# sijieaaa/AGPlace

Measured on AMD Instinct MI355X. Metric: aerial-ground pairs/sec (backbone+ODE+pool), higher is better.
Workload: dtype f16 (fp16 x fp16, fp32 accumulate); 1 GPU; nuScenes-AG 6-cam (C3/C4): MM.forward_q on [b,3,224,1344] + DBVanilla2D on [b,1,3,224,224], ResNet18 stem+layer1-3, euler h=0.1 x3 FCODE, GeM, stage-2 fusion; inference forward; the voxel branch's pooled outputs enter as fixed tensors (SURVEY.md 8d); global_batch=64, parallelism=dp1, bn=per-rank (eval: running statistics), paired_trunks=True, hipgraph=True, steps_in_flight=2, library_default_precision=4, headline_is_library_default=True, streams=2, query_sub_batches_on_streams=1, query_input=fp32 normalised panorama

## Files before the change

### agplace_amd/_lib.py

```python
import ctypes as C
import os

_HERE = os.path.dirname(os.path.abspath(__file__))
LIB_PATH = os.environ.get("AGP_HIP_LIB") or os.path.join(_HERE, "lib", "libagplace_hip.so")

AGP_OK = 0
PREC_BF16 = 1
PREC_F16W2 = 2
PREC_BF16X3 = 3
PREC_F16 = 4
FMT_BF16, FMT_F16 = 0, 1
ACT = {None: 0, "id": 0, "relu": 1, "tanh": 2, "sigmoid": 3}
ODE = {"euler": 0, "midpoint": 1, "rk4": 2}
ODE_ADAPTIVE = {"dopri5": 3}
ODE_STATUS = {0: "ok", 1: "odeint_max_steps attempted steps did not reach t = 1", 2: "step size underflow (t + dt == t)",
              3: "the error ratio is NaN"}
ODE_MAX_STEPS_LIMIT = 4096
E_UNSUPPORTED = 3
GP_FLOATS = 1 + 16384 + 1
_ERR = {1: "AGP_E_BADARG (unsupported shape / enum / null pointer)",
        2: "AGP_E_LAUNCH (HIP launch failed)",
        3: "AGP_E_UNSUPPORTED"}


class ConvDesc(C.Structure):
    _fields_ = [
        ("in_hi", C.c_void_p), ("in_lo", C.c_void_p),
        ("w_hi", C.c_void_p), ("w_lo", C.c_void_p),
        ("out_hi", C.c_void_p), ("out_lo", C.c_void_p),
        ("res_hi", C.c_void_p), ("res_lo", C.c_void_p),
        ("scale", C.c_void_p), ("shift", C.c_void_p),
        ("n", C.c_int32), ("hin", C.c_int32), ("win", C.c_int32), ("cin", C.c_int32),
        ("pin", C.c_int32), ("in_w_step", C.c_int32),
        ("hout", C.c_int32), ("wout", C.c_int32), ("cout", C.c_int32), ("pout", C.c_int32),
        ("kh", C.c_int32), ("kw", C.c_int32), ("stride", C.c_int32), ("pad", C.c_int32),
        ("relu", C.c_int32), ("prec", C.c_int32),
        ("w_q8", C.c_void_p), ("w_q8_exp", C.c_int32),
        ("stat_partial", C.c_void_p),
        ("pool_partial", C.c_void_p), ("pool_p", C.c_void_p), ("pool_eps", C.c_float), ("hi_only", C.c_int32),
        ("w_cm", C.c_void_p),
        ("bstat_z_hi", C.c_void_p), ("bstat_z_lo", C.c_void_p), ("bstat_y_hi", C.c_void_p),
        ("bstat_mean", C.c_void_p), ("bstat_rstd", C.c_void_p),
        ("w_cm_lo", C.c_void_p),
        ("in_h16", C.c_void_p), ("out_absmax", C.c_void_p),
        ("pool_stat", C.c_int32), ("reserved0", C.c_int32),
    ]


class BBlock64Desc(C.Structure):
    _fields_ = [("inp", C.c_void_p), ("out", C.c_void_p), ("w1", C.c_void_p), ("w2", C.c_void_p),
                ("scale1", C.c_void_p), ("shift1", C.c_void_p), ("scale2", C.c_void_p), ("shift2", C.c_void_p),
                ("pool_partial", C.c_void_p), ("n", C.c_int32), ("h", C.c_int32), ("w", C.c_int32), ("form", C.c_int32)]


class VecProgOp(C.Structure):
    _fields_ = [("op", C.c_int32), ("dst", C.c_int32), ("r", C.c_int32 * 6), ("k", C.c_int32), ("act", C.c_int32),
                ("aux", C.c_int32), ("n", C.c_int32), ("f0", C.c_float), ("pad", C.c_int32), ("p", C.c_void_p * 6)]


VP_LOAD, VP_STORE, VP_LINEAR, VP_FCODE, VP_L2NORM, VP_LAYERNORM, VP_WSUM = 1, 2, 3, 4, 5, 6, 7
VECPROG_MAXOPS, VECPROG_NREG = 36, 6

_P, _I, _L, _F = C.c_void_p, C.c_int, C.c_int64, C.c_float

SIGNATURES = {
    "agp_version": (C.c_char_p, []),
    "agp_arch": (C.c_char_p, []),
    "agp_range_flag_set": (_P, [_P]),
    "agp_range_flag_get": (_P, []),
    "agp_split_f32": (_I, [_P, _P, _P, _L, _I, _P]),
    "agp_split_conv_weight": (_I, [_P, _I, _I, _I, _I, _I, _P, _P, _P]),
    "agp_split_conv_weight_both": (_I, [_P, _I, _I, _I, _I, _P, _P, _P, _P, _I, _P]),
    "agp_pack_f32_to_nhwc": (_I, [_P, _L, _L, _L, _L, _I, _I, _I, _I, _I, _I, _P, _P, _P]),
    "agp_pack_f32_to_nhwc4_h16": (_I, [_P, _L, _L, _L, _L, _I, _I, _I, _I, _I, _P, _P, _P, _P]),
    "agp_pack_u8_cams_to_nhwc": (_I, [_P, _I, _I, _I, _I, C.POINTER(_F), C.POINTER(_F), _I, _P, _P, _P]),
    "agp_resize_ksize": (_I, [_I, _I]),
    "agp_resize_coeffs": (_I, [_I, _I, C.POINTER(C.c_int32), C.POINTER(C.c_int32)]),
    "agp_resized_size": (_I, [_I, _I, _I, C.POINTER(_I), C.POINTER(_I)]),
    "agp_resize_u8_cams": (_I, [_P, _I, _I, _I, _I, _I, _I, _P, _P, _P, _P, _P, _P]),
    "agp_resize_pack_u8_cams": (_I, [_P, _I, _I, _I, _I, _I, _I, _P, _P, _P, _P, C.POINTER(_F), C.POINTER(_F), _I, _P, _P, _P]),
    "agp_unpack_nhwc_to_f32": (_I, [_P, _P, _I, _I, _I, _I, _I, _P, _P]),
    "agp_map_zero_halo": (_I, [_P, _P, _I, _I, _I, _I, _I, _P]),
    "agp_map_absmax": (_I, [_P, _P, _I, _I, _I, _I, _I, _P, _P]),
    "agp_map_absmax_reset": (_I, [_P, _I, _P]),
    "agp_conv2d_fwd": (_I, [C.POINTER(ConvDesc), _P]),
    "agp_conv2d_fwd_grouped": (_I, [C.POINTER(ConvDesc), _I, _P]),
    "agp_bblock64_fwd_grouped": (_I, [C.POINTER(BBlock64Desc), _I, _P]),
    "agp_bblock64_pool_floats": (_L, [C.POINTER(BBlock64Desc)]),
    "agp_bblock64_pool_finish": (_I, [_P, _I, _I, _I, _P, _P]),
    "agp_conv_w_q8_prepare": (_I, [_P, _I, _I, _P, C.POINTER(C.c_int32), _P]),
    "agp_conv2d_tile_plan": (_I, [C.POINTER(ConvDesc), _I, C.POINTER(C.c_int32)]),
    "agp_conv2d_stat_tiles": (_I, [C.POINTER(ConvDesc)]),
    "agp_conv2d_pool_blocks": (_I, [C.POINTER(ConvDesc)]),
    "agp_pool_from_conv": (_I, [_P, _I, _I, _I, _I, _P, _P, _P, _P]),
    "agp_bn_stats_from_partial": (_I, [_P, _I, _I, _L, _F, _F, _P, _P, _P, _P, _P, _P, _P, _P, _P]),
    "agp_stem_pool_fwd": (_I, [C.POINTER(ConvDesc), _P]),
    "agp_stem_pool_raw_fwd": (_I, [C.POINTER(ConvDesc), _I, _L, _L, _L, _L, _I, C.POINTER(_F), C.POINTER(_F), _P]),
    "agp_maxpool3x3s2_fwd": (_I, [_P, _P, _I, _I, _I, _I, _I, _P, _P, _I, _I, _I, _P, _P]),
    "agp_bcast_add_fwd": (_I, [_P, _P, _P, _I, _I, _I, _I, _I, _P, _P, _I, _P]),
    "agp_pool_workspace_floats": (_L, [_I, _I, _I, _I]),
    "agp_pool_fwd": (_I, [_P, _P, _I, _I, _I, _I, _I, _P, _F, _P, _P, _P, _P]),
    "agp_pool_f32_fwd": (_I, [_P, _L, _L, _L, _L, _I, _I, _I, _I, _P, _F, _P, _P, _P, _P]),
    "agp_gem_f32_bwd": (_I, [_P, _L, _L, _L, _L, _I, _I, _I, _I, _P, _F, _P, _P, _P, _P, _P]),
    "agp_linear_fwd": (_I, [_P, _P, _P, _P, _P, _P, _I, _I, _I, _I, _P, _P]),
    "agp_fcode_fwd": (_I, [_P, _P, _P, _P, _P, _P, _I, _I, _I, C.POINTER(_F), _I, _P, _P, _P]),
    "agp_fcode_traj_floats": (_L, [_I, _I, _I]),
    "agp_fcode_bwd_workspace_bytes": (_L, [_I, _I, _I]),
    "agp_fcode_bwd": (_I, [_P, _P, _P, _P, _I, _I, _I, C.POINTER(_F), _I, _P, _P, _P, _P, _L, _P]),
    "agp_fcode_adaptive_ctrl_bytes": (_L, [_I]),
    "agp_fcode_adaptive_ring_floats": (_L, [_I, _I, _I]),
    "agp_fcode_adaptive_fwd": (_I, [_P, _P, _P, _P, _P, _P, _I, _I, _I, C.c_double, C.c_double, _I, _P, _P, _I, _P, _P]),
    "agp_fcode_adaptive_bwd_workspace_bytes": (_L, [_I, _I]),
    "agp_fcode_adaptive_bwd": (_I, [_P, _P, _P, _P, _P, _I, _I, _I, _I, _P, _P, _P, _P, _L, _P]),
    "agp_linear_bwd_workspace_bytes": (_L, [_I, _I, _I]),
    "agp_linear_bwd": (_I, [_P, _P, _P, _P, _P, _I, _I, _I, _I, _P, _P, _P, _P, _L, _P]),
    "agp_layernorm_bwd": (_I, [_P, _P, _P, _P, _I, _I, _F, _I, _P, _P, _P, _P, _P]),
    "agp_l2normalize_bwd": (_I, [_P, _P, _I, _I, _P, _P]),
    "agp_layernorm_fwd": (_I, [_P, _P, _P, _P, _I, _I, _F, _I, _P, _P]),
    "agp_l2normalize_fwd": (_I, [_P, _I, _I, _P, _P]),
    "agp_wsum_fwd": (_I, [_P] * 12 + [_L, _P, _P]),
    "agp_dot_f32": (_I, [_P, _P, _L, _P, _P]),
    "agp_vecprog_run": (_I, [C.POINTER(VecProgOp), _I, _I, _I, C.POINTER(_F), _I, _P]),
    "agp_vecprog_run2": (_I, [C.POINTER(VecProgOp), _I, _I, C.POINTER(VecProgOp), _I, _I, _I, C.POINTER(_F), _I, _P]),
    "agp_conv2d_wgrad_workspace_bytes": (_L, [C.POINTER(ConvDesc)]),
    "agp_conv2d_wgrad": (_I, [C.POINTER(ConvDesc), _P, _P, _L, _P]),
    "agp_conv2d_wgrad_param": (_I, [C.POINTER(ConvDesc), _P, _I, _P, _L, _P]),
    "agp_upsample2_zero": (_I, [_P, _P, _I, _I, _I, _I, _I, _P, _P, _I, _I, _I, _P]),
    "agp_train_reduce_workspace_floats": (_L, [_I, _I, _I, _I]),
    "agp_bn_stats": (_I, [_P, _P, _I, _I, _I, _I, _I, _F, _F] + [_P] * 10),
    "agp_map_affine": (_I, [_P, _P, _P, _P, _P, _P, _I, _I, _I, _I, _I, _I, _P, _P, _P, _P]),
    "agp_bn_bwd": (_I, [_P] * 9 + [_I] * 6 + [_P] * 9),
    "agp_bn_bwd_from_partial": (_I, [_P, _I] + [_P] * 9 + [_I] * 7 + [_P] * 8),
    "agp_bn_bwd_frozen": (_I, [_P] * 9 + [_I] * 6 + [_P] * 9),
    "agp_bn_sums": (_I, [_P, _P, _I, _I, _I, _I, _I, _P, _P, _P]),
    "agp_bn_sums_from_partial": (_I, [_P, _I, _I, _L, _P, _P]),
    "agp_bn_stats_from_sums": (_I, [_P, _I, _F, _F] + [_P] * 9),
    "agp_bn_bwd_sums": (_I, [_P] * 8 + [_I] * 6 + [_P] * 5),
    "agp_bn_bwd_apply": (_I, [_P] * 11 + [_I] * 6 + [_P] * 6),
    "agp_bn_frozen_coeffs": (_I, [_P, _P, _P, _P, _I, _F, _P, _P, _P, _P, _P]),
    "agp_map_chan_sum": (_I, [_P, _P, _I, _I, _I, _I, _I, _P, _P, _P]),
    "agp_map_add": (_I, [_P] * 6 + [_I] * 5 + [_P, _P, _P]),
    "agp_maxpool3x3s2_bwd": (_I, [_P, _P, _P] + [_I] * 8 + [_P, _P, _P]),
    "agp_maxpool_bn_bwd": (_I, [_P, _P, _P, _I, _I, _I] + [_P] * 12 + [_I] * 7 + [_P] * 7),
    "agp_affine_maxpool3x3s2_fwd": (_I, [_P, _P, _P, _P] + [_I] * 5 + [_P, _P] + [_I] * 3 + [_P, _P, _P]),
    "agp_pool_bwd": (_I, [_P, _P, _P, _P, _P, _P, _F, _P, _P, _I, _I, _I, _I, _I, _P, _P, _P, _P]),
    "agp_netvlad_fwd": (_I, [_P, _P, _P, _I, _I, _I, _I, _I, _P, _P]),
    "agp_netvlad_bwd": (_I, [_P, _P, _P, _P, _I, _I, _I, _I, _I, _P, _P, _P, _P, _P]),
    "agp_netvlad_workspace_bytes": (_L, [_I, _I, _I, _I]),
    "agp_netvlad_fwd_mfma": (_I, [_P, _P, _P, _I, _I, _I, _I, _I, _P, _P, _L, _P]),
    "agp_sparse_conv_fwd": (_I, [_P, _P, _L, _P, _L, _I, _I, _I, _P, _P, _P, _P, _P, _P, _I, _P, _P, _I, _P, _P, _P, _P]),
    "agp_sparse_tile_taps": (_I, [_P, _L, _I, _L, _P, _P, _P, _L, _P]),
    "agp_sparse_zplane_perm": (_I, [_P, _P, _I, _L, _P, _P]),
    "agp_sparse_kernel_map": (_I, [_P, _L, _P, _L, _P, _I, _P, _P, _P]),
    "agp_sparse_kernel_map_grid": (_I, [_P, _L, _P, _L, _I, _I, _I, _P, _P, _P, _P, _P]),
    "agp_sparse_conv_cin1_fwd": (_I, [_P, _L, _P, _L, _I, _P, _I, _P, _P, _I, _P, _P, _P, _P]),
    "agp_sparse_conv0_fwd": (_I, [_P, _L, _P, _P, _I, _I, _P, _I, _P, _P, _I, _P, _P, _P, _I, _P]),
    "agp_sparse_coords_workspace_bytes": (_L, [_L, _I, _I]),
    "agp_sparse_build": (_I, [_P, _I, _L, _P, _I, _I, _P, _P, _P, _P, _P, _P, _L, _P]),
    "agp_sparse_coarsen": (_I, [_P, _P, _L, _I, _I, _P, _P, _P, _P, _L, _P]),
    "agp_sparse_points_workspace_bytes": (_L, [_L, _I]),
    "agp_sparse_build_points": (_I, [_P, _P, _L, _I, _F, _P, _I, _P, _P, _P, _P, _P, _P, _L, _P]),
    "agp_seg_pool_fwd": (_I, [_P, _P, _P, _I, _I, _P, _F, _P, _P, _P]),
    "agp_eca_scale_fwd": (_I, [_P, _I, _I, _P, _I, _P, _P]),
    "agp_seg_affine_fwd": (_I, [_P, _P, _P, _P, _P, _P, _P, _L, _I, _I, _P, _P, _P, _P]),
    "agp_sparse_conv_wgrad_workspace_bytes": (_L, [_L, _I, _I, _I]),
    "agp_sparse_conv_wgrad": (_I, [_P, _P, _L, _P, _L, _I, _I, _I, _P, _P, _P, _P, _L, _P]),
    "agp_sparse_conv_cin1_wgrad": (_I, [_P, _L, _P, _L, _I, _P, _P, _I, _P, _P, _I, _P]),
    "agp_seg_dot_fwd": (_I, [_P, _P, _P, _P, _P, _I, _I, _P, _P]),
    "agp_eca_scale_bwd": (_I, [_P, _P, _P, _P, _I, _I, _P, _I, _P, _P, _P]),
    "agp_seg_pool_bwd": (_I, [_P, _P, _P, _P, _P, _P, _P, _P, _F, _P, _P, _L, _I, _P, _P, _P, _P]),
    "agp_triplet_loss_workspace_floats": (_L, [_I]),
    "agp_triplet_loss": (_I, [_P, _I, _I, _P, _I, _F, _P, _P, _P, _P]),
    "agp_sare_loss": (_I, [_P, _I, _I, _P, _I, _I, _P, _P, _P, _P]),
    "agp_pairdist_loss_workspace_floats": (_L, [_I, _I]),
    "agp_pairdist_loss": (_I, [_P, _P, _I, _I, _I, _P, _P, _F, _F, _I, _P, _P, _P, _P, _P, _P]),
    "agp_mine_best_positive": (_I, [_P, _L, _P, _L, _I, _P, _P, _P, _P, _P]),
    "agp_knn_pad_rows": (_L, [_L]),
    "agp_knn_prepare_db": (_I, [_P, _L, _I, _I, _P, _P, _P, _P]),
    "agp_knn_workspace_bytes": (_L, [_L, _L, _I, _I]),
    "agp_knn_search": (_I, [_P, _L, _P, _P, _P, _P, _L, _I, _I, _I, _P, _P, _P, _L, _P]),
    "agp_knn_coarse_pass": (_I, [_P, _L, _P, _P, _P, _L, _I, _I, _P, _L, _P]),
}

_lib = None


def load():
    global _lib
    if _lib is not None:
        return _lib
    if not os.path.exists(LIB_PATH):
        raise RuntimeError(
            f"agplace_amd: HIP extension not built: {LIB_PATH} is missing. Run "
            "`python -c 'import __graft_entry__ as g; g.build()'` (or `make -C agplace_amd/csrc`). "
            "There is no CPU fallback.")
    import torch
    lib = C.CDLL(LIB_PATH)
    for name, (res, args) in SIGNATURES.items():
        fn = getattr(lib, name)
        fn.restype = res
        fn.argtypes = args
    _lib = lib
    return lib


def check(rc, what):
    if rc != AGP_OK:
        raise RuntimeError(f"{what} failed: {_ERR.get(rc, rc)}")


def ptr(t):
    return None if t is None else t.data_ptr()


def stream():
    import torch
    return torch.cuda.current_stream().cuda_stream
```

### agplace_amd/csrc/igemm.hip

```cpp

#ifndef AGP_SCHED
#define AGP_SCHED 0
#endif

#include "igemm_params.hpp"

namespace agp_igemm {


template <int BK> struct Swz;
template <> struct Swz<32> { __device__ static __forceinline__ int f(int row) { return (row >> 2) & 3; } };
template <> struct Swz<64> { __device__ static __forceinline__ int f(int row) { return (row >> 1) & 7; } };

template <int WM, int WN, int BK, int NPREC, int NST>
constexpr int igemm_lds_bytes() {
    constexpr int stage = (WM * 64 * PrecT<NPREC>::XPL + WN * 64 * PrecT<NPREC>::WPL) * BK * 2;
    constexpr int epi = WM * WN * 32 * EPI_ROWB + (NPREC == 3 ? WM * WN * 64 * 2 * 4 : 0);
    return (NST * stage > epi) ? NST * stage : epi;
}

#if defined(__HIP_DEVICE_COMPILE__)
template <int WM, int WN, int BK, int NPREC, int EPI, int NST, bool RG = false>
__device__ __forceinline__ void igemm_body(const IgemmParams& p, const int bid, uint32_t* rflag = nullptr) {
    constexpr int BM = WM * 64, BN = WN * 64, NW = WM * WN;
// ... 379 lines not shown
    }
    for (int i = n; i < 5; ++i) g.start[i] = grid;
    if (plan) {
        *plan = TilePlan{AGP_CONV_KERNEL_GENERIC, WM * 64, WN * 64, mt, one_nt ? ps[0].NT : 0, mt, 0, grid};
        return AGP_OK;
    }
    static std::atomic<uint64_t> attr_done{0};
    if (!agp_lds_attr((const void*)igemm_group_kernel<WM, WN, BK, NPREC, EPI_CONV, NST, RG>, lds, attr_done)) return AGP_E_LAUNCH;
    g.rflag = RG ? agp_range_flag_get() : nullptr;
    AGP_LAUNCH((igemm_group_kernel<WM, WN, BK, NPREC, EPI_CONV, NST, RG>), dim3(grid), dim3(WM * WN * 64), lds, s, g);
    AGP_CHECK_LAUNCH();
    return AGP_OK;
}

int launch_group_f16(IgemmParams* ps, int n, hipStream_t s, TilePlan* plan = nullptr) {
#if defined(AGP_TUNING)
    const int var = AGP_TUNE("GROUP_VARIANT", 0);
    if (var == 1) return launch_group_f16_cfg<64, 2>(ps, n, s, plan);
    if (var == 2) return launch_group_f16_cfg<32, 2>(ps, n, s, plan);
#endif
    return agp_rg_dispatch(agp_range_flag_get(), [&](auto rg) { return launch_group_f16_cfg<32, 3, decltype(rg)::value>(ps, n, s, plan); });
}

template <int WM, int WN, int BK, int NPREC, int EPI, int NST, bool RG = false>
int launch_cfg_rg(IgemmParams& p, uint32_t* rflag, hipStream_t s, TilePlan* plan = nullptr) {
    constexpr int lds = igemm_lds_bytes<WM, WN, BK, NPREC, NST>();
    static_assert(lds <= 160 * 1024, "LDS budget");
    constexpr int BM = WM * 64, BN = WN * 64;
    p.MT = (p.M + BM - 1) / BM;
    p.NT = (p.N + BN - 1) / BN;
    p.mt_chunk = (p.MT + 7) / 8;
    const int grid = p.mt_chunk * 8 * p.NT;
    if (plan) {
        *plan = TilePlan{AGP_CONV_KERNEL_GENERIC, BM, BN, p.MT, p.NT, p.MT, 0, grid};
        return AGP_OK;
    }
    static std::atomic<uint64_t> attr_done{0};
    if (!agp_lds_attr((const void*)igemm_kernel<WM, WN, BK, NPREC, EPI, NST, RG>, lds, attr_done)) return AGP_E_LAUNCH;
    const int splits = 1;
    AGP_LAUNCH((igemm_kernel<WM, WN, BK, NPREC, EPI, NST, RG>), dim3(grid, splits), dim3(WM * WN * 64), lds, s, p, rflag);
    AGP_CHECK_LAUNCH();
    return AGP_OK;
}
template <int WM, int WN, int BK, int NPREC, int EPI, int NST>
int launch_cfg(IgemmParams& p, hipStream_t s, TilePlan* plan = nullptr) {
    if constexpr (EPI == EPI_CONV && PrecT<NPREC>::F16) {
        uint32_t* const rflag = agp_range_flag_get();
        return agp_rg_dispatch(rflag, [&](auto rg) { return launch_cfg_rg<WM, WN, BK, NPREC, EPI, NST, decltype(rg)::value>(p, rflag, s, plan); });
    }
    return launch_cfg_rg<WM, WN, BK, NPREC, EPI, NST>(p, nullptr, s, plan);
}

inline int igemm_variant() { return AGP_TUNE("IGEMM_VARIANT", 0); }

template <int EPI>
int launch_igemm(IgemmParams& p, int prec, hipStream_t s, TilePlan* plan = nullptr) {
    const bool wide = (p.N % 128 == 0) || (EPI == EPI_GMIN);
    const int var = igemm_variant();
    p.dbg = AGP_TUNE("IGEMM_DBG", 0);
    if (EPI == EPI_GMIN && var == 0) {
        if (prec == AGP_PREC_BF16X3) return launch_cfg<4, 2, 32, 3, EPI, 2>(p, s, plan);
        if (prec == AGP_PREC_BF16)
            return p.CK % 64 == 0 ? launch_cfg<4, 2, 64, 1, EPI, 2>(p, s, plan) : launch_cfg<4, 2, 32, 1, EPI, 2>(p, s, plan);
        if (prec == AGP_PREC_F16)
            return p.CK % 64 == 0 ? launch_cfg<4, 2, 64, 4, EPI, 2>(p, s, plan) : launch_cfg<4, 2, 32, 4, EPI, 2>(p, s, plan);
        return AGP_E_BADARG;
    }
    if (prec == AGP_PREC_BF16X3) {
#if defined(AGP_TUNING)
        if (var == 1) return wide ? launch_cfg<2, 2, 32, 3, EPI, 3>(p, s, plan) : launch_cfg<4, 1, 32, 3, EPI, 3>(p, s, plan);
        if (var == 2) return wide ? launch_cfg<4, 2, 32, 3, EPI, 2>(p, s, plan) : launch_cfg<4, 1, 32, 3, EPI, 2>(p, s, plan);
        if (var == 3) return wide ? launch_cfg<4, 2, 32, 3, EPI, 3>(p, s, plan) : launch_cfg<4, 1, 32, 3, EPI, 3>(p, s, plan);
        if (var == 4) return wide ? launch_cfg<2, 2, 32, 3, EPI, 4>(p, s, plan) : launch_cfg<4, 1, 32, 3, EPI, 4>(p, s, plan);
#endif
        return wide ? launch_cfg<2, 2, 32, 3, EPI, 2>(p, s, plan) : launch_cfg<4, 1, 32, 3, EPI, 2>(p, s, plan);
    } else if (prec == AGP_PREC_BF16) {
        if (p.CK % 64 == 0) {
#if defined(AGP_TUNING)
            if (var == 1) return wide ? launch_cfg<2, 2, 64, 1, EPI, 3>(p, s, plan) : launch_cfg<4, 1, 64, 1, EPI, 3>(p, s, plan);
#endif
            return wide ? launch_cfg<2, 2, 64, 1, EPI, 2>(p, s, plan) : launch_cfg<4, 1, 64, 1, EPI, 2>(p, s, plan);
        }
        return wide ? launch_cfg<2, 2, 32, 1, EPI, 2>(p, s, plan) : launch_cfg<4, 1, 32, 1, EPI, 2>(p, s, plan);
    }
    if constexpr (EPI == EPI_CONV) {
        if (prec == AGP_PREC_F16W2)
            return wide ? launch_cfg<2, 2, 32, 2, EPI, 2>(p, s, plan) : launch_cfg<4, 1, 32, 2, EPI, 2>(p, s, plan);
        if (prec == AGP_PREC_F16) {
#if defined(AGP_TUNING)
            if (var == 5) {
                if (p.CK % 64 == 0) return wide ? launch_cfg<2, 2, 64, 4, EPI, 2>(p, s, plan) : launch_cfg<4, 1, 64, 4, EPI, 2>(p, s, plan);
                return wide ? launch_cfg<2, 2, 32, 4, EPI, 2>(p, s, plan) : launch_cfg<4, 1, 32, 4, EPI, 2>(p, s, plan);
            }
#endif
            if (p.tap_stride && var == 0) {
                if (!wide) return launch_cfg<4, 1, 32, 4, EPI, 2>(p, s, plan);
                if ((int64_t)((p.M + 255) / 256) * (p.N / 128) >= 512) return launch_cfg<4, 2, 32, 4, EPI, 3>(p, s, plan);
            }
            return wide ? launch_cfg<2, 2, 32, 4, EPI, 3>(p, s, plan) : launch_cfg<4, 1, 32, 4, EPI, 3>(p, s, plan);
        }
    }
    return AGP_E_BADARG;
}

}
using namespace agp_igemm;

int agp_internal_conv_d16(agp_igemm::IgemmParams& p, int prec, hipStream_t s, agp_igemm::TilePlan* plan);
int agp_internal_conv_d16_pool(agp_igemm::IgemmParams& p, int prec, hipStream_t s);
int agp_internal_stem_raw(agp_igemm::IgemmParams& p, int kind, const void* x, long long sn, long long sc, long long sh, long long sw,
                          int h, int w, int ncam, const float* mean3, const float* std3, hipStream_t s);
int agp_internal_conv_kxr(agp_igemm::IgemmParams& p, const agp_conv_desc* d, hipStream_t s, agp_igemm::TilePlan* plan);

extern "C" int agp_conv2d_stat_tiles(const agp_conv_desc* d) {
    if (!d || d->prec != AGP_PREC_BF16X3) return 0;
    const int force = AGP_TUNE("CONV_KERNEL", 0);
    if (d->in_w_step != d->cin && !force && d->cout % 64 == 0)
        return (int)(((int64_t)d->n * d->hout * d->wout + 255) / 256);
    if (d->in_w_step == d->cin && !force && !AGP_TUNE("IGEMM_VARIANT", 0) && d->cin % 32 == 0 && d->cout % 64 == 0 &&
        !(d->kh == 3 && d->kw == 3 && d->stride == 1 && d->pad == 1)) {
        const int bm = (d->cout % 128 == 0) ? 128 : 256;
        return (int)(((int64_t)d->n * d->hout * d->wout + bm - 1) / bm);
    }
    const bool kxr_ok = d->kh == 3 && d->kw == 3 && d->stride == 1 && d->pad == 1 && d->pin == 1 &&
                        d->pout == 1 && d->in_w_step == d->cin && d->hout == d->hin && d->wout == d->win &&
                        (int64_t)d->n * (d->hin + 2) * (d->win + 2) * d->cin * 2 < (1ll << 31);
    if (!kxr_ok || d->cin % 32 || d->cout % 64 || (force && force != 3)) return 0;
    const int64_t m = (int64_t)d->n * d->hin * (d->win + 2);
    const int bm = (d->cout % 128 == 0 && !d->hi_only) ? 128 : 256;
    return (int)((m + bm - 1) / bm);
}

static bool conv_kxr_ok(const agp_conv_desc* d);
bool agp_internal_use_kxr2(const agp_conv_desc* d);

extern "C" int agp_conv2d_pool_blocks(const agp_conv_desc* d) {
    if (!d || d->prec != AGP_PREC_F16 || d->in_lo || d->out_lo || d->cin % 32 || d->cout % 64 || d->n <= 0) return 0;
    if (!conv_kxr_ok(d) || !agp_internal_use_kxr2(d) || AGP_TUNE("CONV_KERNEL", 0) || AGP_TUNE("NO_CONV_POOL", 0)) return 0;
    const int64_t rp = ((int64_t)d->hin * (d->win + 2) + 63) / 64 * 64;
    if ((int64_t)d->n * rp >= (1ll << 31)) return 0;
    return (int)(((int64_t)d->n * rp + 511) / 512 * 8);
}

static bool conv_kxr_ok(const agp_conv_desc* d) {
    return d->kh == 3 && d->kw == 3 && d->stride == 1 && d->pad == 1 && d->pin == 1 &&
           d->pout == 1 && d->in_w_step == d->cin && d->hout == d->hin && d->wout == d->win &&
           (int64_t)d->n * (d->hin + 2) * (d->win + 2) * d->cin * 2 < (1ll << 31);
}

static int conv_fill_params(const agp_conv_desc* d, IgemmParams& p);
void agp_internal_conv_kxr_geometry(agp_igemm::IgemmParams& p, const agp_conv_desc* d);
bool agp_internal_use_kxr2(const agp_conv_desc* d);
int agp_internal_conv_kxr2(agp_igemm::IgemmParams* ps, int n, hipStream_t s, agp_igemm::TilePlan* plan);
int agp_internal_conv_s2(agp_igemm::IgemmParams* ps, const agp_conv_desc* descs, int n, hipStream_t s, agp_igemm::TilePlan* plan);

static int conv2d_fwd_one(const agp_conv_desc* d, void* stream, TilePlan* plan);

static int conv2d_fwd_group(const agp_conv_desc* descs, int n, void* stream, TilePlan* plan) {
    if (!descs || n <= 0) return AGP_E_BADARG;
    bool group = n >= 2 && n <= 4;
    for (int i = 0; i < n && group; ++i) {
        const agp_conv_desc* d = descs + i;
        group = d->in_hi && d->w_hi && d->out_hi && !d->in_lo && !d->out_lo && !d->res_lo && d->n > 0 &&
                d->cin % 32 == 0 && d->cout % 64 == 0 && conv_kxr_ok(d) && agp_internal_use_kxr2(d) &&
                d->cin == descs[0].cin && d->cout == descs[0].cout && !AGP_TUNE("CONV_KERNEL", 0);
    }
    if (!group && !AGP_TUNE("CONV_KERNEL", 0) && !AGP_TUNE("NO_S2", 0)) {
        const int h = n / 2;
        bool s2 = (n == 2 || n == 4);
        for (int i = 0; i < h && s2; ++i) {
            const agp_conv_desc* c = descs + i;
            const agp_conv_desc* d = descs + h + i;
            s2 = c->prec == AGP_PREC_F16 && d->prec == AGP_PREC_F16 && c->in_hi && c->w_hi && c->out_hi && d->w_hi && d->out_hi &&
                 !c->in_lo && !c->out_lo && !d->in_lo && !d->out_lo && !c->res_hi && !d->res_hi && !c->stat_partial && !d->stat_partial &&
                 !c->pool_partial && !d->pool_partial &&
                 c->kh == 3 && c->kw == 3 && c->stride == 2 && c->pad == 1 && c->pin == 1 && c->pout == 1 && c->in_w_step == c->cin &&
                 d->kh == 1 && d->kw == 1 && d->stride == 2 && d->pad == 0 && d->pin == 1 && d->pout == 1 && d->in_w_step == d->cin &&
                 d->in_hi == c->in_hi && d->n == c->n && d->hin == c->hin && d->win == c->win && d->cin == c->cin &&
                 d->cout == c->cout && d->hout == c->hout && d->wout == c->wout && !d->relu &&
                 c->hout == (c->hin - 1) / 2 + 1 && c->wout == (c->win - 1) / 2 + 1 &&
                 c->cin % 32 == 0 && c->cout % 64 == 0 && c->n > 0 && c->cin == descs[0].cin && c->cout == descs[0].cout &&
                 (int64_t)c->n * (c->hin + 2) * (c->win + 2) * c->cin * 2 < (1ll << 31) &&
                 (int64_t)c->n * (c->hout + 2) * (c->wout + 2) * c->cout * 2 < (1ll << 31);
        }
        if (s2) {
            IgemmParams ps[2];
            for (int i = 0; i < h; ++i) {
                ps[i] = IgemmParams{};
                const int rc = conv_fill_params(descs + i, ps[i]);
                if (rc != AGP_OK) return rc;
                const agp_conv_desc* d = descs + h + i;
                ps[i].w2_hi = d->w_hi; ps[i].w2_cm = d->w_cm; ps[i].scale2 = d->scale; ps[i].shift2 = d->shift; ps[i].o2_hi = d->out_hi;
            }
            return agp_internal_conv_s2(ps, descs, h, (hipStream_t)stream, plan);
        }
    }
    if (!group) {
        bool g2 = n >= 2 && n <= 4 && !AGP_TUNE("CONV_KERNEL", 0) && !AGP_TUNE("NO_IGEMM_GROUP", 0);
        for (int i = 0; i < n && g2; ++i) {
            const agp_conv_desc* d = descs + i;
            g2 = d->in_hi && d->w_hi && d->out_hi && !d->in_lo && !d->out_lo && !d->res_lo && d->n > 0 &&
                 d->prec == AGP_PREC_F16 && !d->stat_partial && d->cin % 64 == 0 && d->cout % 128 == 0 &&
                 !conv_kxr_ok(d) && d->in_w_step == d->cin && !(d->pin < d->pad);
        }
        if (g2) {
            IgemmParams ps[4];
            for (int i = 0; i < n; ++i) {
                ps[i] = IgemmParams{};
                const int rc = conv_fill_params(descs + i, ps[i]);
                if (rc != AGP_OK) return rc;
            }
            return launch_group_f16(ps, n, (hipStream_t)stream, plan);
        }
        if (plan && n > 1) return AGP_E_UNSUPPORTED;
        for (int i = 0; i < n; ++i) {
            const int rc = conv2d_fwd_one(descs + i, stream, plan);
            if (rc != AGP_OK) return rc;
        }
        return AGP_OK;
    }
    IgemmParams ps[4];
    for (int i = 0; i < n; ++i) {
        ps[i] = IgemmParams{};
        const int rc = conv_fill_params(descs + i, ps[i]);
        if (rc != AGP_OK) return rc;
        agp_internal_conv_kxr_geometry(ps[i], descs + i);
    }
    return agp_internal_conv_kxr2(ps, n, (hipStream_t)stream, plan);
}

extern "C" int agp_conv2d_fwd_grouped(const agp_conv_desc* descs, int n, void* stream) {
    return conv2d_fwd_group(descs, n, stream, nullptr);
}

extern "C" int agp_conv2d_fwd(const agp_conv_desc* d, void* stream) { return conv2d_fwd_one(d, stream, nullptr); }

extern "C" int agp_conv2d_tile_plan(const agp_conv_desc* descs, int n, int32_t plan[8]) {
    if (!descs || !plan || n <= 0) return AGP_E_BADARG;
    TilePlan tp = {};
    const int rc = n == 1 ? conv2d_fwd_one(descs, nullptr, &tp) : conv2d_fwd_group(descs, n, nullptr, &tp);
    if (rc != AGP_OK) return rc;
    const int32_t v[8] = {tp.kernel, tp.BM, tp.BN, tp.MT, tp.NT, tp.MT_full, tp.half_tiles, tp.grid};
    for (int i = 0; i < 8; ++i) plan[i] = v[i];
    return AGP_OK;
}

static int conv2d_fwd_one(const agp_conv_desc* d, void* stream, TilePlan* plan) {
    if (!d || !d->in_hi || !d->w_hi || !d->out_hi) return AGP_E_BADARG;
    if (d->prec == AGP_PREC_BF16X3) {
        if ((!d->hi_only && (!d->in_lo || !d->w_lo)) || !d->out_lo || (d->res_hi && !d->res_lo)) return AGP_E_BADARG;
    } else if (d->prec == AGP_PREC_F16W2 || d->prec == AGP_PREC_F16) {
        if (d->in_lo || d->out_lo || d->res_lo) return AGP_E_BADARG;
        if (d->prec == AGP_PREC_F16W2 && !d->w_lo) return AGP_E_BADARG;
    } else {
        return AGP_E_BADARG;
    }
    if (d->cin % 32 || d->cout % 64 || d->n <= 0) return AGP_E_BADARG;
    if (d->pin < d->pad && d->in_w_step == d->cin) return AGP_E_BADARG;
    IgemmParams p = {};
    {
        const int rc = conv_fill_params(d, p);
        if (rc != AGP_OK) return rc;
    }
    const int force = AGP_TUNE("CONV_KERNEL", 0);
    const bool kxr_ok = conv_kxr_ok(d);
    const bool stem = d->in_w_step != d->cin;
#if defined(AGP_TUNING)
    if (p.dbg & 0x1000000) {
        const uint64_t a = ((uint64_t)(uint32_t)AGP_TUNE("CENSUS_BUF_HI", 0) << 32) | (uint32_t)AGP_TUNE("CENSUS_BUF_LO", 0);
        p.gmin = (float*)(uintptr_t)a;
        if (!p.gmin) p.dbg &= ~0x1000000;
    }
#endif
    int which = force ? force : (kxr_ok ? 3 : (stem ? 2 : 1));
    if (which == 3 && !kxr_ok) which = stem ? 2 : 1;
    if (d->hi_only && (d->prec != AGP_PREC_BF16X3 || which != 3)) return AGP_E_BADARG;
    if (d->w_cm && d->w_cm == d->w_hi && (which != 3 || !p.w_cm)) return AGP_E_BADARG;
    if (which == 3) return agp_internal_conv_kxr(p, d, (hipStream_t)stream, plan);
    if (which == 2) return agp_internal_conv_d16(p, d->prec, (hipStream_t)stream, plan);
    return launch_igemm<EPI_CONV>(p, d->prec, (hipStream_t)stream, plan);
}

static int conv_fill_params(const agp_conv_desc* d, IgemmParams& p) {
    const int hp = d->hin + 2 * d->pin, wp = d->win + 2 * d->pin;
    const int wstep = d->in_w_step;
    const int64_t x_elems = (int64_t)d->n * hp * wp * wstep;
    const int64_t w_elems = (int64_t)d->cout * d->kh * d->kw * d->cin;
    if (x_elems * 2 >= (1ll << 32) || w_elems * 2 >= (1ll << 31)) return AGP_E_BADARG;
    p.x_hi = d->in_hi; p.x_lo = d->in_lo; p.x_bytes = (uint32_t)(x_elems * 2);
    p.w_hi = d->w_hi; p.w_lo = d->w_lo; p.w_bytes = (uint32_t)(w_elems * 2);
    if (d->prec == AGP_PREC_F16W2 && d->w_q8) { p.w_q8 = d->w_q8; p.w_q8_exp = d->w_q8_exp; }
    if (d->prec == AGP_PREC_F16 && d->w_cm) p.w_cm = d->w_cm;
    if ((d->prec == AGP_PREC_F16W2 || d->prec == AGP_PREC_BF16X3) && d->w_cm && d->kh == 3 && d->kw == 3 &&
        d->stride == 1 && d->pad == 1 && d->in_w_step == d->cin && (d->w_cm_lo || (d->hi_only && d->prec == AGP_PREC_BF16X3))) {
        p.w_cm = d->w_cm; p.w_cm_lo = d->w_cm_lo;
    }
    if (d->stat_partial) {
        if (agp_conv2d_stat_tiles(d) <= 0) return AGP_E_BADARG;
        p.stat_partial = d->stat_partial;
        if (d->bstat_z_hi) {
            if (!d->bstat_mean || !d->bstat_rstd || d->in_w_step != d->cin ||
                !(d->kh == 3 && d->kw == 3 && d->stride == 1 && d->pad == 1))
                return AGP_E_BADARG;
            p.bs_z_hi = d->bstat_z_hi; p.bs_z_lo = d->bstat_z_lo; p.bs_y_hi = d->bstat_y_hi;
            p.bs_mean = d->bstat_mean; p.bs_rstd = d->bstat_rstd;
        }
    } else if (d->bstat_z_hi) {
        return AGP_E_BADARG;
    }
    if (d->pool_partial) {
        if (agp_conv2d_pool_blocks(d) <= 0) return AGP_E_BADARG;
        if (d->pool_stat != 0 && d->pool_stat != 1) return AGP_E_BADARG;
        p.pool_partial = d->pool_partial; p.pool_p = d->pool_stat ? nullptr : d->pool_p; p.pool_eps = d->pool_eps; p.pool_sq = d->pool_stat;
    }
    p.M = d->n * d->hout * d->wout;
    p.N = d->cout;
    p.KW = d->kw; p.CK = d->cin; p.ntaps = d->kh * d->kw;
    p.Ktot = d->kh * d->kw * d->cin;
    p.d_howo = make_fastdiv((uint32_t)(d->hout * d->wout));
    p.d_wo = make_fastdiv((uint32_t)d->wout);
    p.x_sw = wstep; p.x_sh = wp * wstep; p.x_sn = hp * wp * wstep;
    p.x_base = ((d->pin - d->pad) * wp + (d->pin - d->pad)) * wstep;
    p.sy = d->stride; p.sx = d->stride;
    const int hop = d->hout + 2 * d->pout, wop = d->wout + 2 * d->pout;
    p.o_hi = d->out_hi; p.o_lo = d->out_lo;
    p.o_sw = d->cout; p.o_sh = wop * d->cout; p.o_sn = hop * wop * d->cout;
    p.o_base = (d->pout * wop + d->pout) * d->cout;
    p.r_hi = d->res_hi; p.r_lo = d->res_lo;
    p.scale = d->scale; p.shift = d->shift; p.relu = d->relu;
    p.dbg = AGP_TUNE("IGEMM_DBG", 0);
    return AGP_OK;
}

int agp_internal_gmin(const void* q_hi, const void* q_lo, int64_t nq, const void* db_hi,
                      const void* db_lo, const float* db_norm, int64_t nb, int64_t nb_pad, int d,
                      int prec, float* gmin, int gq_stride, hipStream_t s) {
    IgemmParams p = {};
    if (nq * d * 2 >= (1ll << 32) || nb_pad * d * 2 >= (1ll << 31)) return AGP_E_BADARG;
    p.x_hi = q_hi; p.x_lo = q_lo; p.x_bytes = (uint32_t)(nq * d * 2);
    p.w_hi = db_hi; p.w_lo = db_lo; p.w_bytes = (uint32_t)(nb_pad * d * 2);
    p.M = (int)nq; p.N = (int)nb; p.Ktot = d; p.KW = 1; p.CK = d; p.ntaps = 1;
    p.d_howo = make_fastdiv(1); p.d_wo = make_fastdiv(1);
    p.x_sn = d; p.x_sh = 0; p.x_sw = 0; p.x_base = 0; p.sy = 1; p.sx = 1;
    p.gmin = gmin; p.wnorm = db_norm; p.gq_stride = gq_stride;
    return launch_igemm<EPI_GMIN>(p, prec, s);
}


extern "C" int agp_sparse_conv_fwd(const void* f_hi, const void* f_lo, int64_t n_in_rows, const int32_t* nbr, int64_t n_out,
                                   int cin, int cout, int ntaps, const void* w_hi, const void* w_lo, const float* scale,
                                   const float* shift, const void* res_hi, const void* res_lo, int relu, void* out_hi,
                                   void* out_lo, int prec, const int64_t* n_dev, const int32_t* row_perm, const uint32_t* tile_taps, void* stream) {
    if (!f_hi || !nbr || !w_hi || !out_hi || n_out <= 0 || n_in_rows <= 0 || ntaps <= 0) return AGP_E_BADARG;
    if (cin % 32 || cout % 64) return AGP_E_BADARG;
    if (prec == AGP_PREC_BF16X3) { if (!f_lo || !w_lo || !out_lo || (res_hi && !res_lo)) return AGP_E_BADARG; }
    else if (prec == AGP_PREC_F16W2 || prec == AGP_PREC_F16) { if (f_lo || out_lo || res_lo || (prec == AGP_PREC_F16W2 && !w_lo)) return AGP_E_BADARG; }
    else return AGP_E_BADARG;
    const int64_t x_elems = n_in_rows * cin, w_elems = (int64_t)cout * ntaps * cin;
    if (x_elems * 2 >= (1ll << 31) || w_elems * 2 >= (1ll << 31) || n_out * (int64_t)cout * 2 >= (1ll << 31)) return AGP_E_BADARG;
    IgemmParams p = {};
    p.x_hi = f_hi; p.x_lo = f_lo; p.x_bytes = (uint32_t)(x_elems * 2);
    p.w_hi = w_hi; p.w_lo = w_lo; p.w_bytes = (uint32_t)(w_elems * 2);
    p.M = (int)n_out; p.N = cout; p.Ktot = ntaps * cin;
    p.KW = ntaps; p.CK = cin; p.ntaps = ntaps;
    p.d_howo = make_fastdiv((uint32_t)n_out); p.d_wo = make_fastdiv((uint32_t)n_out);
    p.x_sn = 0; p.x_sh = 0; p.x_sw = 0; p.x_base = 0; p.sy = 1; p.sx = 1;
    p.xrow_tab = nbr; p.tap_stride = (int)n_out; p.tab_mul = cin; p.m_dev = n_dev; p.row_perm = row_perm; p.tile_taps = tile_taps;
    p.o_hi = out_hi; p.o_lo = out_lo; p.o_sn = 0; p.o_sh = 0; p.o_sw = cout; p.o_base = 0;
    p.r_hi = res_hi; p.r_lo = res_lo; p.scale = scale; p.shift = shift; p.relu = relu;
    return launch_igemm<EPI_CONV>(p, prec, (hipStream_t)stream);
}

static int stem_pool_impl(const agp_conv_desc* d, int kind, int64_t sn, int64_t sc, int64_t sh, int64_t sw, int ncam,
                          const float* mean3, const float* std3, void* stream) {
    if (!d || !d->in_hi || !d->w_hi || !d->out_hi || d->in_lo || d->out_lo || d->res_hi) return AGP_E_BADARG;
    if (d->prec != AGP_PREC_F16W2 && d->prec != AGP_PREC_F16) return AGP_E_BADARG;
    if (d->prec == AGP_PREC_F16W2 && !d->w_lo) return AGP_E_BADARG;
    if (d->cin != 32 || d->in_w_step != 4 || d->kw != 1 || d->kh != 7 || d->stride != 2 || d->pad != 3 || d->pin != 3 ||
        d->cout != 64 || !d->relu || d->n <= 0)
        return AGP_E_BADARG;
    const int h1 = (d->hin + 2 * 3 - 7) / 2 + 1, w1 = (d->win + 2 * 3 - 7) / 2 + 1;
    const int h2 = (h1 + 2 - 3) / 2 + 1, w2 = (w1 + 2 - 3) / 2 + 1;
    if (d->hout != h2 || d->wout != w2) return AGP_E_BADARG;
    IgemmParams p = {};
    const int hp = d->hin + 6, wp = d->win + 6;
    const int64_t x_elems = (int64_t)d->n * hp * wp * 4;
    const int64_t w_elems = (int64_t)64 * 7 * 32;
    if (kind == 0 && x_elems * 2 >= (1ll << 32)) return AGP_E_BADARG;
// ... 27 lines not shown
```

### agplace_amd/csrc/igemm_kxr2.hip

```cpp

#include <type_traits>

#include "igemm_params.hpp"

#ifndef AGP_CENSUS
#define AGP_CENSUS 0
#endif
#if AGP_CENSUS
#define KXR2_STAMP(i) do { if (census && tid == 0) rec[4 + (i)] = __builtin_amdgcn_s_memrealtime(); } while (0)
#else
#define KXR2_STAMP(i) do { } while (0)
#endif

namespace agp_igemm {

constexpr int KXR2_MAXP = 4;
struct Kxr2Group {
    IgemmParams p[KXR2_MAXP];
    int mt_end[KXR2_MAXP];
    int nprob, MT, NT, mt_chunk;
};

constexpr int KXR2_BM = 256, KXR2_MINB = 3;
constexpr int kxr2_lds_bytes() { return 2 * (KXR2_BM + 16) * 64 + 3 * 64 * 64 + 2 * 64 * 4; }
// ... 249 lines not shown
    }

    KXR2_STAMP(2);
    if (p.dbg & 128) {
        float t = 0.f;
#pragma unroll
        for (int a = 0; a < TN; ++a)
#pragma unroll
            for (int b = 0; b < TM; ++b)
#pragma unroll
                for (int r = 0; r < 16; ++r) t += acc[a][b][r];
        if (t == 1.2345e30f) ((float*)p.o_hi)[0] = t;
        return;
    }
    asm volatile("s_waitcnt lgkmcnt(0)" ::: "memory");
    __builtin_amdgcn_s_barrier();
    constexpr int ERS = 144;
    char* const strip = smem + wave * (32 * ERS);
    const int a_off = l31 * ERS + lh * 16;
    const int l_off = (lane >> 3) * ERS + (lane & 7) * 16;
    const float* tb = tab + 8 * lh;
    bf16_t* const ohi = (bf16_t*)p.o_hi;
    const float relu_lo = p.relu ? 0.f : -65504.f;
    RangeTrack<RG> rg;
    u32x4 rres[TM][TN * 2];
    if (rhi) {
#pragma unroll
        for (int tm = 0; tm < TM; ++tm) {
#pragma unroll
            for (int i = 0; i < 4; ++i) *(u32x4*)(strip + l_off + i * (8 * ERS)) = rpf[tm * 4 + i];
            __builtin_amdgcn_fence(__ATOMIC_RELEASE, "wavefront");
#pragma unroll
            for (int jj = 0; jj < TN * 2; ++jj) rres[tm][jj] = *(const u32x4*)(strip + a_off + jj * 32);
            __builtin_amdgcn_fence(__ATOMIC_RELEASE, "wavefront");
        }
    }
    float psum[2] = {0.f, 0.f};
    const float* const ppp = POOL ? p.pool_p : nullptr;
    const float pool_pw = ppp ? ppp[0] : 1.f, pool_eps = POOL ? p.pool_eps : 0.f;
    const bool pool_cube = pool_pw == 3.f;
    const bool pool_sq = POOL && p.pool_sq;
#pragma unroll
    for (int tm = 0; tm < TM; ++tm) {
        u32x4 outv[TN * 2];
#pragma unroll
        for (int jp = 0; jp < TN; ++jp) {
            f32x4 sc4[2][2], sh4[2][2];
#pragma unroll
            for (int u = 0; u < 2; ++u) {
                const int jj = 2 * jp + u;
                sc4[u][0] = *(const f32x4*)(tb + 16 * jj);
                sc4[u][1] = *(const f32x4*)(tb + 16 * jj + 4);
                sh4[u][0] = *(const f32x4*)(tb + BN + 16 * jj);
                sh4[u][1] = *(const f32x4*)(tb + BN + 16 * jj + 4);
            }
#pragma unroll
            for (int u = 0; u < 2; ++u) {
                const int jj = 2 * jp + u;
                float v[8];
#pragma unroll
                for (int e = 0; e < 8; ++e) v[e] = acc[jj >> 1][tm][8 * (jj & 1) + e] * sc4[u][e >> 2][e & 3] + sh4[u][e >> 2][e & 3];
                if (rhi) {
                    float r[8];
                    unpack8_h(rres[tm][jj], r);
#pragma unroll
                    for (int e = 0; e < 8; ++e) v[e] += r[e];
                }
                rg.any8(v);
                outv[jj] = pack8_h_lo(v, relu_lo);
            }
        }
#pragma unroll
        for (int jj = 0; jj < TN * 2; ++jj) *(u32x4*)(strip + a_off + jj * 32) = outv[jj];
        __builtin_amdgcn_fence(__ATOMIC_RELEASE, "wavefront");
        u32x4 lines[4];
#pragma unroll
        for (int i = 0; i < 4; ++i) lines[i] = *(const u32x4*)(strip + l_off + i * (8 * ERS));
#pragma unroll
        for (int i = 0; i < 4; ++i) {
            const int off = eoff[tm * 4 + i];
            if (off >= 0) *(u32x4*)(ohi + off) = lines[i];
        }
        if constexpr (POOL) {
            if (ppart) {
                const bf16_t* const col = (const bf16_t*)strip + lane;
                const uint32_t mk = pmask[tm];
#pragma unroll
                for (int p8 = 0; p8 < 32; p8 += 8) {
                    float v[8];
#pragma unroll
                    for (int u = 0; u < 8; ++u) v[u] = h2f(col[(p8 + u) * (ERS / 2)]);
#pragma unroll
                    for (int u = 0; u < 8; ++u) {
                        const bool a = (mk >> (p8 + u)) & 1u;
                        psum[0] += a ? v[u] : 0.f;
                        if (pool_sq) {
                            psum[1] += a ? v[u] * v[u] : 0.f;
                        } else if (ppp) {
                            const float c = fmaxf(v[u], pool_eps);
                            const float gq = pool_cube ? c * c * c : __builtin_exp2f(pool_pw * __builtin_log2f(c));
                            psum[1] += a ? gq : 0.f;
                        }
                    }
                }
            }
        }
        __builtin_amdgcn_fence(__ATOMIC_RELEASE, "wavefront");
    }
    if constexpr (POOL) {
        if (ppart && n0 + lane < pN) {
            float* o = ppart + ((size_t)(mt * NW + wave) * 2) * pN + n0 + lane;
            o[0] = psum[0];
            if (ppp || pool_sq) o[pN] = psum[1];
        }
    }
    rg.flush(rg_word(rf...), relu_lo);
#if AGP_CENSUS
    if (census && tid == 0) {
        rec[4 + 3] = __builtin_amdgcn_s_memrealtime();
        asm volatile("s_waitcnt vmcnt(0)" ::: "memory");
        rec[3] = __builtin_amdgcn_s_memrealtime();
    }
#endif
#endif
}

template <bool POOL, bool RG>
int launch_kxr2(Kxr2Group& g, hipStream_t s, TilePlan* plan) {
    constexpr int BM = KXR2_BM, lds = kxr2_lds_bytes();
    static_assert(lds * KXR2_MINB <= 160 * 1024, "LDS budget of the intended workgroups per CU");
    static std::atomic<uint64_t> attr_done{0};
    int mt = 0;
    for (int i = 0; i < g.nprob; ++i) {
        mt += (g.p[i].M + BM - 1) / BM;
        g.mt_end[i] = mt;
    }
    const XcdGrid xg = xcd_grid(mt, (g.p[0].N + 63) / 64);
    if (plan) return plan_xcd(plan, AGP_CONV_KERNEL_KXR2, BM, 64, xg);
    g.MT = xg.MT;
    g.NT = xg.NT;
    g.mt_chunk = xg.mt_chunk;
    if (!agp_lds_attr(RG ? (const void*)igemm_kxr2_kernel<POOL, uint32_t*> : (const void*)igemm_kxr2_kernel<POOL>, lds, attr_done)) return AGP_E_LAUNCH;
    if constexpr (RG) {
        AGP_LAUNCH((igemm_kxr2_kernel<POOL, uint32_t*>), dim3(xg.blocks), dim3(256), lds, s, g, agp_range_flag_get());
    } else {
        AGP_LAUNCH((igemm_kxr2_kernel<POOL>), dim3(xg.blocks), dim3(256), lds, s, g);
    }
    AGP_CHECK_LAUNCH();
    return AGP_OK;
}

}

int agp_internal_conv_kxrw(agp_igemm::IgemmParams* ps, int n, hipStream_t s, agp_igemm::TilePlan* plan);

int agp_internal_conv_kxr2(agp_igemm::IgemmParams* ps, int n, hipStream_t s, agp_igemm::TilePlan* plan) {
    using namespace agp_igemm;
    if (n < 1 || n > KXR2_MAXP) return AGP_E_BADARG;
    if (AGP_TUNE("KXR_WIDE", 1) && ps[0].N % 128 == 0) return agp_internal_conv_kxrw(ps, n, s, plan);
    Kxr2Group g = {};
    g.nprob = n;
    for (int i = 0; i < n; ++i) {
        if (ps[i].N != ps[0].N || ps[i].CK != ps[0].CK) return AGP_E_BADARG;
        g.p[i] = ps[i];
    }
    bool pool = false;
    for (int i = 0; i < n; ++i) pool = pool || ps[i].pool_partial != nullptr;
    return agp_rg_dispatch(agp_range_flag_get(), [&](auto rg) {
        constexpr bool RG = decltype(rg)::value;
        if (pool) return launch_kxr2<true, RG>(g, s, plan);
        return launch_kxr2<false, RG>(g, s, plan);
    });
}
```

### agplace_amd/csrc/igemm_kxrw.hip

```cpp

#include <type_traits>

#include "igemm_params.hpp"

namespace agp_igemm {

constexpr int KXRW_MAXP = 4;
struct KxrwGroup {
    IgemmParams p[KXRW_MAXP];
    int mt_end[KXRW_MAXP];
    int nprob, MT, NT, mt_chunk;
    int MT_full, half_bid0;
    uint32_t* rflag;
    uint32_t r_bytes[KXRW_MAXP];
};
constexpr uint32_t KXRW_ROOB = 0xffffff00u;

constexpr int KW_ROWB = 64;
template <int TM_, int TN_> struct KwShape {
    static constexpr int BM = 128 * TM_, BN = 32 * TN_, BMX = BM + 16;
    static constexpr int XBUF = BMX * KW_ROWB, WTAP = BN * KW_ROWB;
    static constexpr int LDS = 2 * XBUF + 3 * WTAP + 2 * BN * 4;
    static constexpr int STRIP = 32 * 2 * BN, XWAVES = XBUF / STRIP, SPARE = LDS + (TM_ == 1 ? 2048 : 0);
    static constexpr int EPI_LDS = SPARE + (4 - XWAVES) * STRIP;
};

template <bool POOL, int TM_, int TN_, bool RG, bool RES>
__device__ __forceinline__ void kxrw_tile(const KxrwGroup& g, const int pid, const int m0, const int n0) {
#if defined(__HIP_DEVICE_COMPILE__)
    using SH = KwShape<TM_, TN_>;
    constexpr int BN = SH::BN, NW = 4, TM = TM_, TN = TN_, ROWB = KW_ROWB;
    constexpr int X_BUF = SH::XBUF, W_TAP = SH::WTAP;
    constexpr int XINS = SH::BMX / 16;
    constexpr int NX = (XINS + NW - 1) / NW;
    constexpr int NWP = BN / (NW * 16);
    static_assert(TN == 4 && (TM == 2 || TM == 1), "the full tile (256 x 128) and its half tile (128 x 128)");
    static_assert(NWP == 2 && (NX == 5 || NX == 3), "the vmcnt counts exist for these");
    extern __shared__ __attribute__((aligned(16))) char smem[];
    char* const ws = smem + 2 * X_BUF;
    float* const tab = (float*)(ws + 3 * W_TAP);

    const int tid = threadIdx.x;
    const int lane = tid & 63;
    const int wave = __builtin_amdgcn_readfirstlane(tid >> 6);

    const IgemmParams& p = g.p[pid];

    const FastDiv d_howo = p.d_howo, d_wo = p.d_wo;
    const int pM = p.M, pN = p.N, pKtot = p.Ktot;
    const uint32_t pR = (uint32_t)p.img_rows;
    const int x_sn = p.x_sn, x_sh_ = p.x_sh, x_sw = p.x_sw, x_base = p.x_base;
    const int o_sn = p.o_sn, o_sw = p.o_sw, o_base = p.o_base;
    const float* const pscale = p.scale;
    const float* const pshift = p.shift;

    const int lrow = lane >> 2, lpos = lane & 3;
    int xoff[NX], woff[NWP];
#pragma unroll
    for (int q = 0; q < NX; ++q) {
        int ins = wave + NW * q;
        ins = ins < XINS ? ins : XINS - 1;
        const int row = ins * 16 + lrow;
        const int m = m0 + row;
        const uint32_t img = fdiv((uint32_t)m, d_howo);
        const uint32_t rem = (uint32_t)m - img * d_howo.d;
        const uint32_t y = fdiv(rem, d_wo);
        const uint32_t xq = rem - y * d_wo.d;
        const int el = (int)img * x_sn + (int)y * x_sh_ + (int)xq * x_sw + x_base;
        xoff[q] = el * 2 + ((lpos ^ swz32(row)) << 4);
    }
#pragma unroll
    for (int i = 0; i < NWP; ++i) {
        const int row = (wave + NW * i) * 16 + lrow;
        int n = n0 + row;
        n = n < pN ? n : pN - 1;
        woff[i] = (p.w_cm ? n * 64 : n * pKtot * 2) + ((lpos ^ swz32(row)) << 4);
    }
    const __amdgpu_buffer_rsrc_t rx = __builtin_amdgcn_make_buffer_rsrc((void*)p.x_hi, 0, p.x_bytes, 0x00020000);
    const __amdgpu_buffer_rsrc_t rw = __builtin_amdgcn_make_buffer_rsrc((void*)(p.w_cm ? p.w_cm : p.w_hi), 0, p.w_bytes, 0x00020000);

    const int CK = __builtin_amdgcn_readfirstlane(p.CK), x_sh = __builtin_amdgcn_readfirstlane(x_sh_);
    const int cchunks = CK / 32;
    const int nsteps = 3 * cchunks;
    const int tapb = CK * 2;
    float tab_s = 1.f, tab_t = 0.f;
    if (tid < BN) {
        const int n = n0 + tid < pN ? n0 + tid : pN - 1;
        if (pscale) tab_s = pscale[n];
        if (pshift) tab_t = pshift[n];
    }
    float pool_pw_v = 1.f;
    if (POOL && p.pool_p) pool_pw_v = p.pool_p[0];
    auto load_x = [&](int buf, int ky_, int cc_) {
        const int xs = __builtin_amdgcn_readfirstlane((ky_ * x_sh + cc_ * 32) * 2);
        char* base_ = smem + buf * X_BUF;
#pragma unroll
        for (int q = 0; q < NX; ++q) {
            int ins = wave + NW * q;
            ins = ins < XINS ? ins : XINS - 1;
            __builtin_amdgcn_raw_ptr_buffer_load_lds(rx, LDS_PTR(base_ + ins * 1024), 16, xoff[q], xs, 0, 0);
        }
    };
    const int wmul = __builtin_amdgcn_readfirstlane(p.w_cm ? pN : 1);
    auto load_w = [&](int slot, int wbytes) {
        const int so = __builtin_amdgcn_readfirstlane(wbytes * wmul);
#pragma unroll
        for (int i = 0; i < NWP; ++i)
            __builtin_amdgcn_raw_ptr_buffer_load_lds(rw, LDS_PTR(ws + slot * W_TAP + (wave + NW * i) * 1024), 16, woff[i], so, 0, 0);
    };
    load_x(0, 0, 0);
    load_w(0, 0);
    load_w(1, tapb);

    const int l31 = lane & 31, lh = lane >> 5;
    int xrd[3][2], wrd[2];
#pragma unroll
    for (int kx = 0; kx < 3; ++kx)
#pragma unroll
        for (int ks = 0; ks < 2; ++ks) {
            const int r = wave * (TM * 32) + l31 + kx;
            xrd[kx][ks] = r * ROWB + (((2 * ks + lh) ^ swz32(r)) << 4);
        }
    {
        const int wrow = (l31 & 0x13) | ((l31 & 4) << 1) | ((l31 & 8) >> 1);
#pragma unroll
        for (int ks = 0; ks < 2; ++ks) wrd[ks] = wrow * ROWB + (((2 * ks + lh) ^ swz32(wrow)) << 4);
    }

    f32x16 acc[TN][TM];
#pragma unroll
    for (int a = 0; a < TN; ++a)
#pragma unroll
        for (int b = 0; b < TM; ++b)
#pragma unroll
            for (int r = 0; r < 16; ++r) acc[a][b][r] = 0.f;

    constexpr int LPP = BN / 8, PPI = 64 / LPP, NEI = 32 / PPI;
    int eoff[TM * NEI];
    {
        const uint32_t wlast = d_wo.d - 1;
        const int img_extra = o_sn - (int)d_howo.d * o_sw;
#pragma unroll
        for (int q = 0; q < TM * NEI; ++q) {
            const int m = m0 + wave * (TM * 32) + (q / NEI) * 32 + (q % NEI) * PPI + lane / LPP;
            const uint32_t mm = (uint32_t)(m < pM ? m : pM - 1);
            const uint32_t img = fdiv(mm, d_howo);
            const uint32_t rem = mm - img * d_howo.d;
            const uint32_t y = fdiv(rem, d_wo);
            const uint32_t xq = rem - y * d_wo.d;
            const bool ok = (m < pM) && rem < pR && xq != 0 && xq != wlast;
            const int chunk = (lane % LPP) ^ (((q % NEI) * PPI + lane / LPP) & 15);
            eoff[q] = ok ? (int)mm * o_sw + (int)img * img_extra + o_base + n0 + 8 * chunk : -1;
        }
    }
    float* const ppart = POOL ? p.pool_partial : nullptr;
    static_assert(LPP == 16 && PPI == 4 && NEI == 8 && SH::STRIP == NEI * 1024, "a tile row = 8 pieces of 4 pixel lines of 256 bytes");
    const int xidle = nsteps & 1;
    char* const strip0 = wave < SH::XWAVES ? smem + xidle * X_BUF + wave * SH::STRIP : smem + SH::SPARE + (wave - SH::XWAVES) * SH::STRIP;
    char* const strip1 = wave < 2 ? smem + (xidle ^ 1) * X_BUF + wave * SH::STRIP : ws + (wave - 2) * SH::STRIP;
    static_assert(TM == 1 || (SH::XWAVES == 2 && 2 * SH::STRIP <= 3 * W_TAP), "tile row 1: two waves per X buffer, two in the W ring");
    const __amdgpu_buffer_rsrc_t rr = __builtin_amdgcn_make_buffer_rsrc((void*)p.r_hi, 0, g.r_bytes[pid], 0x00020000);
    auto load_residual = [&](char* strip, int tm, int i) {
        const int off = eoff[tm * NEI + i];
        __builtin_amdgcn_raw_ptr_buffer_load_lds(rr, LDS_PTR(strip + i * 1024), 16, off >= 0 ? off * 2 : (int)KXRW_ROOB, 0, 0, 0);
    };

    int ky = 0, cc = 0;
    wait_vm_lgkm<NWP>();
    __builtin_amdgcn_s_barrier();
    if (tid < BN) { tab[tid] = tab_s; tab[BN + tid] = tab_t; }
    const float pool_pw = __builtin_bit_cast(float, __builtin_amdgcn_readfirstlane(__builtin_bit_cast(int, pool_pw_v)));
    auto phase = [&](auto KX, auto LAST, const char* xb, int st_, int nky_, int ncc_, int wcur_, int wnext_) {
        constexpr int kx = decltype(KX)::value;
        constexpr bool last = decltype(LAST)::value;
        constexpr int nres = last && RES && kx < 2 ? NEI / 2 : 0;
        const char* wb = ws + kx * W_TAP;
        bf16x8 xf[2][TM], wf[2][TN];
#pragma unroll
        for (int t = 0; t < TM; ++t) xf[0][t] = *(const bf16x8*)(xb + xrd[kx][0] + t * (32 * ROWB));
#pragma unroll
        for (int t = 0; t < TN; ++t) wf[0][t] = *(const bf16x8*)(wb + wrd[0] + t * (32 * ROWB));
        constexpr int ndma = (kx == 0 ? (last ? NWP : NWP + NX) : (last ? 0 : NWP)) + nres;
        static_assert(ndma <= 8, "one piece per MFMA pair");
#pragma unroll
        for (int t = 0; t < TM; ++t) xf[1][t] = *(const bf16x8*)(xb + xrd[kx][1] + t * (32 * ROWB));
#pragma unroll
        for (int t = 0; t < TN; ++t) wf[1][t] = *(const bf16x8*)(wb + wrd[1] + t * (32 * ROWB));
        auto piece = [&](int i) {
            if (nres && i >= ndma - nres) {
                load_residual(strip0, 0, kx * (NEI / 2) + i - (ndma - nres));
            } else if (kx == 0) {
                if (i < NWP) {
                    const int so = __builtin_amdgcn_readfirstlane((wcur_ + 2 * tapb) * wmul);
                    __builtin_amdgcn_raw_ptr_buffer_load_lds(rw, LDS_PTR(ws + 2 * W_TAP + (wave + NW * i) * 1024), 16, woff[i], so, 0, 0);
                } else {
                    const int q = i - NWP;
                    const int xs = __builtin_amdgcn_readfirstlane((nky_ * x_sh + ncc_ * 32) * 2);
                    int ins = wave + NW * q;
                    ins = ins < XINS ? ins : XINS - 1;
                    __builtin_amdgcn_raw_ptr_buffer_load_lds(rx, LDS_PTR(smem + ((st_ + 1) & 1) * X_BUF + ins * 1024), 16, xoff[q], xs, 0, 0);
                }
            } else {
                const int so = __builtin_amdgcn_readfirstlane((wnext_ + (kx - 1) * tapb) * wmul);
                __builtin_amdgcn_raw_ptr_buffer_load_lds(rw, LDS_PTR(ws + (kx - 1) * W_TAP + (wave + NW * i) * 1024), 16, woff[i], so, 0, 0);
            }
        };
        int ip = 0;
#pragma unroll
        for (int ks = 0; ks < 2; ++ks)
#pragma unroll
            for (int tn = 0; tn < TN; ++tn)
#pragma unroll
                for (int tm = 0; tm < TM; ++tm) {
                    acc[tn][tm] = __builtin_amdgcn_mfma_f32_32x32x16_f16(__builtin_bit_cast(f16x8, wf[ks][tn]),
                                                                         __builtin_bit_cast(f16x8, xf[ks][tm]), acc[tn][tm], 0, 0, 0);
                    if ((TM == 1 || (tm & 1)) && ip < ndma) { piece(ip); ++ip; }
                }
        __builtin_amdgcn_sched_group_barrier(0x100, 2 * (TM + TN), 0);
#pragma unroll
        for (int i = 0; i < 8; ++i) {
            __builtin_amdgcn_sched_group_barrier(0x008, TM == 1 ? 1 : 2, 0);
            if (i < ndma) __builtin_amdgcn_sched_group_barrier(0x010, 1, 0);
        }
        __builtin_amdgcn_sched_barrier(0);
    };
    using I0 = std::integral_constant<int, 0>; using I1 = std::integral_constant<int, 1>; using I2 = std::integral_constant<int, 2>;
    using BF = std::false_type; using BT = std::true_type;
    for (int st = 0; st < nsteps - 1; ++st) {
        int nky = ky, ncc = cc + 1;
        if (ncc == cchunks) { ncc = 0; ++nky; }
        const int wcur = (ky * 3 * CK + cc * 32) * 2, wnext = (nky * 3 * CK + ncc * 32) * 2;
        const char* xb = smem + (st & 1) * X_BUF;
        phase(I0{}, BF{}, xb, st, nky, ncc, wcur, wnext);
        wait_vm_lgkm<NX + NWP>();
        __builtin_amdgcn_s_barrier();
        phase(I1{}, BF{}, xb, st, nky, ncc, wcur, wnext);
        wait_vm_lgkm<NX + NWP>();
        __builtin_amdgcn_s_barrier();
        phase(I2{}, BF{}, xb, st, nky, ncc, wcur, wnext);
        wait_vm_lgkm<NWP>();
        __builtin_amdgcn_s_barrier();
        ky = nky; cc = ncc;
    }
    {
        const int st = nsteps - 1;
        const int wcur = (ky * 3 * CK + cc * 32) * 2;
        const char* xb = smem + (st & 1) * X_BUF;
        phase(I0{}, BT{}, xb, st, 0, 0, wcur, 0);
        wait_vm_lgkm<NWP + (RES ? NEI / 2 : 0)>();
        __builtin_amdgcn_s_barrier();
        phase(I1{}, BT{}, xb, st, 0, 0, wcur, 0);
        wait_vm_lgkm<(RES ? NEI : 0)>();
        __builtin_amdgcn_s_barrier();
        phase(I2{}, BT{}, xb, st, 0, 0, wcur, 0);
    }

    asm volatile("s_waitcnt lgkmcnt(0)" ::: "memory");
    __builtin_amdgcn_s_barrier();
    if constexpr (RES) {
        if constexpr (TM == 2) {
#pragma unroll
            for (int i = 0; i < NEI; ++i) load_residual(strip1, 1, i);
            wait_vm_lgkm<NEI>();
        } else {
            wait_vm_lgkm<0>();
        }
    }
    const int a_off = l31 * (2 * BN) + ((lh ^ (l31 & 1)) << 4), a_swz = (l31 >> 1) & 7;
    const int l_off = lane * 16;
    const float* tb = tab + 8 * lh;
    bf16_t* const ohi = (bf16_t*)p.o_hi;
    const float relu_lo = p.relu ? 0.f : -65504.f;
    RangeTrack<RG> rg;
    float psum[2][2] = {{0.f, 0.f}, {0.f, 0.f}};
    float psum0[2][2] = {{0.f, 0.f}, {0.f, 0.f}};
    const float* const ppp = POOL ? p.pool_p : nullptr;
    const float pool_eps = POOL ? p.pool_eps : 0.f;
    const bool pool_cube = pool_pw == 3.f;
    const bool pool_sq = POOL && p.pool_sq;
#pragma unroll
    for (int tm = 0; tm < TM; ++tm) {
        char* const strip = tm == 0 ? strip0 : strip1;
        if constexpr (POOL && TM == 2) {
            if (tm == 1) {
#pragma unroll
                for (int a = 0; a < 2; ++a)
#pragma unroll
                    for (int b = 0; b < 2; ++b) { psum0[a][b] = psum[a][b]; psum[a][b] = 0.f; }
            }
        }
        u32x4 rres[TN * 2];
        if constexpr (RES) {
#pragma unroll
            for (int jj = 0; jj < TN * 2; ++jj) rres[jj] = *(const u32x4*)(strip + a_off + ((jj ^ a_swz) << 5));
        }
        u32x4 outv[TN * 2];
#pragma unroll
        for (int jj = 0; jj < TN * 2; ++jj) {
            const f32x4 s0 = *(const f32x4*)(tb + 16 * jj), s1 = *(const f32x4*)(tb + 16 * jj + 4);
            const f32x4 h0 = *(const f32x4*)(tb + BN + 16 * jj), h1 = *(const f32x4*)(tb + BN + 16 * jj + 4);
            float v[8];
#pragma unroll
            for (int e = 0; e < 8; ++e)
                v[e] = acc[jj >> 1][tm][8 * (jj & 1) + e] * (e < 4 ? s0[e & 3] : s1[e & 3]) + (e < 4 ? h0[e & 3] : h1[e & 3]);
            if constexpr (RES) {
                float r[8];
                unpack8_h(rres[jj], r);
#pragma unroll
                for (int e = 0; e < 8; ++e) v[e] += r[e];
            }
            rg.any8(v);
            outv[jj] = pack8_h_lo(v, relu_lo);
        }
#pragma unroll
        for (int jj = 0; jj < TN * 2; ++jj) *(u32x4*)(strip + a_off + ((jj ^ a_swz) << 5)) = outv[jj];
        __builtin_amdgcn_fence(__ATOMIC_RELEASE, "wavefront");
        u32x4 lines[NEI];
#pragma unroll
        for (int i = 0; i < NEI; ++i) lines[i] = *(const u32x4*)(strip + l_off + i * 1024);
        if constexpr (TM == 2) {
            if (tm == 0 && RES) wait_vm_lgkm<0>();
        }
#pragma unroll
        for (int i = 0; i < NEI; ++i) {
            const int off = eoff[tm * NEI + i];
            if (off >= 0) *(u32x4*)(ohi + off) = lines[i];
        }
        if constexpr (POOL) {
            if (ppart) {
#pragma unroll
                for (int i = 0; i < NEI; ++i)
                    if (eoff[tm * NEI + i] < 0) *(u32x4*)(strip + l_off + i * 1024) = u32x4{0u, 0u, 0u, 0u};
                __builtin_amdgcn_fence(__ATOMIC_RELEASE, "wavefront");
                auto sweep = [&](auto STAT) {
#pragma clang fp contract(off)
                    constexpr int stat = decltype(STAT)::value;
#pragma unroll
                    for (int p8 = 0; p8 < 32; p8 += 8) {
                        uint32_t w[8];
#pragma unroll
                        for (int u = 0; u < 8; ++u) w[u] = *(const uint32_t*)(strip + (p8 + u) * (2 * BN) + ((lane * 4) ^ (((p8 + u) & 15) << 4)));
#pragma unroll
                        for (int u = 0; u < 8; ++u) {
                            const float v0 = h2f((bf16_t)(w[u] & 0xffffu)), v1 = h2f((bf16_t)(w[u] >> 16));
                            psum[0][0] += v0;
                            psum[1][0] += v1;
                            if constexpr (stat == 1) {
                                psum[0][1] += v0 * v0;
                                psum[1][1] += v1 * v1;
                            } else if constexpr (stat >= 2) {
                                const float c0 = fmaxf(v0, pool_eps), c1 = fmaxf(v1, pool_eps);
                                psum[0][1] += stat == 2 ? c0 * c0 * c0 : __builtin_exp2f(pool_pw * __builtin_log2f(c0));
                                psum[1][1] += stat == 2 ? c1 * c1 * c1 : __builtin_exp2f(pool_pw * __builtin_log2f(c1));
                            }
                        }
                    }
                };
                using I3 = std::integral_constant<int, 3>;
                if (pool_sq) sweep(I1{});
                else if (!ppp) sweep(I0{});
                else if (pool_cube) sweep(I2{});
                else sweep(I3{});
            }
        }
        __builtin_amdgcn_fence(__ATOMIC_RELEASE, "wavefront");
    }
    if constexpr (POOL) {
        if (ppart) {
            if constexpr (TM == 2) {
#pragma unroll
                for (int a = 0; a < 2; ++a)
#pragma unroll
                    for (int b = 0; b < 2; ++b) psum[a][b] = psum0[a][b] + psum[a][b];
            }
            if constexpr (TM == 1) {
                float* const scr = (float*)(ws + 3 * W_TAP) + 2 * BN;
                if (wave & 1) *(f32x4*)(scr + ((wave >> 1) * 64 + lane) * 4) = f32x4{psum[0][0], psum[0][1], psum[1][0], psum[1][1]};
                __syncthreads();
                if (!(wave & 1)) {
                    const f32x4 o = *(const f32x4*)(scr + ((wave >> 1) * 64 + lane) * 4);
                    psum[0][0] += o[0]; psum[0][1] += o[1]; psum[1][0] += o[2]; psum[1][1] += o[3];
                }
            }
            if (TM == 2 || !(wave & 1)) {
                const int block = m0 / 64 + (TM == 2 ? wave : (wave >> 1));
#pragma unroll
                for (int h = 0; h < 2; ++h) {
                    const int n = n0 + 2 * lane + h;
                    if (n < pN) {
                        float* o = ppart + ((size_t)block * 2) * pN + n;
                        o[0] = psum[h][0];
                        if (ppp || pool_sq) o[pN] = psum[h][1];
                    }
                }
            }
        }
    }
    rg.flush(g.rflag, relu_lo);
#endif
}

template <bool POOL, bool MIX, bool RG>
__global__ void __launch_bounds__(256, 2) igemm_kxrw_kernel(KxrwGroup g) {
#if defined(__HIP_DEVICE_COMPILE__)
    constexpr int TM_ = 2, TN_ = 4;
    constexpr int BM = KwShape<TM_, TN_>::BM, BN = KwShape<TM_, TN_>::BN;
    const int bid = blockIdx.x;
    const int gNT = g.NT, gnprob = g.nprob;
    const int e0 = g.mt_end[0], e1 = g.mt_end[1], e2 = g.mt_end[2];
    int mt, nt, sub = 0;
    bool half = false;
    if (MIX && bid >= g.half_bid0) {
        const int h = bid - g.half_bid0;
        nt = h % gNT;
        const int hm = h / gNT;
        mt = g.MT_full + (hm >> 1);
        sub = hm & 1;
        half = true;
        if (mt >= g.MT) return;
    } else {
        const int xcd = bid & 7, j = bid >> 3;
        nt = j % gNT;
        mt = xcd * g.mt_chunk + j / gNT;
        if (mt >= g.MT_full) return;
    }
    const int pid = group_problem(mt, gnprob, e0, e1, e2);
    const int n0 = nt * BN;
    if constexpr (MIX) {
        if (half) {
            const int m0 = mt * BM + sub * (BM / 2);
            if (m0 >= g.p[pid].M) return;
            if (g.p[pid].r_hi) kxrw_tile<POOL, 1, TN_, RG, true>(g, pid, m0, n0);
            else kxrw_tile<POOL, 1, TN_, RG, false>(g, pid, m0, n0);
            return;
        }
    }
    if (g.p[pid].r_hi) kxrw_tile<POOL, TM_, TN_, RG, true>(g, pid, mt * BM, n0);
    else kxrw_tile<POOL, TM_, TN_, RG, false>(g, pid, mt * BM, n0);
#endif
}

struct KxrwPlan {
    int MT_full, mt_chunk, half_bid0, half_tiles, blocks;
    bool mix;
};
inline KxrwPlan kxrw_plan(int MT, int NT) {
    KxrwPlan k = {};
    k.MT_full = MT;
    const int slots = 512, T = MT * NT;
    const int tail = T - (T - 1) / slots * slots;
    if (tail <= slots / 4 && tail % NT == 0) {
        k.MT_full = MT - tail / NT;
        k.mix = true;
    }
    const XcdGrid xg = xcd_grid(k.MT_full, NT);
    k.mt_chunk = xg.mt_chunk;
    k.half_bid0 = xg.blocks;
    k.half_tiles = k.mix ? 2 * (MT - k.MT_full) * NT : 0;
    k.blocks = k.half_bid0 + k.half_tiles;
    return k;
}

template <bool POOL, bool MIX, bool RG>
int launch_kxrw(KxrwGroup& g, const KxrwPlan& k, hipStream_t s) {
    constexpr int lds = KwShape<2, 4>::EPI_LDS;
    static_assert(2 * lds <= 160 * 1024, "two workgroups per CU");
    static_assert(KwShape<1, 4>::EPI_LDS <= lds, "half tiles: their stage, the pooling scratch and their strips fit the full tile's LDS");
    static std::atomic<uint64_t> attr_done{0};
    if (!agp_lds_attr((const void*)igemm_kxrw_kernel<POOL, MIX, RG>, lds, attr_done)) return AGP_E_LAUNCH;
    AGP_LAUNCH((igemm_kxrw_kernel<POOL, MIX, RG>), dim3(MIX ? k.blocks : k.half_bid0), dim3(256), lds, s, g);
    AGP_CHECK_LAUNCH();
    return AGP_OK;
}

}

int agp_internal_conv_kxrw(agp_igemm::IgemmParams* ps, int n, hipStream_t s, agp_igemm::TilePlan* plan) {
    using namespace agp_igemm;
    if (n < 1 || n > KXRW_MAXP || ps[0].N % 128) return AGP_E_BADARG;
    constexpr int bm = KwShape<2, 4>::BM, bn = KwShape<2, 4>::BN;
    KxrwGroup g = {};
    g.nprob = n;
    int mt = 0;
    bool pool = false;
    for (int i = 0; i < n; ++i) {
        if (ps[i].N != ps[0].N || ps[i].CK != ps[0].CK) return AGP_E_BADARG;
        g.p[i] = ps[i];
        mt += (ps[i].M + bm - 1) / bm;
        g.mt_end[i] = mt;
        pool = pool || ps[i].pool_partial != nullptr;
        const int64_t rb = (int64_t)(ps[i].M / (int)ps[i].d_howo.d) * ps[i].o_sn * 2;
        if (ps[i].r_hi && (rb <= 0 || rb > (int64_t)KXRW_ROOB)) return AGP_E_BADARG;
        g.r_bytes[i] = (uint32_t)rb;
    }
    g.MT = mt;
    g.NT = ps[0].N / bn;
    const KxrwPlan k = kxrw_plan(g.MT, g.NT);
    if (plan) {
        *plan = TilePlan{AGP_CONV_KERNEL_KXRW, bm, bn, g.MT, g.NT, k.MT_full, k.half_tiles, k.blocks};
        return AGP_OK;
    }
    const bool mix = k.mix;
    g.MT_full = k.MT_full;
    g.mt_chunk = k.mt_chunk;
    g.half_bid0 = k.half_bid0;
    g.rflag = agp_range_flag_get();
    return agp_rg_dispatch(g.rflag, [&](auto rg) {
        constexpr bool RG = decltype(rg)::value;
        if (mix) return pool ? launch_kxrw<true, true, RG>(g, k, s) : launch_kxrw<false, true, RG>(g, k, s);
        return pool ? launch_kxrw<true, false, RG>(g, k, s) : launch_kxrw<false, false, RG>(g, k, s);
    });
}
```

### agplace_amd/csrc/igemm_params.hpp

```cpp
#pragma once
#include "common.hpp"

namespace agp_igemm {

enum { EPI_CONV = 0, EPI_GMIN = 1 };

struct IgemmParams {
    const void* x_hi; const void* x_lo; uint32_t x_bytes;
    const void* w_hi; const void* w_lo; uint32_t w_bytes;
    int M, N, Ktot;
    int KW, CK, ntaps;
    FastDiv d_howo, d_wo;
    int x_sn, x_sh, x_sw, x_base, sy, sx;
    void* o_hi; void* o_lo;
    int o_sn, o_sh, o_sw, o_base;
    const void* r_hi; const void* r_lo;
    const float* scale; const float* shift;
    int relu;
    float* gmin; const float* wnorm; int gq_stride;
    const int* xrow_tab;
    int tap_stride, tab_mul;
    const void* w2_hi; const float* scale2; const float* shift2; void* o2_hi;
    const int64_t* m_dev;
    const int* row_perm;
    const uint32_t* tile_taps;
    int pool_h1, pool_w1, pool_h2, pool_w2, pool_ty, pool_tx;
    float* stat_partial;
    const void* bs_z_hi; const void* bs_z_lo; const void* bs_y_hi; const float* bs_mean; const float* bs_rstd;
    float* pool_partial; const float* pool_p; float pool_eps;
    int pool_sq;
    int img_rows;
    const void* w_cm;
    const void* w2_cm;
    const void* w_cm_lo;
    const void* w_q8; int w_q8_exp;
    int dbg;
    int MT, NT, mt_chunk;
};

struct StemRaw {
    const void* x;
    long long sn, sc, sh, sw;
    int h, w, ncam, wcam;
    float m[3], s[3];
    uint32_t bytes;
};

template <int NPREC> struct PrecT {
    static constexpr int XPL = (NPREC == 3) ? 2 : 1;
    static constexpr int WPL = (NPREC == 3 || NPREC == 2) ? 2 : 1;
    static constexpr int NPROD = (NPREC == 3) ? 3 : (NPREC == 2 ? 2 : 1);
    static constexpr bool F16 = (NPREC == 2 || NPREC == 4);
};

template <int NPREC>
__device__ __forceinline__ void mfma32(f32x16& acc, const bf16x8& wh, const bf16x8& wl, const bf16x8& xh,
                                       const bf16x8& xl) {
    if (NPREC == 3) {
        acc = __builtin_amdgcn_mfma_f32_32x32x16_bf16(wl, xh, acc, 0, 0, 0);
        acc = __builtin_amdgcn_mfma_f32_32x32x16_bf16(wh, xl, acc, 0, 0, 0);
        acc = __builtin_amdgcn_mfma_f32_32x32x16_bf16(wh, xh, acc, 0, 0, 0);
    } else if (NPREC == 1) {
        acc = __builtin_amdgcn_mfma_f32_32x32x16_bf16(wh, xh, acc, 0, 0, 0);
    } else {
        const f16x8 x = __builtin_bit_cast(f16x8, xh);
        if (NPREC == 2)
            acc = __builtin_amdgcn_mfma_f32_32x32x16_f16(__builtin_bit_cast(f16x8, wl), x, acc, 0, 0, 0);
        acc = __builtin_amdgcn_mfma_f32_32x32x16_f16(__builtin_bit_cast(f16x8, wh), x, acc, 0, 0, 0);
    }
}
template <int NPREC>
__device__ __forceinline__ void mfma16(f32x4& acc, const bf16x8& wh, const bf16x8& wl, const bf16x8& xh,
                                       const bf16x8& xl) {
    if (NPREC == 3) {
        acc = __builtin_amdgcn_mfma_f32_16x16x32_bf16(wl, xh, acc, 0, 0, 0);
        acc = __builtin_amdgcn_mfma_f32_16x16x32_bf16(wh, xl, acc, 0, 0, 0);
        acc = __builtin_amdgcn_mfma_f32_16x16x32_bf16(wh, xh, acc, 0, 0, 0);
    } else if (NPREC == 1) {
        acc = __builtin_amdgcn_mfma_f32_16x16x32_bf16(wh, xh, acc, 0, 0, 0);
    } else {
        const f16x8 x = __builtin_bit_cast(f16x8, xh);
        if (NPREC == 2)
            acc = __builtin_amdgcn_mfma_f32_16x16x32_f16(__builtin_bit_cast(f16x8, wl), x, acc, 0, 0, 0);
        acc = __builtin_amdgcn_mfma_f32_16x16x32_f16(__builtin_bit_cast(f16x8, wh), x, acc, 0, 0, 0);
    }
}

__device__ __forceinline__ int swz32(int row) { return (row >> 2) & 3; }

template <int N> __device__ __forceinline__ void wait_vm_lgkm() {
    if constexpr (N == 0) asm volatile("s_waitcnt vmcnt(0) lgkmcnt(0)" ::: "memory");
    else if constexpr (N == 1) asm volatile("s_waitcnt vmcnt(1) lgkmcnt(0)" ::: "memory");
    else if constexpr (N == 2) asm volatile("s_waitcnt vmcnt(2) lgkmcnt(0)" ::: "memory");
    else if constexpr (N == 4) asm volatile("s_waitcnt vmcnt(4) lgkmcnt(0)" ::: "memory");
    else if constexpr (N == 5) asm volatile("s_waitcnt vmcnt(5) lgkmcnt(0)" ::: "memory");
    else if constexpr (N == 6) asm volatile("s_waitcnt vmcnt(6) lgkmcnt(0)" ::: "memory");
    else if constexpr (N == 7) asm volatile("s_waitcnt vmcnt(7) lgkmcnt(0)" ::: "memory");
    else if constexpr (N == 8) asm volatile("s_waitcnt vmcnt(8) lgkmcnt(0)" ::: "memory");
    else static_assert(N < 0, "add the count");
}

__device__ __forceinline__ int group_problem(int& mt, int nprob, int e0, int e1, int e2) {
    int pid = 0, base = 0;
    if (nprob > 1 && mt >= e0) { pid = 1; base = e0; }
    if (nprob > 2 && mt >= e1) { pid = 2; base = e1; }
    if (nprob > 3 && mt >= e2) { pid = 3; base = e2; }
    mt -= base;
    return pid;
}

constexpr int EPI_ROWB = 64 * 4 + 16;

struct TilePlan {
    int32_t kernel, BM, BN, MT, NT, MT_full, half_tiles, grid;
};

struct XcdGrid {
    int MT, NT, mt_chunk, blocks;
};
inline XcdGrid xcd_grid(int MT, int NT) {
    const int mt_chunk = (MT + 7) / 8;
    return XcdGrid{MT, NT, mt_chunk, mt_chunk * 8 * NT};
}
inline int plan_xcd(TilePlan* plan, int kernel, int BM, int BN, const XcdGrid& x) {
    *plan = TilePlan{kernel, BM, BN, x.MT, x.NT, x.MT, 0, x.blocks};
    return AGP_OK;
}

}
```

### agplace_amd/csrc/igemm_s2.hip

```cpp

#include <type_traits>

#include "igemm_params.hpp"

namespace agp_igemm {

constexpr int S2_MAXP = 2;
struct S2Group {
    IgemmParams p[S2_MAXP];
    int mt_end[S2_MAXP];
    int nprob, MT, NT, mt_chunk;
};

constexpr int S2_BM = 128, S2_ROWB = 64;
constexpr int S2_BMX = S2_BM + 16;
constexpr int S2_XBLK = S2_BMX * S2_ROWB;
constexpr int S2_XBUF = 2 * S2_XBLK;
template <int TN> constexpr int s2_lds() {
    return 2 * S2_XBUF + 4 * (32 * TN * S2_ROWB) + 4 * (32 * TN) * 4;
}

template <int TN, class... RF>
__global__ void __launch_bounds__(256, TN == 2 ? 3 : 2) igemm_s2_kernel(S2Group g, RF... rf) {
#if defined(__HIP_DEVICE_COMPILE__)
    constexpr bool RG = sizeof...(RF) != 0;
    constexpr int BM = S2_BM, BN = 32 * TN, NW = 4, ROWB = S2_ROWB;
    constexpr int S2_WTAP = BN * S2_ROWB;
    constexpr int NWP = TN / 2;
    constexpr int XINS = 2 * (S2_BMX / 16);
    constexpr int NX = (XINS + NW - 1) / NW;
    static_assert(NX == 5, "the vmcnt counts below are written for NX = 5");
    extern __shared__ __attribute__((aligned(16))) char smem[];
    char* const ws = smem + 2 * S2_XBUF;
    float* const tab = (float*)(ws + 4 * S2_WTAP);

    const int tid = threadIdx.x;
    const int lane = tid & 63;
    const int wave = __builtin_amdgcn_readfirstlane(tid >> 6);

    const int bid = blockIdx.x;
    const int xcd = bid & 7, j = bid >> 3;
    const int gNT = g.NT, gchunk = g.mt_chunk, gMT = g.MT, gnprob = g.nprob;
    const int e0 = g.mt_end[0];
    const int nt = j % gNT;
    int mt = xcd * gchunk + j / gNT;
    if (mt >= gMT) return;
    int pid = 0;
    if (gnprob > 1 && mt >= e0) { pid = 1; mt -= e0; }
    const IgemmParams& p = g.p[pid];
    const int m0 = mt * BM, n0 = nt * BN;

    const FastDiv d_howo = p.d_howo, d_wo = p.d_wo;
    const int pM = p.M, pN = p.N, pKtot = p.Ktot;
    const int x_sn = p.x_sn, x_sh_ = p.x_sh, x_sw = p.x_sw, x_base = p.x_base;
    const int o_sn = p.o_sn, o_sw = p.o_sw, o_base = p.o_base;
    const bool has_ds = p.w2_hi != nullptr;

    const int lrow = lane >> 2, lpos = lane & 3;
    const int cpix = p.CK * 2;
    int xoff[NX];
#pragma unroll
    for (int q = 0; q < NX; ++q) {
        int ins = wave + NW * q;
        ins = ins < XINS ? ins : XINS - 1;
        const int blk = ins >= XINS / 2 ? 1 : 0;
        const int row = (ins - blk * (XINS / 2)) * 16 + lrow;
        const int m = m0 + row;
        const uint32_t img = fdiv((uint32_t)m, d_howo);
        const uint32_t rem = (uint32_t)m - img * d_howo.d;
        const uint32_t y = fdiv(rem, d_wo);
        const uint32_t xq = rem - y * d_wo.d;
        const int el = (int)img * x_sn + (int)y * x_sh_ + (int)xq * x_sw + x_base;
        xoff[q] = el * 2 + blk * cpix + ((lpos ^ swz32(row)) << 4);
    }
    int woff_c[NWP], woff_d[NWP];
#pragma unroll
    for (int i = 0; i < NWP; ++i) {
        const int row = (wave + NW * i) * 16 + lrow;
        const int n = (n0 + row) < pN ? (n0 + row) : pN - 1;
        const int wsw = (lpos ^ swz32(row)) << 4;
        woff_c[i] = (p.w_cm ? n * 64 : n * pKtot * 2) + wsw;
        woff_d[i] = (p.w2_cm ? n * 64 : n * p.CK * 2) + wsw;
    }
    const __amdgpu_buffer_rsrc_t rx = __builtin_amdgcn_make_buffer_rsrc((void*)p.x_hi, 0, p.x_bytes, 0x00020000);
    const __amdgpu_buffer_rsrc_t rw = __builtin_amdgcn_make_buffer_rsrc((void*)(p.w_cm ? p.w_cm : p.w_hi), 0, p.w_bytes, 0x00020000);
    const __amdgpu_buffer_rsrc_t rd = __builtin_amdgcn_make_buffer_rsrc((void*)(has_ds ? (p.w2_cm ? p.w2_cm : p.w2_hi) : (p.w_cm ? p.w_cm : p.w_hi)), 0,
                                                                        has_ds ? (uint32_t)(pN * p.CK * 2) : p.w_bytes, 0x00020000);

    const int CK = __builtin_amdgcn_readfirstlane(p.CK);
    const int in_row = __builtin_amdgcn_readfirstlane(p.sy);
    const int cchunks = CK / 32;
    const int nsteps = 3 * cchunks;
    const int tapb = CK * 2;
    float tab_v[4] = {1.f, 0.f, 1.f, 0.f};
    if (tid < BN) {
        const int n = n0 + tid < pN ? n0 + tid : pN - 1;
        if (p.scale) tab_v[0] = p.scale[n];
        if (p.shift) tab_v[1] = p.shift[n];
        if (has_ds && p.scale2) tab_v[2] = p.scale2[n];
        if (has_ds && p.shift2) tab_v[3] = p.shift2[n];
    }
    auto load_x = [&](int buf, int ky_, int cc_) {
        const int xs = __builtin_amdgcn_readfirstlane((ky_ * in_row + cc_ * 32) * 2);
        char* base = smem + buf * S2_XBUF;
#pragma unroll
        for (int q = 0; q < NX; ++q) {
            int ins = wave + NW * q;
            ins = ins < XINS ? ins : XINS - 1;
            __builtin_amdgcn_raw_ptr_buffer_load_lds(rx, LDS_PTR(base + ins * 1024), 16, xoff[q], xs, 0, 0);
        }
    };
    const int wmul = __builtin_amdgcn_readfirstlane(p.w_cm ? pN : 1), dmul = __builtin_amdgcn_readfirstlane(p.w2_cm ? pN : 1);
    auto load_w = [&](int slot, int wbytes) {
        const int so = __builtin_amdgcn_readfirstlane(wbytes * wmul);
#pragma unroll
        for (int i = 0; i < NWP; ++i)
            __builtin_amdgcn_raw_ptr_buffer_load_lds(rw, LDS_PTR(ws + slot * S2_WTAP + (wave + NW * i) * 1024), 16, woff_c[i], so, 0, 0);
    };
    load_x(0, 0, 0);
    load_w(0, 0);
    load_w(1, tapb);

    const int l31 = lane & 31, lh = lane >> 5;
    int xrd[3][2];
#pragma unroll
    for (int kx = 0; kx < 3; ++kx)
#pragma unroll
        for (int ks = 0; ks < 2; ++ks) {
            const int r = wave * 32 + l31 + (kx == 2 ? 1 : 0);
            xrd[kx][ks] = (kx == 1 ? S2_XBLK : 0) + r * ROWB + (((2 * ks + lh) ^ swz32(r)) << 4);
        }
    int wrd[2];
    {
        const int wrow = (l31 & 0x13) | ((l31 & 4) << 1) | ((l31 & 8) >> 1);
#pragma unroll
        for (int ks = 0; ks < 2; ++ks) wrd[ks] = wrow * ROWB + (((2 * ks + lh) ^ swz32(wrow)) << 4);
    }

    f32x16 acc[TN], acc2[TN];
#pragma unroll
    for (int a = 0; a < TN; ++a)
#pragma unroll
        for (int r = 0; r < 16; ++r) { acc[a][r] = 0.f; acc2[a][r] = 0.f; }

    constexpr int LPP = BN / 8, PPI = 64 / LPP, NEI = 32 / PPI;
    int eoff[NEI];
    {
        const uint32_t wlast = d_wo.d - 1;
        const int img_extra = o_sn - (int)d_howo.d * o_sw;
#pragma unroll
        for (int q = 0; q < NEI; ++q) {
            const int m = m0 + wave * 32 + q * PPI + lane / LPP;
            const uint32_t mm = (uint32_t)(m < pM ? m : pM - 1);
            const uint32_t img = fdiv(mm, d_howo);
            const uint32_t rem = mm - img * d_howo.d;
            const uint32_t y = fdiv(rem, d_wo);
            const uint32_t xq = rem - y * d_wo.d;
            const bool ok = (m < pM) && xq != 0 && xq != wlast;
            eoff[q] = ok ? (int)mm * o_sw + (int)img * img_extra + o_base + n0 + 8 * (lane % LPP) : -1;
        }
    }

    int ky = 0, cc = 0;
    wait_vm_lgkm<NWP>();
    __builtin_amdgcn_s_barrier();
    if (tid < BN) { tab[tid] = tab_v[0]; tab[BN + tid] = tab_v[1]; tab[2 * BN + tid] = tab_v[2]; tab[3 * BN + tid] = tab_v[3]; }
    auto phase = [&](auto KX, auto LAST, const char* xb, int st_, int ky_, int nky_, int ncc_, int wcur_, int wnext_) {
        constexpr int kx = decltype(KX)::value;
        constexpr bool last = decltype(LAST)::value;
        const char* wb = ws + kx * S2_WTAP;
        bf16x8 xf[2], wf[2][TN];
#pragma unroll
        for (int ks = 0; ks < 2; ++ks) {
            xf[ks] = *(const bf16x8*)(xb + xrd[kx][ks]);
#pragma unroll
            for (int t = 0; t < TN; ++t) wf[ks][t] = *(const bf16x8*)(wb + wrd[ks] + t * (32 * ROWB));
        }
        constexpr int ndma = kx == 0 ? (last ? NWP : NWP + NX) : (last ? 0 : (kx == 2 ? 2 * NWP : NWP));
        auto piece = [&](int i) {
            if (kx == 0) {
                if (i < NWP) {
                    const int so = __builtin_amdgcn_readfirstlane((wcur_ + 2 * tapb) * wmul);
                    __builtin_amdgcn_raw_ptr_buffer_load_lds(rw, LDS_PTR(ws + 2 * S2_WTAP + (wave + NW * i) * 1024), 16, woff_c[i], so, 0, 0);
                } else {
                    const int q = i - NWP;
                    const int xs = __builtin_amdgcn_readfirstlane((nky_ * in_row + ncc_ * 32) * 2);
                    int ins = wave + NW * q;
                    ins = ins < XINS ? ins : XINS - 1;
                    __builtin_amdgcn_raw_ptr_buffer_load_lds(rx, LDS_PTR(smem + ((st_ + 1) & 1) * S2_XBUF + ins * 1024), 16, xoff[q], xs, 0, 0);
                }
            } else if (i < NWP) {
                const int so = __builtin_amdgcn_readfirstlane((wnext_ + (kx - 1) * tapb) * wmul);
                __builtin_amdgcn_raw_ptr_buffer_load_lds(rw, LDS_PTR(ws + (kx - 1) * S2_WTAP + (wave + NW * i) * 1024), 16, woff_c[i], so, 0, 0);
            } else {
                const int so = __builtin_amdgcn_readfirstlane((nky_ == 1 ? ncc_ : 0) * 64 * dmul);
                const int k = i - NWP;
                __builtin_amdgcn_raw_ptr_buffer_load_lds(rd, LDS_PTR(ws + 3 * S2_WTAP + (wave + NW * k) * 1024), 16,
                                                         has_ds ? woff_d[k] : woff_c[k], has_ds ? so : 0, 0, 0);
            }
        };
        int ip = 0;
#pragma unroll
        for (int ks = 0; ks < 2; ++ks)
#pragma unroll
            for (int tn = 0; tn < TN; ++tn) {
                acc[tn] = __builtin_amdgcn_mfma_f32_32x32x16_f16(__builtin_bit_cast(f16x8, wf[ks][tn]), __builtin_bit_cast(f16x8, xf[ks]),
                                                                 acc[tn], 0, 0, 0);
                if (ip < ndma) { piece(ip); ++ip; }
            }
#pragma unroll
        for (int i = 2 * TN; i < ndma; ++i) piece(i);
        __builtin_amdgcn_sched_group_barrier(0x100, 2 * (1 + TN), 0);
#pragma unroll
        for (int i = 0; i < 2 * TN; ++i) {
            __builtin_amdgcn_sched_group_barrier(0x008, 1, 0);
            if (i < ndma) __builtin_amdgcn_sched_group_barrier(0x010, 1, 0);
        }
        __builtin_amdgcn_sched_barrier(0);
        if (kx == 1 && ky_ == 1 && has_ds) {
            const char* db = ws + 3 * S2_WTAP;
            bf16x8 df[2][TN];
#pragma unroll
            for (int ks = 0; ks < 2; ++ks)
#pragma unroll
                for (int t = 0; t < TN; ++t) df[ks][t] = *(const bf16x8*)(db + wrd[ks] + t * (32 * ROWB));
#pragma unroll
            for (int ks = 0; ks < 2; ++ks)
#pragma unroll
                for (int tn = 0; tn < TN; ++tn)
                    acc2[tn] = __builtin_amdgcn_mfma_f32_32x32x16_f16(__builtin_bit_cast(f16x8, df[ks][tn]),
                                                                      __builtin_bit_cast(f16x8, xf[ks]), acc2[tn], 0, 0, 0);
        }
    };
    using I0 = std::integral_constant<int, 0>; using I1 = std::integral_constant<int, 1>; using I2 = std::integral_constant<int, 2>;
    for (int st = 0; st < nsteps - 1; ++st) {
        int nky = ky, ncc = cc + 1;
        if (ncc == cchunks) { ncc = 0; ++nky; }
        const int wcur = (ky * 3 * CK + cc * 32) * 2, wnext = (nky * 3 * CK + ncc * 32) * 2;
        const char* xb = smem + (st & 1) * S2_XBUF;
        phase(I0{}, std::false_type{}, xb, st, ky, nky, ncc, wcur, wnext);
        wait_vm_lgkm<NX + NWP>();
        __builtin_amdgcn_s_barrier();
        phase(I1{}, std::false_type{}, xb, st, ky, nky, ncc, wcur, wnext);
        wait_vm_lgkm<NX + NWP>();
        __builtin_amdgcn_s_barrier();
        phase(I2{}, std::false_type{}, xb, st, ky, nky, ncc, wcur, wnext);
        wait_vm_lgkm<2 * NWP>();
        __builtin_amdgcn_s_barrier();
        ky = nky; cc = ncc;
    }
    {
        const int st = nsteps - 1;
        const int wcur = (ky * 3 * CK + cc * 32) * 2;
        const char* xb = smem + (st & 1) * S2_XBUF;
        phase(I0{}, std::true_type{}, xb, st, ky, 0, 0, wcur, 0);
        wait_vm_lgkm<NWP>();
        __builtin_amdgcn_s_barrier();
        phase(I1{}, std::true_type{}, xb, st, ky, 0, 0, wcur, 0);
        wait_vm_lgkm<0>();
        __builtin_amdgcn_s_barrier();
        phase(I2{}, std::true_type{}, xb, st, ky, 0, 0, wcur, 0);
    }

    asm volatile("s_waitcnt lgkmcnt(0)" ::: "memory");
    __builtin_amdgcn_s_barrier();
    constexpr int ERS = 2 * BN + 16;
    char* const strip = smem + wave * (32 * ERS);
    const int a_off = l31 * ERS + lh * 16;
    const int l_off = (lane / LPP) * ERS + (lane % LPP) * 16;
    RangeTrack<RG> rg;
    auto epilogue = [&](const f32x16* a, const float* tb0, bf16_t* out, float relu_lo, bool sym) {
        const float* tb = tb0 + 8 * lh;
        u32x4 outv[TN * 2];
#pragma unroll
        for (int jj = 0; jj < TN * 2; ++jj) {
            const f32x4 s0 = *(const f32x4*)(tb + 16 * jj), s1 = *(const f32x4*)(tb + 16 * jj + 4);
            const f32x4 h0 = *(const f32x4*)(tb + BN + 16 * jj), h1 = *(const f32x4*)(tb + BN + 16 * jj + 4);
            float v[8];
#pragma unroll
            for (int e = 0; e < 8; ++e) v[e] = a[jj >> 1][8 * (jj & 1) + e] * (e < 4 ? s0[e & 3] : s1[e & 3]) + (e < 4 ? h0[e & 3] : h1[e & 3]);
            if (sym) rg.sym8(v);
            else rg.any8(v);
            outv[jj] = pack8_h_lo(v, relu_lo);
        }
#pragma unroll
        for (int jj = 0; jj < TN * 2; ++jj) *(u32x4*)(strip + a_off + jj * 32) = outv[jj];
        __builtin_amdgcn_fence(__ATOMIC_RELEASE, "wavefront");
        u32x4 lines[NEI];
#pragma unroll
        for (int i = 0; i < NEI; ++i) lines[i] = *(const u32x4*)(strip + l_off + i * (PPI * ERS));
#pragma unroll
        for (int i = 0; i < NEI; ++i)
            if (eoff[i] >= 0) *(u32x4*)(out + eoff[i]) = lines[i];
        __builtin_amdgcn_fence(__ATOMIC_RELEASE, "wavefront");
    };
    epilogue(acc, tab, (bf16_t*)p.o_hi, p.relu ? 0.f : -65504.f, false);
    if (has_ds) epilogue(acc2, tab + 2 * BN, (bf16_t*)p.o2_hi, -65504.f, true);
    rg.flush(rg_word(rf...), p.relu ? 0.f : -65504.f);
#endif
}

}

int agp_internal_conv_s2(agp_igemm::IgemmParams* ps, const agp_conv_desc* descs, int n, hipStream_t s, agp_igemm::TilePlan* plan) {
    using namespace agp_igemm;
    if (n < 1 || n > S2_MAXP) return AGP_E_BADARG;
    S2Group g = {};
    g.nprob = n;
    int mt = 0;
    for (int i = 0; i < n; ++i) {
        const agp_conv_desc* d = descs + i;
        IgemmParams& p = ps[i];
        if (p.N != ps[0].N || p.CK != ps[0].CK) return AGP_E_BADARG;
        const int wpo = d->wout + 2, wpi = d->win + 2, hpi = d->hin + 2;
        p.M = d->n * d->hout * wpo;
        p.d_howo = make_fastdiv((uint32_t)(d->hout * wpo));
        p.d_wo = make_fastdiv((uint32_t)wpo);
        p.x_sw = 2 * d->cin; p.x_sh = 2 * wpi * d->cin; p.x_sn = hpi * wpi * d->cin;
        p.sy = wpi * d->cin;
        p.x_base = -2 * d->cin;
        p.o_sw = d->cout; p.o_sh = wpo * d->cout; p.o_sn = (d->hout + 2) * wpo * d->cout;
        p.o_base = wpo * d->cout;
        mt += (p.M + S2_BM - 1) / S2_BM;
        g.mt_end[i] = mt;
        g.p[i] = p;
    }
    g.MT = mt;
    g.mt_chunk = (g.MT + 7) / 8;
    const int wide = AGP_TUNE("S2_WIDE", 1);
    auto launch = [&](auto kern, int lds, std::atomic<uint64_t>& attr, auto... rf) -> int {
        if (!agp_lds_attr((const void*)kern, lds, attr)) return AGP_E_LAUNCH;
        AGP_LAUNCH(kern, dim3(g.mt_chunk * 8 * g.NT), dim3(256), lds, s, g, rf...);
        return AGP_OK;
    };
    static std::atomic<uint64_t> a4s{0}, a2s{0}, a4g{0}, a2g{0};
    uint32_t* const rflag = agp_range_flag_get();
    const bool w4 = wide && ps[0].N % 128 == 0;
    g.NT = w4 ? ps[0].N / 128 : (ps[0].N + 63) / 64;
    if (plan) {
        *plan = TilePlan{AGP_CONV_KERNEL_S2, S2_BM, w4 ? 128 : 64, g.MT, g.NT, g.MT, 0, g.mt_chunk * 8 * g.NT};
        return AGP_OK;
    }
    int rc;
    if (rflag) rc = w4 ? launch(igemm_s2_kernel<4, uint32_t*>, s2_lds<4>(), a4g, rflag)
                       : launch(igemm_s2_kernel<2, uint32_t*>, s2_lds<2>(), a2g, rflag);
    else rc = w4 ? launch(igemm_s2_kernel<4>, s2_lds<4>(), a4s) : launch(igemm_s2_kernel<2>, s2_lds<2>(), a2s);
    if (rc != AGP_OK) return rc;
    AGP_CHECK_LAUNCH();
    return AGP_OK;
}
```

### agplace_amd/ops.py

```python
import ctypes as C
import math
import os

import torch

from . import _lib
from ._lib import ptr, check

GEM_EPS = 1e-6
CONV_PROFILE = None
LO_FP8 = True
CHUNK_MAJOR_TRAIN = True
USE_W_CM = True


def _L():
    return _lib.load()


def _need_cuda(t, what):
    if not t.is_cuda:
        raise RuntimeError(f"{what}: tensor must live on the GPU (agplace_amd has no CPU path)")


# ... 461 lines not shown
        if pool is not None and x.lo is None and out.lo is None and int(_L().agp_conv2d_pool_blocks(C.byref(d))) > 0:
            d.pool_partial = 1
    if len(jobs) == 1:
        if stat_partial:
            arr[0].stat_partial = 1
        if hi_only:
            arr[0].hi_only = 1
        return tile_plan(arr[0])
    return tile_plan(arr)


class PoolReq:
    __slots__ = ("p", "eps", "want_mean", "want_gem", "mean", "gem", "fused", "_partial", "gem_out", "exp")

    def __init__(self, p=None, eps=GEM_EPS, want_mean=True, want_gem=False, gem_out=None):
        if want_gem and p is None:
            raise ValueError("PoolReq: GeM needs its exponent tensor p")
        self.p = None if p is None else p.detach()
        self.eps, self.want_mean, self.want_gem = eps, want_mean, want_gem
        self.mean = self.gem = self._partial = None
        self.gem_out = gem_out
        self.fused = False
        self.exp = 0

    @property
    def scale(self):
        t = self.mean if self.mean is not None else self.gem
        return pow2_scalar(t.device, self.exp)

    def true_mean(self):
        return scale_pow2(self.mean, self.exp)

    def true_gem(self):
        return scale_pow2(self.gem, self.exp)

    def attach(self, d, x, cw, out, prec):
        self.fused = False
        self.exp = out.exp
        if x.lo is None and out.lo is None:
            blocks = int(_L().agp_conv2d_pool_blocks(C.byref(d)))
            if blocks > 0:
                self._partial = torch.empty(blocks * 2 * cw.cout, dtype=torch.float32, device=out.hi.device)
                d.pool_partial = ptr(self._partial)
                d.pool_p = ptr(self.p) if self.want_gem else None
                d.pool_eps = math.ldexp(self.eps, -self.exp)
                self.fused = True

    def finish(self, out):
        go = self.gem_out
        if go is not None and (tuple(go.shape) != (out.n, out.c) or go.dtype != torch.float32 or not go.is_contiguous()):
            go = None
        self.exp = out.exp
        if not self.fused:
            self.mean, self.gem = pool_map(out, self.p, want_mean=self.want_mean, want_gem=self.want_gem, eps=self.eps, gem_out=go,
                                           raw=True)
            return
        dev = out.hi.device
        self.mean = torch.empty((out.n, out.c), dtype=torch.float32, device=dev) if self.want_mean else None
        self.gem = (go if go is not None else torch.empty((out.n, out.c), dtype=torch.float32, device=dev)) if self.want_gem else None
        check(_L().agp_pool_from_conv(ptr(self._partial), out.n, out.h, out.w, out.c, ptr(self.p) if self.want_gem else None,
                                      ptr(self.mean), ptr(self.gem), _lib.stream()), "agp_pool_from_conv")


class SqStatReq:
    __slots__ = ("fused", "partial", "blocks")

    def __init__(self):
        self.fused, self.partial, self.blocks = False, None, 0

    def attach(self, d, x, cw, out, prec):
        self.fused = False
        if x.lo is None and out.lo is None:
            blocks = int(_L().agp_conv2d_pool_blocks(C.byref(d)))
            if blocks > 0:
                self.partial = torch.empty(blocks * 2 * cw.cout, dtype=torch.float32, device=out.hi.device)
                d.pool_partial = ptr(self.partial)
                d.pool_stat = 1
                self.blocks = out.n * ((out.h * (out.w + 2) + 63) // 64)
                assert self.blocks <= blocks
                self.fused = True

    def finish(self, out):
        pass


def _fill_conv_desc(d, x, cw, out, residual, relu, prec, stat_partial=None, bstat=None):
    d.in_hi, d.in_lo = ptr(x.hi), ptr(x.lo)
    w_hi, w_lo = cw.planes(prec)
    d.w_hi, d.w_lo = ptr(w_hi), ptr(w_lo)
    d.out_hi, d.out_lo = ptr(out.hi), ptr(out.lo)
    d.res_hi = ptr(residual.hi) if residual is not None else None
    d.res_lo = ptr(residual.lo) if residual is not None else None
    d.scale, d.shift = ptr(cw.scale), ptr(cw.shift)
    d.n, d.hin, d.win, d.pin = x.n, x.h, x.w, x.pad
    d.cin = cw.cin
    d.in_w_step = cw.in_w_step_stem or cw.cin
    d.hout, d.wout, d.cout, d.pout = out.h, out.w, cw.cout, out.pad
    d.kh, d.kw, d.stride, d.pad = cw.kh, cw.kw, cw.stride, cw.pad
    d.relu = 1 if relu else 0
    d.prec = prec
    if stat_partial is not None:
        d.stat_partial = ptr(stat_partial)
        if bstat is not None:
            bz, by, bmean, brstd = bstat
            d.bstat_z_hi, d.bstat_z_lo = ptr(bz.hi), ptr(bz.lo)
            d.bstat_y_hi = ptr(by.hi) if by is not None else None
            d.bstat_mean, d.bstat_rstd = ptr(bmean), ptr(brstd)
    if not USE_W_CM and not getattr(cw, "_train_cm", False):
        pass
    elif prec == _lib.PREC_F16:
        d.w_cm = ptr(cw.cm())
    elif prec in (_lib.PREC_F16W2, _lib.PREC_BF16X3):
        if getattr(cw, "_train_cm", False):
            d.w_cm, d.w_cm_lo = d.w_hi, d.w_lo
        else:
            c2 = cw.cm2(prec)
            if c2 is not None:
                d.w_cm, d.w_cm_lo = ptr(c2[0]), ptr(c2[1])
    if LO_FP8 and prec == _lib.PREC_F16W2:
        q = cw.q8()
        if q is not None:
            d.w_q8, d.w_q8_exp = ptr(q[0]), q[1]
    return d


def conv2d_grouped(jobs, prec):
    jobs = [tuple(j) + (None,) * (6 - len(j)) for j in jobs]
    if len(jobs) == 1:
        x, cw, out, residual, relu, pool = jobs[0]
        return [conv2d(x, cw, out, residual=residual, relu=relu, prec=prec, pool=pool)]
    arr = (_lib.ConvDesc * len(jobs))()
    keep = []
    for d, (x, cw, out, residual, relu, pool) in zip(arr, jobs):
        keep.append(cw.planes(prec))
        _fill_conv_desc(d, x, cw, out, residual, relu, prec)
        if pool is not None:
            pool.attach(d, x, cw, out, prec)
    e0 = e1 = None
    if CONV_PROFILE is not None:
        e0, e1 = torch.cuda.Event(enable_timing=True), torch.cuda.Event(enable_timing=True)
        e0.record()
    check(_L().agp_conv2d_fwd_grouped(arr, len(jobs), _lib.stream()), "agp_conv2d_fwd_grouped")
    if CONV_PROFILE is not None:
        e1.record()
        x, cw, out = jobs[0][:3]
        macs = sum(j[0].n * j[2].h * j[2].w * j[1].cout * j[1].alg_k for j in jobs)
        CONV_PROFILE.append((e0, e1, macs, (sum(j[0].n for j in jobs), out.h, out.w, cw.cin, cw.cout, cw.kh, cw.kw, cw.stride)))
    for j in jobs:
        if j[5] is not None:
            j[5].finish(j[2])
    return [j[2] for j in jobs]


def conv2d(x: SplitMap, cw: ConvWeights, out: SplitMap, residual: SplitMap = None, relu=False, prec=3, stat_partial=None, pool=None,
           bstat=None, hi_only=False):
    d = _fill_conv_desc(_lib.ConvDesc(), x, cw, out, residual, relu, prec, stat_partial, bstat)
    if hi_only:
        d.hi_only = 1
    if pool is not None:
        pool.attach(d, x, cw, out, prec)
    if CONV_PROFILE is not None:
        e0, e1 = torch.cuda.Event(enable_timing=True), torch.cuda.Event(enable_timing=True)
        e0.record()
        check(_L().agp_conv2d_fwd(C.byref(d), _lib.stream()), "agp_conv2d_fwd")
        e1.record()
        CONV_PROFILE.append((e0, e1, x.n * out.h * out.w * cw.cout * cw.alg_k,
                             (x.n, out.h, out.w, cw.cin, cw.cout, cw.kh, cw.kw, cw.stride)))
    else:
        check(_L().agp_conv2d_fwd(C.byref(d), _lib.stream()), "agp_conv2d_fwd")
    if pool is not None:
        pool.finish(out)
    return out


FUSED_BLOCK64 = True


def bblock64_ok(x: SplitMap, cw1: ConvWeights, cw2: ConvWeights, prec):
    if not FUSED_BLOCK64 or prec != _lib.PREC_F16 or x.lo is not None or x.pad != 1 or x.c != 64 or x.h % 2:
        return False
    for cw in (cw1, cw2):
        if (cw.cin, cw.cout, cw.kh, cw.kw, cw.stride, cw.pad) != (64, 64, 3, 3, 1, 1) or cw.in_w_step_stem or cw.w is None:
            return False
    return x.n * (x.h + 2) * (x.w + 2) * 128 < (1 << 31)


def bblock64_grouped(jobs, exact=False):
    jobs = [tuple(j) + (None,) * (5 - len(j)) for j in jobs]
    arr = (_lib.BBlock64Desc * len(jobs))()
    keep = []
    for d, (x, cw1, cw2, out, pool) in zip(arr, jobs):
        if (out.n, out.h, out.w, out.c, out.pad) != (x.n, x.h, x.w, 64, 1) or out.lo is not None:
            raise ValueError("bblock64: the output map must have the input's geometry (fp16, halo 1, 64 channels)")
        w1, w2 = cw1.planes(_lib.PREC_F16)[0], cw2.planes(_lib.PREC_F16)[0]
        keep.append((w1, w2))
        d.inp, d.out, d.w1, d.w2 = ptr(x.hi), ptr(out.hi), ptr(w1), ptr(w2)
        d.scale1, d.shift1, d.scale2, d.shift2 = ptr(cw1.scale), ptr(cw1.shift), ptr(cw2.scale), ptr(cw2.shift)
        d.n, d.h, d.w, d.form = x.n, x.h, x.w, 1 if exact else 0
        if pool is not None:
            if pool.want_gem:
                raise ValueError("bblock64: the fused block pools the mean only")
            nfl = int(_L().agp_bblock64_pool_floats(C.byref(d)))
            pool._partial = torch.empty(nfl, dtype=torch.float32, device=out.hi.device)
            d.pool_partial = ptr(pool._partial)
    e0 = e1 = None
    if CONV_PROFILE is not None:
        e0, e1 = torch.cuda.Event(enable_timing=True), torch.cuda.Event(enable_timing=True)
        e0.record()
    check(_L().agp_bblock64_fwd_grouped(arr, len(jobs), _lib.stream()), "agp_bblock64_fwd_grouped")
    if CONV_PROFILE is not None:
        e1.record()
        macs = sum(2 * j[0].n * j[0].h * j[0].w * 64 * 576 for j in jobs)
        x = jobs[0][0]
        CONV_PROFILE.append((e0, e1, macs, (sum(j[0].n for j in jobs), x.h, x.w, 64, 64, 3, 3, 1, "bblock64")))
    for x, cw1, cw2, out, pool in jobs:
        if pool is not None:
            pool.fused = True
            pool.mean = torch.empty((out.n, 64), dtype=torch.float32, device=out.hi.device)
            pool.gem = None
            pool.exp = out.exp
            check(_L().agp_bblock64_pool_finish(ptr(pool._partial), out.n, out.h, out.w, ptr(pool.mean), _lib.stream()),
                  "agp_bblock64_pool_finish")
    return [j[3] for j in jobs]


def stem_pool(x: SplitMap, cw: ConvWeights, out: SplitMap, prec=2):
    d = _lib.ConvDesc()
    d.in_hi, d.in_lo = ptr(x.hi), ptr(x.lo)
    w_hi, w_lo = cw.planes(prec)
    d.w_hi, d.w_lo = ptr(w_hi), ptr(w_lo)
    d.out_hi, d.out_lo = ptr(out.hi), ptr(out.lo)
    d.res_hi = d.res_lo = None
    d.scale, d.shift = ptr(cw.scale), ptr(cw.shift)
    d.n, d.hin, d.win, d.pin = x.n, x.h, x.w, x.pad
    d.cin, d.in_w_step = cw.cin, cw.in_w_step_stem
    d.hout, d.wout, d.cout, d.pout = out.h, out.w, cw.cout, out.pad
    d.kh, d.kw, d.stride, d.pad = cw.kh, cw.kw, cw.stride, cw.pad
    d.relu, d.prec = 1, prec
    check(_L().agp_stem_pool_fwd(C.byref(d), _lib.stream()), "agp_stem_pool_fwd")
    return out


def stem_walk_reads(x):
    if torch.is_tensor(x) and x.dtype == torch.uint8 and x.dim() == 5 and x.shape[-1] == 3:
        n, ncam, h, wcam, _ = x.shape
        return x.is_contiguous() and wcam % 32 == 0 and x.data_ptr() % 16 == 0 and n * ncam * h * wcam * 3 < (1 << 31)
    if not torch.is_tensor(x) or x.dtype != torch.float32 or x.dim() != 4 or x.shape[1] != 3:
        return False
    sn, sc, sh, sw = x.stride()
    n, _, h, w = x.shape
    if sw != 1 or sn % 4 or sc % 4 or sh % 4 or w % 4 or x.data_ptr() % 16 or min(sn, sc, sh) < 0:
        return False
    return ((n - 1) * sn + 2 * sc + (h - 1) * sh + w) * 4 < (1 << 31)


def stem_pool_raw(x, cw: ConvWeights, out: SplitMap, mean=IMAGENET_MEAN, std=IMAGENET_STD):
    _need_cuda(x, "stem_pool_raw")
    d = _lib.ConvDesc()
    w_hi, _ = cw.planes(4)
    d.w_hi, d.w_lo = ptr(w_hi), None
    d.out_hi, d.out_lo = ptr(out.hi), None
    d.res_hi = d.res_lo = None
    d.in_lo = None
    d.scale, d.shift = ptr(cw.scale), ptr(cw.shift)
    m = (C.c_float * 3)(*mean)
    sd = (C.c_float * 3)(*std)
    if x.dtype == torch.uint8:
        if x.dim() != 5 or x.shape[-1] != 3:
            raise ValueError("stem_pool_raw expects uint8 [n, ncam, h, wcam, 3]")
        x = x.contiguous()
        n, ncam, h, wcam, _ = x.shape
        kind, w, st = 2, ncam * wcam, (0, 0, 0, 0)
    else:
        if x.dtype != torch.float32 or x.dim() != 4 or x.shape[1] != 3:
            raise ValueError("stem_pool_raw expects fp32 [n, 3, h, w]")
        n, _, h, w = x.shape
        kind, ncam, st = 1, 1, tuple(x.stride())
    d.in_hi = ptr(x)
    d.n, d.hin, d.win, d.pin = n, h, w, 3
    d.cin, d.in_w_step = cw.cin, cw.in_w_step_stem
    d.hout, d.wout, d.cout, d.pout = out.h, out.w, cw.cout, out.pad
    d.kh, d.kw, d.stride, d.pad = cw.kh, cw.kw, cw.stride, cw.pad
    d.relu, d.prec = 1, 4
    check(_L().agp_stem_pool_raw_fwd(C.byref(d), kind, st[0], st[1], st[2], st[3], ncam, m, sd, _lib.stream()),
          "agp_stem_pool_raw_fwd")
    return out


def conv_out_size(h, k, stride, pad):
    return (h + 2 * pad - k) // stride + 1


def maxpool3x3s2(x: SplitMap, out: SplitMap, argmax=None):
    check(_L().agp_maxpool3x3s2_fwd(ptr(x.hi), ptr(x.lo), x.n, x.h, x.w, x.c, x.pad, ptr(out.hi),
                                    ptr(out.lo), out.h, out.w, out.pad, ptr(argmax), _lib.stream()),
          "agp_maxpool3x3s2_fwd")
    return out


def bcast_add(x: SplitMap, vec, out: SplitMap):
    if tuple(vec.shape) != (x.n, x.c) or vec.device != x.hi.device:
        raise RuntimeError(f"bcast_add: vector of shape {tuple(vec.shape)} on {vec.device} for a map [{x.n}, {x.c}, ...] on {x.hi.device}")
    vec = vec.contiguous().float()
    check(_L().agp_bcast_add_fwd(ptr(x.hi), ptr(x.lo), ptr(vec), x.n, x.h, x.w, x.c, x.pad,
                                 ptr(out.hi), ptr(out.lo), out.pad, _lib.stream()), "agp_bcast_add_fwd")
    out.exp = x.exp
# ... 344 lines not shown
```

### agplace_amd/resnet.py

```python
import math

import os

import torch
import torch.nn as nn

from . import ops, train_graph

ARCH = {
    "resnet18": ("basic", [2, 2, 2, 2]),
    "resnet34": ("basic", [3, 4, 6, 3]),
    "resnet50": ("bottleneck", [3, 4, 6, 3]),
}
PLANES = [64, 128, 256, 512]


def _conv(cin, cout, k, stride, pad):
    m = nn.Conv2d(cin, cout, k, stride, pad, bias=False)
    nn.init.kaiming_normal_(m.weight, mode="fan_out", nonlinearity="relu")
    return m


class _Block(nn.Module):
    def __init__(self, kind, inplanes, planes, stride):
        super().__init__()
        self.kind, self.stride = kind, stride
        exp = 1 if kind == "basic" else 4
        if kind == "basic":
            self.conv1 = _conv(inplanes, planes, 3, stride, 1)
            self.bn1 = nn.BatchNorm2d(planes)
            self.conv2 = _conv(planes, planes, 3, 1, 1)
            self.bn2 = nn.BatchNorm2d(planes)
        else:
            self.conv1 = _conv(inplanes, planes, 1, 1, 0)
            self.bn1 = nn.BatchNorm2d(planes)
            self.conv2 = _conv(planes, planes, 3, stride, 1)
            self.bn2 = nn.BatchNorm2d(planes)
            self.conv3 = _conv(planes, planes * exp, 1, 1, 0)
            self.bn3 = nn.BatchNorm2d(planes * exp)
        self.relu = nn.ReLU(inplace=True)
        self.downsample = None
        if stride != 1 or inplanes != planes * exp:
            self.downsample = nn.Sequential(_conv(inplanes, planes * exp, 1, stride, 0),
                                            nn.BatchNorm2d(planes * exp))
        self.out_planes = planes * exp

    def convs(self):
        seq = [(self.conv1, self.bn1), (self.conv2, self.bn2)]
        if self.kind == "bottleneck":
            seq.append((self.conv3, self.bn3))
        ds = (self.downsample[0], self.downsample[1]) if self.downsample is not None else None
        return seq, ds


FUSE_STEM_POOL = True


class ResNet(nn.Module):

    def __init__(self, fe_type, nstages=4):
        super().__init__()
        kind, layers = ARCH[fe_type]
        self.fe_type, self.kind, self.nstages = fe_type, kind, nstages
        self.conv1 = _conv(3, 64, 7, 2, 3)
        self.bn1 = nn.BatchNorm2d(64)
        self.relu = nn.ReLU(inplace=True)
        self.maxpool = nn.MaxPool2d(3, 2, 1)
        inplanes = 64
        exp = 1 if kind == "basic" else 4
        for li in range(4):
            if li < nstages:
                blocks = []
                for bi in range(layers[li]):
                    stride = 2 if (li > 0 and bi == 0) else 1
                    blk = _Block(kind, inplanes, PLANES[li], stride)
                    inplanes = blk.out_planes
                    blocks.append(blk)
                setattr(self, f"layer{li + 1}", nn.Sequential(*blocks))
            else:
                setattr(self, f"layer{li + 1}", nn.Identity())
        self.avgpool = nn.AdaptiveAvgPool2d((1, 1))
        self.fc = nn.Linear(512 * exp, 1000)
        self.fc.requires_grad_(False)
        self._prep = {}
        self._prep_key = None
        self._ws = ops.Workspace()
        self._map_exp = {}

    def _version_key(self):
        return tuple((p.data_ptr(), p._version) for p in self.parameters()) + \
            tuple((b.data_ptr(), b._version) for b in self.buffers()) + tuple(sorted(self._map_exp.items()))

    def map_exponent_names(self):
        groups, internal = {}, []
        for li in range(self.nstages):
            mem = ["stem"] if li == 0 else []
            for bi, blk in enumerate(getattr(self, f"layer{li + 1}")):
                seq, ds = blk.convs()
                if ds:
                    mem.append(f"layer{li + 1}.{bi}.downsample")
                internal += [f"layer{li + 1}.{bi}.conv{ci + 1}" for ci in range(len(seq) - 1)]
                mem.append(f"layer{li + 1}.{bi}.out")
            groups[f"layer{li + 1}"] = mem
        return groups, internal

    def _prepared(self, scaled=False):
        key = self._version_key()
        if key != self._prep_key:
            self._prep, self._prep_key = {}, key
        scaled = bool(scaled) and any(self._map_exp.values())
        if scaled in self._prep:
            return self._prep[scaled]
        prep = {}
        mexp = prep["exp"] = {}

        def E(name):
            return int(self._map_exp.get(name, 0)) if scaled else 0

        def fold(conv, bn, e_in, e_out, stem=False):
            s, t = ops.fold_exp(*ops.fold_bn(bn.weight, bn.bias, bn.running_mean, bn.running_var, bn.eps), e_in, e_out)
            return ops.ConvWeights(conv.weight, s, t, conv.stride[0], conv.padding[0], stem=stem)

        mexp["stem"] = E("layer1")
        prep["stem"] = fold(self.conv1, self.bn1, 0, mexp["stem"], stem=True)
        for li in range(self.nstages):
            g_out = E(f"layer{li + 1}")
            for bi, blk in enumerate(getattr(self, f"layer{li + 1}")):
                seq, ds = blk.convs()
                g_in = E(f"layer{li}") if (bi == 0 and li > 0) else g_out
                cws, e_prev = [], g_in
                for ci, (c, b) in enumerate(seq):
                    e_o = g_out if ci == len(seq) - 1 else E(f"layer{li + 1}.{bi}.conv{ci + 1}")
                    cws.append(fold(c, b, e_prev, e_o))
                    mexp[(li, bi, ci)] = e_prev = e_o
                mexp[("ds", li, bi)] = g_out
                prep[(li, bi)] = (cws, fold(*ds, g_in, g_out) if ds else None)
        self._prep[scaled] = prep
        return prep

    @staticmethod
    def _input_geometry(x):
        if isinstance(x, ops.SplitMap):
            return x.n, x.h, x.w, x.hi.device
        if isinstance(x, ops.RawFrames):
            return x.shape[0], x.h, x.shape[1] * x.w, x.device
        if x.dtype == torch.uint8:
            n, ncam, h, w, _ = x.shape
            return n, h, ncam * w, x.device
        n, _, h, w = x.shape
        return n, h, w, x.device

    def _stem_input(self, x, tag, prec, lo=0, hi=None, h16=False):
        n, h, w, dev = self._input_geometry(x)
        hi = n if hi is None else hi
        if isinstance(x, ops.SplitMap):
            if x.c != 4 or x.pad != 3 or x.prec != (3 if prec == 3 else 2):
                raise ValueError("stem input map must be NHWC4 with halo 3 in the conv's storage format")
            return ops.slice_map(x, lo, hi)
        raw = isinstance(x, ops.RawFrames)
        want16 = h16 and prec == 3 and not raw and x.dtype != torch.uint8
        xin = ops.slice_map(self._ws.map(tag, n, h, w, 4, 3, prec, dev, h16=want16), lo, hi)
        if not want16 and xin.h16 is not None:
            xin = ops.SplitMap(xin.hi, xin.lo, xin.n, xin.h, xin.w, xin.c, xin.pad)
        if raw:
            ops.pack_cameras_resized_u8(x.frames[lo:hi], (x.h, x.w), prec, out=xin)
        elif x.dtype == torch.uint8:
            ops.pack_cameras_u8(x[lo:hi], prec, out=xin)
        else:
            xin = ops.pack_f32(x[lo:hi], 4, 3, prec, out=xin)
        return xin

    def forward_maps(self, x, prec=3, level_means=None, final_pool=None):
        return forward_maps_multi([self], [x], prec=prec, level_means=[level_means], final_pools=[final_pool])[0]

    def _unit(self, name, conv, bn, stem=False, pre="t."):
        u = self._units.get(pre + name)
        if u is None:
            u = train_graph.ConvBNUnit(conv, bn, pre + name, self._ws, stem=stem)
            self._units[pre + name] = u
        return u

    def forward_maps_train(self, x, prec=3, slot=0):
        if not hasattr(self, "_units"):
            self._units, self._tapes, self._tape_gens = {}, {}, {}
        self._tape_gens[slot] = self._tape_gens.get(slot, 0) + 1
        pre = "t." if slot == 0 else f"t{slot}."
        n, h, w, dev = self._input_geometry(x)
        ws = self._ws
        stem = self._unit("stem", self.conv1, self.bn1, stem=True, pre=pre)
        xin = self._stem_input(x, pre + "in", prec, h16=stem.wgrad_f16_ok(prec))
        c1 = self.conv1
        hs = ops.conv_out_size(xin.h, c1.kernel_size[0], c1.stride[0], c1.padding[0])
        wss = ops.conv_out_size(xin.w, c1.kernel_size[0], c1.stride[0], c1.padding[0])
        h2, w2 = ops.conv_out_size(hs, 3, 2, 1), ops.conv_out_size(wss, 3, 2, 1)
        pooled = ws.map(pre + "pool", n, h2, w2, 64, 1, prec, dev)
        argmax = ws.tensor(pre + "pool.argmax", (n, h2, w2, 64), torch.uint8, dev)
        blocks = []
        for li in range(self.nstages):
            for bi, blk in enumerate(getattr(self, f"layer{li + 1}")):
                seq, ds = blk.convs()
                units = [self._unit(f"l{li}.{bi}.c{ci}", c, b, pre=pre) for ci, (c, b) in enumerate(seq)]
                ud = self._unit(f"l{li}.{bi}.ds", ds[0], ds[1], pre=pre) if ds else None
                blocks.append((li, units, ud))
        stem.forward(xin, relu=True, prec=prec, pool=(pooled, argmax), out_h16=blocks[0][1][0].wgrad_f16_ok(prec))
        s = pooled
        cur, outs, tape = pooled, [], []
        for k, (li, units, ud) in enumerate(blocks):
            idt = ud.forward(cur, relu=False, prec=prec) if ud else cur
            t = cur
            for ci, u in enumerate(units):
                last = ci == len(units) - 1
                if not last:
                    want = units[ci + 1].wgrad_f16_ok(prec)
                elif k + 1 < len(blocks):
                    want = blocks[k + 1][1][0].wgrad_f16_ok(prec)
                else:
                    want = bool(getattr(self, "last_out_h16", False))
                only16 = (not last) and units[ci + 1].reads_f16_plane_only(prec)
                t = u.forward(t, residual=idt if last else None, relu=True, prec=prec, out_h16=want, out_f16_only=only16)
            tape.append((units, ud))
            cur = t
            if k + 1 == len(blocks) or blocks[k + 1][0] != li:
                outs.append(cur)
                tape.append(("stage_end", li))
        self._tapes[slot] = (tape, s, argmax, stem, prec, pre)
        return outs

    def tape_generation(self, slot=0):
        return getattr(self, "_tape_gens", {}).get(slot, 0)

    def backward_maps(self, stage_grads, slot=0):
        tape, s, argmax, stem, prec, pre = self._tapes[slot]
        ws, dev = self._ws, s.hi.device
        g, part = None, None
        rev = list(reversed(tape))
        for pos, item in enumerate(rev):
            if item[0] == "stage_end":
                sg = stage_grads[item[1]]
                if sg is not None:
                    if g is None:
                        g = sg
                    else:
                        acc = ws.map(f"{pre}gstage{item[1]}", g.n, g.h, g.w, g.c, 1, prec, dev)
                        g = train_graph.map_add(g, sg, acc)
                continue
            units, ud = item
            if g is None:
                continue
            prev_last = None
            if pos + 1 < len(rev):
                nxt = rev[pos + 1]
                if nxt[0] == "stage_end":
                    if stage_grads[nxt[1]] is None and pos + 2 < len(rev) and rev[pos + 2][0] != "stage_end":
                        prev_last = rev[pos + 2][0][-1]
                else:
                    prev_last = nxt[0][-1]
            gh, gres, (_, pnext) = units[-1].backward(g, partial=part, stats_for=units[-2] if len(units) > 1 else None)
            gx2 = None
            added = False
            for ci in range(len(units) - 2, -1, -1):
                if ci == 0:
                    gx2 = ud.backward(gres)[0] if ud is not None else gres
                    gh, _, (added, pnext) = units[0].backward(gh, partial=pnext, add=gx2, stats_for=prev_last)
                else:
                    gh, _, (_, pnext) = units[ci].backward(gh, partial=pnext, stats_for=units[ci - 1])
            if len(units) == 1:
                gx2 = ud.backward(gres)[0] if ud is not None else gres
                pnext = None
            if added:
                g, part = gh, pnext
            else:
                acc = ws.map(units[0].tag + ".gsum", gh.n, gh.h, gh.w, gh.c, 1, prec, dev)
                g, part = train_graph.map_add(gh, gx2, acc), None
        if g is not None:
            stem.backward(g, need_gx=False, pool_argmax=argmax, pooled=s)


STEM_READS_INPUT = "auto"
SATURATION_CHECK = True
STAGE1_CHUNK = 1 << 30


def forward_maps_multi(nets, xs, prec=3, level_means=None, final_pools=None):
    R = len(nets)
    level_means = level_means or [None] * R
    final_pools = final_pools or [None] * R
    stage_pool = [{} for _ in range(R)]
    a = nets[0]
    for b in nets[1:]:
        if (b.fe_type, b.nstages) != (a.fe_type, a.nstages):
            raise ValueError("forward_maps_multi: the trunks must share one architecture")
    preps = [net._prepared(scaled=prec != 3) for net in nets]
    geo = [net._input_geometry(x) for net, x in zip(nets, xs)]
    devs = [g[3] for g in geo]
    nchunks = max(1, -(-geo[0][0] // STAGE1_CHUNK))
    for r in range(R):
        for li in range(a.nstages):
            last_stage = li == a.nstages - 1
            if last_stage and final_pools[r] is not None:
                stage_pool[r][li] = final_pools[r]
            elif not last_stage and level_means[r] is not None:
                stage_pool[r][li] = ops.PoolReq(want_mean=True, want_gem=False)

    def run_stage(li, cur, lo, hi):
        act = [r for r in range(R) if hi[r] > lo[r]]
        nblocks = len(getattr(a, f"layer{li + 1}"))
        for bi in range(nblocks):
            blks = {r: getattr(nets[r], f"layer{li + 1}")[bi] for r in act}
            cws = {r: preps[r][(li, bi)] for r in act}
            idt = dict(cur)

            def view(r, tag, h_, w_, c_, e_):
                v = ops.slice_map(nets[r]._ws.map(tag, geo[r][0], h_, w_, c_, 1, prec, devs[r]), lo[r], hi[r])
                v.exp = e_
                return v
            mexp = {r: preps[r]["exp"] for r in act}
            lname = f"layer{li + 1}.{bi}"
            ds_jobs = []
            if cws[act[0]][1] is not None:
                for r in act:
                    dsw = cws[r][1]
                    ho = ops.conv_out_size(cur[r].h, 3, blks[r].stride, 1)
                    wo = ops.conv_out_size(cur[r].w, 3, blks[r].stride, 1)
                    idt[r] = view(r, f"ds{li}.{bi}", ho, wo, dsw.cout, mexp[r][("ds", li, bi)])
                    ds_jobs.append((cur[r], dsw, idt[r], None, False))
            t = dict(cur)
            nconv = len(cws[act[0]][0])
            if a.kind == "basic" and cws[act[0]][1] is None and len(act) <= 4 and \
                    all(ops.bblock64_ok(cur[r], cws[r][0][0], cws[r][0][1], prec) for r in act):
                jobs, pools = [], {}
                for r in act:
                    pool = stage_pool[r].get(li) if (bi == nblocks - 1 and (li > 0 or nchunks == 1)) else None
                    pools[r] = pool
                    out_ = view(r, f"c{li}.{bi}.1", cur[r].h, cur[r].w, 64, mexp[r][(li, bi, 1)])
                    jobs.append((cur[r], cws[r][0][0], cws[r][0][1], out_, pool if (pool is not None and not pool.want_gem) else None))
                outs_ = ops.bblock64_grouped(jobs)
                for r, o in zip(act, outs_):
                    if pools[r] is not None and pools[r].want_gem:
                        pools[r].fused = False
                        pools[r].finish(o)
                cur = {r: o for r, o in zip(act, outs_)}
                if ops.MAP_PROBE is not None:
                    for r in act:
                        ops.probe_map(nets[r], f"{lname}.out", cur[r])
                continue
            for ci in range(nconv):
                last = ci == nconv - 1
                jobs = []
                for r in act:
                    cw = cws[r][0][ci]
                    oh = ops.conv_out_size(t[r].h, cw.kh, cw.stride, cw.pad)
                    ow = ops.conv_out_size(t[r].w, cw.kw, cw.stride, cw.pad)
                    pool = stage_pool[r].get(li) if (last and bi == nblocks - 1 and (li > 0 or nchunks == 1)) else None
                    jobs.append((t[r], cw, view(r, f"c{li}.{bi}.{ci}", oh, ow, cw.cout, mexp[r][(li, bi, ci)]), idt[r] if last else None,
                                 True, pool))
                if ci == 0 and ds_jobs:
                    if len(jobs) + len(ds_jobs) <= 4 and not (cws[act[0]][0][0].kh == 3 and cws[act[0]][0][0].stride == 1):
                        outs_ = ops.conv2d_grouped(jobs + ds_jobs, prec)[:len(jobs)]
                    else:
                        ops.conv2d_grouped(ds_jobs, prec)
                        outs_ = ops.conv2d_grouped(jobs, prec)
                else:
                    outs_ = ops.conv2d_grouped(jobs, prec)
                t = {r: o for r, o in zip(act, outs_)}
                if ops.MAP_PROBE is not None:
                    for r in act:
                        ops.probe_map(nets[r], f"{lname}.out" if last else f"{lname}.conv{ci + 1}", t[r])
                        if ci == 0 and ds_jobs:
                            ops.probe_map(nets[r], f"{lname}.downsample", idt[r])
            cur = t
        return cur

    stage1_tags = None
    for k in range(nchunks):
        lo = [(g[0] * k) // nchunks for g in geo]
        hi = [(g[0] * (k + 1)) // nchunks for g in geo]
        cur = {}
        for r, (net, x, prep) in enumerate(zip(nets, xs, preps)):
            if hi[r] <= lo[r]:
                continue
            n, h, w, dev = geo[r]
            ws = net._ws
            h1, w1 = ops.conv_out_size(h, 7, 2, 3), ops.conv_out_size(w, 7, 2, 3)
            h2, w2 = ops.conv_out_size(h1, 3, 2, 1), ops.conv_out_size(w1, 3, 2, 1)
            c = ops.slice_map(ws.map("pool", n, h2, w2, 64, 1, prec, dev), lo[r], hi[r])
            c.exp = prep["exp"]["stem"]
            if prec == 4 and FUSE_STEM_POOL and STEM_READS_INPUT != "0" and not isinstance(x, (ops.SplitMap, ops.RawFrames)) and (
                    STEM_READS_INPUT == "1" or ops.stem_walk_reads(x[lo[r]:hi[r]])):
                ops.stem_pool_raw(x[lo[r]:hi[r]], prep["stem"], c)
                cur[r] = c
                continue
            xin = net._stem_input(x, "in", prec, lo[r], hi[r])
            if prec != 3 and FUSE_STEM_POOL:
                ops.stem_pool(xin, prep["stem"], c, prec=prec)
            else:
                s_ = ops.slice_map(ws.map("stem", n, h1, w1, 64, 1, prec, dev), lo[r], hi[r])
                ops.conv2d(xin, prep["stem"], s_, relu=True, prec=prec)
                ops.maxpool3x3s2(s_, c)
            cur[r] = c
        for r in cur:
            ops.probe_map(nets[r], "stem", cur[r])
        last_views = run_stage(0, cur, lo, hi)
        if stage1_tags is None:
            stage1_tags = {r: (v.h, v.w, v.c) for r, v in last_views.items()}
        else:
            stage1_tags.update({r: (v.h, v.w, v.c) for r, v in last_views.items()})
    nb0 = len(a.layer1)
    nc0 = len(preps[0][(0, nb0 - 1)][0])
    cur = {r: nets[r]._ws.map(f"c0.{nb0 - 1}.{nc0 - 1}", geo[r][0], *stage1_tags[r], 1, prec, devs[r]) for r in range(R)}
    for r in range(R):
        cur[r].exp = preps[r]["exp"][(0, nb0 - 1, nc0 - 1)]
    outs = [[] for _ in nets]
    zero, full = [0] * R, [g[0] for g in geo]
    for li in range(a.nstages):
        if li > 0:
            cur = run_stage(li, cur, zero, full)
        for r in range(R):
            outs[r].append(cur[r])
            req = stage_pool[r].get(li)
            if req is not None:
                if req.mean is None and req.gem is None:
                    req.fused = False
                    req.finish(cur[r])
                if li < a.nstages - 1:
                    level_means[r].append(req.mean)
    if SATURATION_CHECK and prec != 3:
        for r, net in enumerate(nets):
            if net.__dict__.get("_sat_checked") != net._prep_key and not torch.cuda.is_current_stream_capturing():
                net.__dict__["_sat_checked"] = net._prep_key
                nsat = sum(ops.count_saturated(m) for m in outs[r])
                net.__dict__["_sat_count"] = nsat
                if nsat:
                    import warnings
                    warnings.warn(f"agplace_amd: {nsat} feature-map elements of a {net.fe_type} trunk sit at the fp16 limit (+-65504): "
                                  f"these weights / inputs leave fp16's range in precision mode {prec}; calibrate map exponents "
                                  "(agplace_amd.map_exponents.calibrate) or run this model with Options.mfma_precision = 3 "
                                  "(split-bf16 maps)")
    return outs
```

### include/agplace_hip.h

```cpp
#ifndef AGPLACE_HIP_H
#define AGPLACE_HIP_H

#include <stdint.h>

#ifdef __cplusplus
extern "C" {
#endif

#define AGP_OK 0
#define AGP_E_BADARG 1
#define AGP_E_LAUNCH 2
#define AGP_E_UNSUPPORTED 3

#define AGP_PREC_BF16 1
#define AGP_PREC_F16W2 2
#define AGP_PREC_BF16X3 3
#define AGP_PREC_F16 4

#define AGP_FMT_BF16 0
#define AGP_FMT_F16 1

#define AGP_ACT_ID 0
#define AGP_ACT_RELU 1
#define AGP_ACT_TANH 2
#define AGP_ACT_SIGMOID 3

#define AGP_ODE_EULER 0
#define AGP_ODE_MIDPOINT 1
#define AGP_ODE_RK4 2
#define AGP_ODE_DOPRI5 3
#define AGP_ODE_OK 0
#define AGP_ODE_E_MAXSTEPS 1
#define AGP_ODE_E_UNDERFLOW 2
#define AGP_ODE_E_NAN 3
#define AGP_ODE_MAX_STEPS_LIMIT 4096

const char* agp_version(void);
const char* agp_arch(void);


uint32_t* agp_range_flag_set(uint32_t* word);
uint32_t* agp_range_flag_get(void);


int agp_split_f32(const float* x, void* hi, void* lo, int64_t n, int fmt, void* stream);
int agp_split_conv_weight(const float* w, int cout, int cin, int kh, int kw, int dgrad, void* hi, void* lo, void* stream);
int agp_split_conv_weight_both(const float* w, int cout, int cin, int kh, int kw, void* hi, void* lo, void* hi_d, void* lo_d,
                               int chunk_major, void* stream);

int agp_pack_f32_to_nhwc(const float* x, int64_t sn, int64_t sc, int64_t sh, int64_t sw,
                         int n, int c, int h, int w, int cpad, int pad,
                         void* hi, void* lo, void* stream);
int agp_pack_f32_to_nhwc4_h16(const float* x, int64_t sn, int64_t sc, int64_t sh, int64_t sw, int n, int c, int h, int w, int pad,
                              void* hi, void* lo, void* h16, void* stream);

int agp_pack_u8_cams_to_nhwc(const uint8_t* img, int n, int ncam, int h, int w, const float* mean3,
                             const float* std3, int pad, void* hi, void* lo, void* stream);

int agp_resize_ksize(int in, int out);
int agp_resize_coeffs(int in, int out, int32_t* k, int32_t* bounds);
int agp_resized_size(int h, int w, int size, int* oh, int* ow);
int agp_resize_u8_cams(const uint8_t* frames, int n, int ncam, int H0, int W0, int h, int w, const int32_t* kx,
                       const int32_t* bx, const int32_t* ky, const int32_t* by, uint8_t* out, void* stream);
int agp_resize_pack_u8_cams(const uint8_t* frames, int n, int ncam, int H0, int W0, int h, int w, const int32_t* kx,
                            const int32_t* bx, const int32_t* ky, const int32_t* by, const float* mean3,
                            const float* std3, int pad, void* hi, void* lo, void* stream);

int agp_unpack_nhwc_to_f32(const void* hi, const void* lo, int n, int h, int w, int c,
                           int pad, float* out, void* stream);

int agp_map_zero_halo(void* hi, void* lo, int n, int h, int w, int c, int pad, void* stream);

int agp_map_absmax(const void* hi, const void* lo, int n, int h, int w, int c, int pad, float* inout_max, void* stream);
int agp_map_absmax_reset(float* words, int n, void* stream);


typedef struct agp_conv_desc {
    const void* in_hi;  const void* in_lo;
    const void* w_hi;   const void* w_lo;
    void* out_hi;       void* out_lo;
    const void* res_hi; const void* res_lo;
    const float* scale; const float* shift;
    int32_t n, hin, win, cin, pin, in_w_step;
    int32_t hout, wout, cout, pout;
    int32_t kh, kw, stride, pad;
    int32_t relu;
    int32_t prec;
    const void* w_q8;
    int32_t w_q8_exp;
    float* stat_partial;
    float* pool_partial;
    const float* pool_p;
    float pool_eps;
    int32_t hi_only;
    const void* w_cm;
    const void* bstat_z_hi; const void* bstat_z_lo;
    const void* bstat_y_hi;
    const float* bstat_mean; const float* bstat_rstd;
    const void* w_cm_lo;
    const void* in_h16;
    uint32_t* out_absmax;
    int32_t pool_stat;
    int32_t reserved0;
} agp_conv_desc;
int agp_conv2d_fwd(const agp_conv_desc* d, void* stream);

int agp_conv2d_fwd_grouped(const agp_conv_desc* descs, int n, void* stream);

#define AGP_CONV_KERNEL_GENERIC 1
#define AGP_CONV_KERNEL_DIRECT_X 2
#define AGP_CONV_KERNEL_KXR 3
#define AGP_CONV_KERNEL_KXR2 4
#define AGP_CONV_KERNEL_KXRW 5
#define AGP_CONV_KERNEL_S2 6
int agp_conv2d_tile_plan(const agp_conv_desc* descs, int n, int32_t plan[8]);

int agp_conv2d_stat_tiles(const agp_conv_desc* d);

int agp_conv2d_pool_blocks(const agp_conv_desc* d);
int agp_pool_from_conv(const float* partial, int n, int h, int w, int c, const float* p, float* mean_out,
                       float* gem_out, void* stream);

typedef struct agp_bblock64_desc {
    const void* in; void* out;
    const void* w1; const void* w2;
    const float* scale1; const float* shift1;
    const float* scale2; const float* shift2;
    float* pool_partial;
    int32_t n, h, w, form;
} agp_bblock64_desc;
int agp_bblock64_fwd_grouped(const agp_bblock64_desc* descs, int n, void* stream);
int64_t agp_bblock64_pool_floats(const agp_bblock64_desc* d);
int agp_bblock64_pool_finish(const float* partial, int n, int h, int w, float* mean_out, void* stream);

int agp_conv_w_q8_prepare(const float* w, int cout, int cin, void* q8, int32_t* exp_host, void* stream);

int agp_stem_pool_fwd(const agp_conv_desc* d, void* stream);
int agp_stem_pool_raw_fwd(const agp_conv_desc* d, int kind, int64_t sn, int64_t sc, int64_t sh, int64_t sw, int ncam,
                          const float* mean3, const float* std3, void* stream);

int agp_maxpool3x3s2_fwd(const void* in_hi, const void* in_lo, int n, int hin, int win, int c,
                         int pin, void* out_hi, void* out_lo, int hout, int wout, int pout,
                         uint8_t* argmax, void* stream);

int agp_bcast_add_fwd(const void* in_hi, const void* in_lo, const float* vec, int n, int h,
                      int w, int c, int pin, void* out_hi, void* out_lo, int pout, void* stream);


int64_t agp_pool_workspace_floats(int n, int c, int h, int w);
int agp_pool_fwd(const void* hi, const void* lo, int n, int h, int w, int c, int pad,
                 const float* p, float eps, float* mean_out, float* gem_out, float* partial,
                 void* stream);
int agp_pool_f32_fwd(const float* x, int64_t sn, int64_t sc, int64_t sh, int64_t sw, int n,
                     int c, int h, int w, const float* p, float eps, float* mean_out,
                     float* gem_out, float* partial, void* stream);
#define AGP_GP_FLOATS (1 + 16384 + 1)
int agp_gem_f32_bwd(const float* x, int64_t sn, int64_t sc, int64_t sh, int64_t sw, int n,
                    int c, int h, int w, const float* p, float eps, const float* y,
                    const float* gy, float* gx, float* gp, void* stream);


int agp_linear_fwd(const float* x, const float* add1, const float* add2, const void* w_hi,
                   const void* w_lo, const float* bias, int b, int k, int n, int act,
                   float* y, void* stream);

int64_t agp_fcode_traj_floats(int b, int method, int nsteps);
int agp_fcode_fwd(const float* x, const float* add1, const float* add2, const void* w_hi,
                  const void* w_lo, const float* bias, int b, int act, int method,
                  const float* dt, int nsteps, float* y, float* traj, void* stream);

int64_t agp_fcode_bwd_workspace_bytes(int b, int method, int nsteps);
int agp_fcode_bwd(const float* traj, const float* gy, const void* wt_hi, const void* wt_lo, int b,
                  int act, int method, const float* dt, int nsteps, float* gx, float* gw, float* gb,
                  void* workspace, int64_t workspace_bytes, void* stream);

typedef struct agp_ode_stats {
    int32_t status;
    int32_t accepted;
    int32_t rejected;
    int32_t f_evals;
    double t0, t1;
} agp_ode_stats;
int64_t agp_fcode_adaptive_ctrl_bytes(int max_steps);
int64_t agp_fcode_adaptive_ring_floats(int b, int max_steps, int want_traj);
int agp_fcode_adaptive_fwd(const float* x, const float* add1, const float* add2, const void* w_hi, const void* w_lo,
                           const float* bias, int b, int act, int method, double rtol, double atol, int max_steps,
                           float* y, float* ring, int want_traj, void* ctrl, void* stream);

int64_t agp_fcode_adaptive_bwd_workspace_bytes(int b, int max_steps);
int agp_fcode_adaptive_bwd(const float* traj, const void* ctrl, const float* gy, const void* wt_hi, const void* wt_lo,
                           int b, int act, int method, int max_steps, float* gx, float* gw, float* gb, void* workspace,
                           int64_t workspace_bytes, void* stream);

int64_t agp_linear_bwd_workspace_bytes(int b, int k, int n);
int agp_linear_bwd(const float* x, const float* y, const float* gy, const void* wt_hi,
                   const void* wt_lo, int b, int k, int n, int act, float* gx, float* gw, float* gb,
                   void* workspace, int64_t workspace_bytes, void* stream);

int agp_layernorm_bwd(const float* x, const float* gamma, const float* y, const float* gy, int b, int d,
                      float eps, int relu, float* gx, float* gres, float* ggamma, float* gbeta,
                      void* stream);
int agp_l2normalize_bwd(const float* x, const float* gy, int b, int d, float* gx, void* stream);

int agp_layernorm_fwd(const float* x, const float* gamma, const float* beta, const float* res,
                      int b, int d, float eps, int relu, float* y, void* stream);
int agp_l2normalize_fwd(const float* x, int b, int d, float* y, void* stream);

int agp_wsum_fwd(const float* x0, const float* x1, const float* x2, const float* x3,
                 const float* x4, const float* x5, const float* w0, const float* w1,
                 const float* w2, const float* w3, const float* w4, const float* w5, int64_t n,
                 float* y, void* stream);
int agp_dot_f32(const float* a, const float* b, int64_t n, float* out, void* stream);

#define AGP_VECPROG_MAXOPS 36
#define AGP_VECPROG_NREG 6
#define AGP_VP_LOAD 1
#define AGP_VP_STORE 2
#define AGP_VP_LINEAR 3
#define AGP_VP_FCODE 4
#define AGP_VP_L2NORM 5
#define AGP_VP_LAYERNORM 6
#define AGP_VP_WSUM 7
typedef struct agp_vecprog_op {
    int op, dst, r[6], k, act, aux, n;
    float f0;
    int pad;
    const void* p[6];
} agp_vecprog_op;
int agp_vecprog_run(const agp_vecprog_op* ops, int nops, int b, int ode_method, const float* ode_dt, int ode_nsteps,
                    void* stream);
int agp_vecprog_run2(const agp_vecprog_op* ops_a, int nops_a, int b_a, const agp_vecprog_op* ops_b, int nops_b, int b_b,
                     int ode_method, const float* ode_dt, int ode_nsteps, void* stream);


int agp_upsample2_zero(const void* g_hi, const void* g_lo, int n, int ho, int wo, int c, int gpad,
                       void* u_hi, void* u_lo, int hu, int wu, int upad, void* stream);

int64_t agp_train_reduce_workspace_floats(int n, int h, int w, int c);
int agp_bn_stats(const void* z_hi, const void* z_lo, int n, int h, int w, int c, int pad, float eps,
                 float momentum, float* mean, float* rstd, float* running_mean, float* running_var,
                 const float* gamma, const float* beta, float* scale, float* shift, float* workspace,
                 void* stream);
int agp_bn_stats_from_partial(const float* partial, int tiles, int c, int64_t count, float eps, float momentum,
                              float* mean, float* rstd, float* running_mean, float* running_var,
                              const float* gamma, const float* beta, float* scale, float* shift, void* stream);
int agp_map_affine(const void* a_hi, const void* a_lo, const float* scale, const float* shift,
                   const void* r_hi, const void* r_lo, int n, int h, int w, int c, int pad, int relu,
                   void* o_hi, void* o_lo, void* o_h16, void* stream);
int agp_bn_bwd(const void* z_hi, const void* z_lo, const void* gy_hi, const void* gy_lo, const void* y_hi,
               const void* y_lo, const float* mean, const float* rstd, const float* gamma, int n, int h,
               int w, int c, int pad, int relu, void* gz_hi, void* gz_lo, void* gres_hi, void* gres_lo,
               float* ggamma, float* gbeta, float* workspace, uint32_t* gz_absmax, void* stream);
int agp_bn_bwd_from_partial(const float* partial, int tiles, const void* z_hi, const void* z_lo, const void* gy_hi,
                            const void* gy_lo, const void* y_hi, const void* y_lo, const float* mean, const float* rstd,
                            const float* gamma, int n, int h, int w, int c, int pad, int relu, int frozen, void* gz_hi,
                            void* gz_lo, void* gres_hi, void* gres_lo, float* ggamma, float* gbeta, uint32_t* gz_absmax,
                            void* stream);
int agp_bn_sums(const void* z_hi, const void* z_lo, int n, int h, int w, int c, int pad, double* sums,
                float* workspace, void* stream);
int agp_bn_sums_from_partial(const float* partial, int tiles, int c, int64_t count, double* sums,
// ... 145 lines not shown
```

Baseline: 41830 pairs/s.

## Fuse 1x1 stride-2 downsample conv into the second 3x3 conv of transition blocks

In ResNet transition basic blocks, the 1x1 stride-2 downsample conv plus its BN is folded into extra K-steps of the second 3x3 conv's implicit GEMM. Its strided input and pre-scaled weights are streamed as a second operand pair, and the BN shifts are summed. This removes the separate downsample launch and the write and re-read of the residual map. The cost is a more complex kernel epilogue schedule, a new s2 path without the downsample, and fp16 rounding of the scale-folded 1x1 weights.

```diff
diff --git a/agplace_amd/_lib.py b/agplace_amd/_lib.py
--- a/agplace_amd/_lib.py
+++ b/agplace_amd/_lib.py
@@ -47,6 +47,11 @@
     ]
 
 
+class ConvStream2(C.Structure):
+    _fields_ = [("in_hi", C.c_void_p), ("w_cm", C.c_void_p),
+                ("n", C.c_int32), ("hin", C.c_int32), ("win", C.c_int32), ("cin", C.c_int32)]
+
+
 class BBlock64Desc(C.Structure):
     _fields_ = [("inp", C.c_void_p), ("out", C.c_void_p), ("w1", C.c_void_p), ("w2", C.c_void_p),
                 ("scale1", C.c_void_p), ("shift1", C.c_void_p), ("scale2", C.c_void_p), ("shift2", C.c_void_p),
@@ -85,6 +90,8 @@
     "agp_map_absmax_reset": (_I, [_P, _I, _P]),
     "agp_conv2d_fwd": (_I, [C.POINTER(ConvDesc), _P]),
     "agp_conv2d_fwd_grouped": (_I, [C.POINTER(ConvDesc), _I, _P]),
+    "agp_conv2d_s2_fwd": (_I, [C.POINTER(ConvDesc), _I, _P]),
+    "agp_conv2d_fwd_grouped2": (_I, [C.POINTER(ConvDesc), C.POINTER(ConvStream2), _I, _P]),
     "agp_bblock64_fwd_grouped": (_I, [C.POINTER(BBlock64Desc), _I, _P]),
     "agp_bblock64_pool_floats": (_L, [C.POINTER(BBlock64Desc)]),
     "agp_bblock64_pool_finish": (_I, [_P, _I, _I, _I, _P, _P]),
diff --git a/agplace_amd/csrc/igemm.hip b/agplace_amd/csrc/igemm.hip
--- a/agplace_amd/csrc/igemm.hip
+++ b/agplace_amd/csrc/igemm.hip
@@ -555,7 +555,8 @@
 void agp_internal_conv_kxr_geometry(agp_igemm::IgemmParams& p, const agp_conv_desc* d);
 bool agp_internal_use_kxr2(const agp_conv_desc* d);
 int agp_internal_conv_kxr2(agp_igemm::IgemmParams* ps, int n, hipStream_t s, agp_igemm::TilePlan* plan);
-int agp_internal_conv_s2(agp_igemm::IgemmParams* ps, const agp_conv_desc* descs, int n, hipStream_t s, agp_igemm::TilePlan* plan);
+int agp_internal_conv_s2(agp_igemm::IgemmParams* ps, const agp_conv_desc* descs, int n, hipStream_t s, agp_igemm::TilePlan* plan, bool nods);
+int agp_internal_conv_kxrw(agp_igemm::IgemmParams* ps, int n, hipStream_t s, agp_igemm::TilePlan* plan, const agp_igemm::KxrwStreams* ds);
 
 static int conv2d_fwd_one(const agp_conv_desc* d, void* stream, TilePlan* plan);
 
@@ -595,7 +596,7 @@
                 const agp_conv_desc* d = descs + h + i;
                 ps[i].w2_hi = d->w_hi; ps[i].w2_cm = d->w_cm; ps[i].scale2 = d->scale; ps[i].shift2 = d->shift; ps[i].o2_hi = d->out_hi;
             }
-            return agp_internal_conv_s2(ps, descs, h, (hipStream_t)stream, plan);
+            return agp_internal_conv_s2(ps, descs, h, (hipStream_t)stream, plan, false);
         }
     }
     if (!group) {
@@ -637,6 +638,68 @@
 }
 
 extern "C" int agp_conv2d_fwd(const agp_conv_desc* d, void* stream) { return conv2d_fwd_one(d, stream, nullptr); }
+
+static bool s2_conv_ok(const agp_conv_desc* c, const agp_conv_desc* d0) {
+    return c->prec == AGP_PREC_F16 && c->in_hi && c->w_hi && c->out_hi && !c->in_lo && !c->w_lo && !c->out_lo && !c->res_hi && !c->res_lo &&
+           !c->stat_partial && !c->pool_partial && !c->hi_only &&
+           c->kh == 3 && c->kw == 3 && c->stride == 2 && c->pad == 1 && c->pin == 1 && c->pout == 1 && c->in_w_step == c->cin &&
+           c->hin > 0 && c->win > 0 && c->hout == (c->hin - 1) / 2 + 1 && c->wout == (c->win - 1) / 2 + 1 &&
+           c->cin % 32 == 0 && c->cout % 64 == 0 && c->n > 0 && c->cin == d0->cin && c->cout == d0->cout &&
+           (int64_t)c->n * (c->hin + 2) * (c->win + 2) * c->cin * 2 < (1ll << 31) &&
+           (int64_t)c->n * (c->hout + 2) * (c->wout + 2) * c->cout * 2 < (1ll << 31);
+}
+
+extern "C" int agp_conv2d_s2_fwd(const agp_conv_desc* descs, int n, void* stream) {
+    if (!descs) return AGP_E_BADARG;
+    if (n < 1 || n > 2 || AGP_TUNE("CONV_KERNEL", 0) || AGP_TUNE("NO_S2", 0)) return AGP_E_UNSUPPORTED;
+    for (int i = 0; i < n; ++i)
+        if (!s2_conv_ok(descs + i, descs)) return AGP_E_UNSUPPORTED;
+    IgemmParams ps[2];
+    for (int i = 0; i < n; ++i) {
+        ps[i] = IgemmParams{};
+        const int rc = conv_fill_params(descs + i, ps[i]);
+        if (rc != AGP_OK) return rc;
+    }
+    return agp_internal_conv_s2(ps, descs, n, (hipStream_t)stream, nullptr, true);
+}
+
+extern "C" int agp_conv2d_fwd_grouped2(const agp_conv_desc* descs, const agp_conv_stream2* s2, int n, void* stream) {
+    if (!descs || !s2) return AGP_E_BADARG;
+    if (n < 1 || n > 4 || AGP_TUNE("CONV_KERNEL", 0) || !AGP_TUNE("KXR_WIDE", 1)) return AGP_E_UNSUPPORTED;
+    bool any = false;
+    for (int i = 0; i < n; ++i) {
+        const agp_conv_desc* d = descs + i;
+        const bool ok = d->prec == AGP_PREC_F16 && d->in_hi && d->w_hi && d->out_hi && !d->in_lo && !d->w_lo && !d->out_lo && !d->res_lo &&
+                        !d->hi_only && d->n > 0 && d->cin % 32 == 0 && d->cout % 128 == 0 && conv_kxr_ok(d) && agp_internal_use_kxr2(d) &&
+                        d->cin == descs[0].cin && d->cout == descs[0].cout;
+        if (!ok) return AGP_E_UNSUPPORTED;
+        const agp_conv_stream2* t = s2 + i;
+        if (!t->in_hi) continue;
+        any = true;
+        if (!t->w_cm || d->res_hi || d->pool_partial || t->n != d->n || t->cin <= 0 || t->cin % 32 || t->hin <= 0 || t->win <= 0 ||
+            (t->hin - 1) / 2 + 1 != d->hout || (t->win - 1) / 2 + 1 != d->wout ||
+            (int64_t)t->n * (t->hin + 2) * (t->win + 2) * t->cin * 2 >= (1ll << 31))
+            return AGP_E_UNSUPPORTED;
+    }
+    IgemmParams ps[4];
+    KxrwStreams ds = {};
+    for (int i = 0; i < n; ++i) {
+        ps[i] = IgemmParams{};
+        const int rc = conv_fill_params(descs + i, ps[i]);
+        if (rc != AGP_OK) return rc;
+        agp_internal_conv_kxr_geometry(ps[i], descs + i);
+        const agp_conv_stream2* t = s2 + i;
+        if (!t->in_hi) continue;
+        const int wp = t->win + 2, hp = t->hin + 2;
+        KxrwStream& k = ds.s[i];
+        k.x = t->in_hi; k.w = t->w_cm;
+        k.x_bytes = (uint32_t)((int64_t)t->n * hp * wp * t->cin * 2);
+        k.w_bytes = (uint32_t)((int64_t)t->cin * descs[i].cout * 2);
+        k.sn = hp * wp * t->cin; k.sh = 2 * wp * t->cin; k.sw = 2 * t->cin; k.base = (wp - 1) * t->cin;
+        k.nc = t->cin / 32;
+    }
+    return agp_internal_conv_kxrw(ps, n, (hipStream_t)stream, nullptr, any ? &ds : nullptr);
+}
 
 extern "C" int agp_conv2d_tile_plan(const agp_conv_desc* descs, int n, int32_t plan[8]) {
     if (!descs || !plan || n <= 0) return AGP_E_BADARG;
diff --git a/agplace_amd/csrc/igemm_kxr2.hip b/agplace_amd/csrc/igemm_kxr2.hip
--- a/agplace_amd/csrc/igemm_kxr2.hip
+++ b/agplace_amd/csrc/igemm_kxr2.hip
@@ -425,12 +425,12 @@
 
 }
 
-int agp_internal_conv_kxrw(agp_igemm::IgemmParams* ps, int n, hipStream_t s, agp_igemm::TilePlan* plan);
+int agp_internal_conv_kxrw(agp_igemm::IgemmParams* ps, int n, hipStream_t s, agp_igemm::TilePlan* plan, const agp_igemm::KxrwStreams* ds);
 
 int agp_internal_conv_kxr2(agp_igemm::IgemmParams* ps, int n, hipStream_t s, agp_igemm::TilePlan* plan) {
     using namespace agp_igemm;
     if (n < 1 || n > KXR2_MAXP) return AGP_E_BADARG;
-    if (AGP_TUNE("KXR_WIDE", 1) && ps[0].N % 128 == 0) return agp_internal_conv_kxrw(ps, n, s, plan);
+    if (AGP_TUNE("KXR_WIDE", 1) && ps[0].N % 128 == 0) return agp_internal_conv_kxrw(ps, n, s, plan, nullptr);
     Kxr2Group g = {};
     g.nprob = n;
     for (int i = 0; i < n; ++i) {
diff --git a/agplace_amd/csrc/igemm_kxrw.hip b/agplace_amd/csrc/igemm_kxrw.hip
--- a/agplace_amd/csrc/igemm_kxrw.hip
+++ b/agplace_amd/csrc/igemm_kxrw.hip
@@ -5,7 +5,6 @@
 
 namespace agp_igemm {
 
-constexpr int KXRW_MAXP = 4;
 struct KxrwGroup {
     IgemmParams p[KXRW_MAXP];
     int mt_end[KXRW_MAXP];
@@ -15,6 +14,7 @@
     uint32_t r_bytes[KXRW_MAXP];
 };
 constexpr uint32_t KXRW_ROOB = 0xffffff00u;
+__device__ __forceinline__ const KxrwStreams& kxrw_streams(const KxrwStreams& s) { return s; }
 
 constexpr int KW_ROWB = 64;
 template <int TM_, int TN_> struct KwShape {
@@ -25,8 +25,8 @@
     static constexpr int EPI_LDS = SPARE + (4 - XWAVES) * STRIP;
 };
 
-template <bool POOL, int TM_, int TN_, bool RG, bool RES>
-__device__ __forceinline__ void kxrw_tile(const KxrwGroup& g, const int pid, const int m0, const int n0) {
+template <bool POOL, int TM_, int TN_, bool RG, int RES>
+__device__ __forceinline__ void kxrw_tile(const KxrwGroup& g, const int pid, const int m0, const int n0, const KxrwStream* sp = nullptr) {
 #if defined(__HIP_DEVICE_COMPILE__)
     using SH = KwShape<TM_, TN_>;
     constexpr int BN = SH::BN, NW = 4, TM = TM_, TN = TN_, ROWB = KW_ROWB;
@@ -36,6 +36,8 @@
     constexpr int NWP = BN / (NW * 16);
     static_assert(TN == 4 && (TM == 2 || TM == 1), "the full tile (256 x 128) and its half tile (128 x 128)");
     static_assert(NWP == 2 && (NX == 5 || NX == 3), "the vmcnt counts exist for these");
+    constexpr int NX2 = SH::BM / (16 * NW);
+    static_assert(!(POOL && RES == 2), "the computed residual is not instantiated with the pooling epilogue");
     extern __shared__ __attribute__((aligned(16))) char smem[];
     char* const ws = smem + 2 * X_BUF;
     float* const tab = (float*)(ws + 3 * W_TAP);
@@ -165,6 +167,23 @@
         __builtin_amdgcn_raw_ptr_buffer_load_lds(rr, LDS_PTR(strip + i * 1024), 16, off >= 0 ? off * 2 : (int)KXRW_ROOB, 0, 0, 0);
     };
 
+    int x2off[RES == 2 ? NX2 : 1], doff[RES == 2 ? NWP : 1];
+    int nc2 = 0;
+    __amdgpu_buffer_rsrc_t rx2 = rx, rd2 = rw;
+    if constexpr (RES == 2) {
+        nc2 = __builtin_amdgcn_readfirstlane(sp->nc);
+        rx2 = __builtin_amdgcn_make_buffer_rsrc((void*)sp->x, 0, sp->x_bytes, 0x00020000);
+        rd2 = __builtin_amdgcn_make_buffer_rsrc((void*)sp->w, 0, sp->w_bytes, 0x00020000);
+    }
+    auto load_x2 = [&](int buf, int j, int q) {
+        __builtin_amdgcn_raw_ptr_buffer_load_lds(rx2, LDS_PTR(smem + buf * X_BUF + (wave + NW * q) * 1024), 16, x2off[q],
+                                                 __builtin_amdgcn_readfirstlane(j * 64), 0, 0);
+    };
+    auto load_d = [&](int slot, int j, int i) {
+        __builtin_amdgcn_raw_ptr_buffer_load_lds(rd2, LDS_PTR(ws + slot * W_TAP + (wave + NW * i) * 1024), 16, doff[i],
+                                                 __builtin_amdgcn_readfirstlane(j * 64 * pN), 0, 0);
+    };
+
     int ky = 0, cc = 0;
     wait_vm_lgkm<NWP>();
     __builtin_amdgcn_s_barrier();
@@ -173,14 +192,15 @@
     auto phase = [&](auto KX, auto LAST, const char* xb, int st_, int nky_, int ncc_, int wcur_, int wnext_) {
         constexpr int kx = decltype(KX)::value;
         constexpr bool last = decltype(LAST)::value;
-        constexpr int nres = last && RES && kx < 2 ? NEI / 2 : 0;
+        constexpr int nres = last && RES == 1 && kx < 2 ? NEI / 2 : 0;
         const char* wb = ws + kx * W_TAP;
         bf16x8 xf[2][TM], wf[2][TN];
 #pragma unroll
         for (int t = 0; t < TM; ++t) xf[0][t] = *(const bf16x8*)(xb + xrd[kx][0] + t * (32 * ROWB));
 #pragma unroll
         for (int t = 0; t < TN; ++t) wf[0][t] = *(const bf16x8*)(wb + wrd[0] + t * (32 * ROWB));
-        constexpr int ndma = (kx == 0 ? (last ? NWP : NWP + NX) : (last ? 0 : NWP)) + nres;
+        constexpr int nstr = last && RES == 2 ? (kx == 0 ? NX2 : NWP) : 0;
+        constexpr int ndma = (kx == 0 ? (last ? NWP : NWP + NX) : (last ? 0 : NWP)) + nres + nstr;
         static_assert(ndma <= 8, "one piece per MFMA pair");
 #pragma unroll
         for (int t = 0; t < TM; ++t) xf[1][t] = *(const bf16x8*)(xb + xrd[kx][1] + t * (32 * ROWB));
@@ -189,6 +209,10 @@
         auto piece = [&](int i) {
             if (nres && i >= ndma - nres) {
                 load_residual(strip0, 0, kx * (NEI / 2) + i - (ndma - nres));
+            } else if (nstr && i >= ndma - nstr) {
+                const int k = i - (ndma - nstr);
+                if (kx == 0) load_x2(xidle, 0, k);
+                else load_d(kx - 1, kx - 1 < nc2 ? kx - 1 : nc2 - 1, k);
             } else if (kx == 0) {
                 if (i < NWP) {
                     const int so = __builtin_amdgcn_readfirstlane((wcur_ + 2 * tapb) * wmul);
@@ -242,22 +266,110 @@
         __builtin_amdgcn_s_barrier();
         ky = nky; cc = ncc;
     }
+    if constexpr (RES == 2) {
+        const int s_sn = sp->sn, s_sh = sp->sh, s_sw = sp->sw, s_base = sp->base;
+#pragma unroll
+        for (int q = 0; q < NX2; ++q) {
+            const int row = (wave + NW * q) * 16 + lrow;
+            const int m = m0 + row;
+            const uint32_t img = fdiv((uint32_t)m, d_howo);
+            const uint32_t rem = (uint32_t)m - img * d_howo.d;
+            const uint32_t y = fdiv(rem, d_wo);
+            const uint32_t xq = rem - y * d_wo.d;
+            const int el = (int)img * s_sn + (int)y * s_sh + (int)xq * s_sw + s_base;
+            x2off[q] = el * 2 + ((lpos ^ swz32(row)) << 4);
+        }
+#pragma unroll
+        for (int i = 0; i < NWP; ++i) {
+            const int row = (wave + NW * i) * 16 + lrow;
+            const int n = n0 + row < pN ? n0 + row : pN - 1;
+            doff[i] = n * 64 + ((lpos ^ swz32(row)) << 4);
+        }
+    }
     {
         const int st = nsteps - 1;
         const int wcur = (ky * 3 * CK + cc * 32) * 2;
         const char* xb = smem + (st & 1) * X_BUF;
         phase(I0{}, BT{}, xb, st, 0, 0, wcur, 0);
-        wait_vm_lgkm<NWP + (RES ? NEI / 2 : 0)>();
+        wait_vm_lgkm<NWP + (RES == 1 ? NEI / 2 : RES == 2 ? NX2 : 0)>();
         __builtin_amdgcn_s_barrier();
         phase(I1{}, BT{}, xb, st, 0, 0, wcur, 0);
-        wait_vm_lgkm<(RES ? NEI : 0)>();
+        wait_vm_lgkm<(RES == 1 ? NEI : RES == 2 ? NX2 + NWP : 0)>();
         __builtin_amdgcn_s_barrier();
         phase(I2{}, BT{}, xb, st, 0, 0, wcur, 0);
     }
+    if constexpr (RES == 2) {
+        {
+            const float* tb = tab + 8 * lh;
+#pragma unroll
+            for (int jj = 0; jj < TN * 2; ++jj) {
+                const f32x4 s0 = *(const f32x4*)(tb + 16 * jj), s1 = *(const f32x4*)(tb + 16 * jj + 4);
+                const f32x4 h0 = *(const f32x4*)(tb + BN + 16 * jj), h1 = *(const f32x4*)(tb + BN + 16 * jj + 4);
+#pragma unroll
+                for (int tm = 0; tm < TM; ++tm)
+#pragma unroll
+                    for (int e = 0; e < 8; ++e)
+                        acc[jj >> 1][tm][8 * (jj & 1) + e] =
+                            acc[jj >> 1][tm][8 * (jj & 1) + e] * (e < 4 ? s0[e & 3] : s1[e & 3]) + (e < 4 ? h0[e & 3] : h1[e & 3]);
+            }
+        }
+        auto tphase = [&](auto MODE, int j) {
+            constexpr int mode = decltype(MODE)::value;
+            const char* xb = smem + ((xidle + j) & 1) * X_BUF;
+            const char* wb = ws + (j % 3) * W_TAP;
+            bf16x8 xf[2][TM], wf[2][TN];
+#pragma unroll
+            for (int ks = 0; ks < 2; ++ks) {
+#pragma unroll
+                for (int t = 0; t < TM; ++t) xf[ks][t] = *(const bf16x8*)(xb + xrd[0][ks] + t * (32 * ROWB));
+#pragma unroll
+                for (int t = 0; t < TN; ++t) wf[ks][t] = *(const bf16x8*)(wb + wrd[ks] + t * (32 * ROWB));
+            }
+            constexpr int ndma = mode == 2 ? NX2 + NWP : (mode == 1 ? NX2 : 0);
+            static_assert(ndma <= 8, "one piece per MFMA pair");
+            int ip = 0;
+#pragma unroll
+            for (int ks = 0; ks < 2; ++ks)
+#pragma unroll
+                for (int tn = 0; tn < TN; ++tn)
+#pragma unroll
+                    for (int tm = 0; tm < TM; ++tm) {
+                        acc[tn][tm] = __builtin_amdgcn_mfma_f32_32x32x16_f16(__builtin_bit_cast(f16x8, wf[ks][tn]),
+                                                                             __builtin_bit_cast(f16x8, xf[ks][tm]), acc[tn][tm], 0, 0, 0);
+                        if ((TM == 1 || (tm & 1)) && ip < ndma) {
+                            if (ip < NX2) load_x2((xidle + j + 1) & 1, j + 1, ip);
+                            else load_d((j + 2) % 3, j + 2, ip - NX2);
+                            ++ip;
+                        }
+                    }
+            __builtin_amdgcn_sched_group_barrier(0x100, 2 * (TM + TN), 0);
+#pragma unroll
+            for (int i = 0; i < 8; ++i) {
+                __builtin_amdgcn_sched_group_barrier(0x008, TM == 1 ? 1 : 2, 0);
+                if (i < ndma) __builtin_amdgcn_sched_group_barrier(0x010, 1, 0);
+            }
+            __builtin_amdgcn_sched_barrier(0);
+        };
+        wait_vm_lgkm<NWP>();
+        __builtin_amdgcn_s_barrier();
+        int j = 0;
+        for (; j + 2 < nc2; ++j) {
+            tphase(I2{}, j);
+            wait_vm_lgkm<NWP>();
+            __builtin_amdgcn_s_barrier();
+        }
+        for (; j + 1 < nc2; ++j) {
+            tphase(I1{}, j);
+            wait_vm_lgkm<0>();
+            __builtin_amdgcn_s_barrier();
+        }
+        tphase(I0{}, j);
+        asm volatile("s_waitcnt vmcnt(0)" ::: "memory");
+    }
 
     asm volatile("s_waitcnt lgkmcnt(0)" ::: "memory");
     __builtin_amdgcn_s_barrier();
-    if constexpr (RES) {
+    if constexpr (RES == 1) {
         if constexpr (TM == 2) {
 #pragma unroll
             for (int i = 0; i < NEI; ++i) load_residual(strip1, 1, i);
@@ -290,7 +402,7 @@
             }
         }
         u32x4 rres[TN * 2];
-        if constexpr (RES) {
+        if constexpr (RES == 1) {
 #pragma unroll
             for (int jj = 0; jj < TN * 2; ++jj) rres[jj] = *(const u32x4*)(strip + a_off + ((jj ^ a_swz) << 5));
         }
@@ -301,9 +413,11 @@
             const f32x4 h0 = *(const f32x4*)(tb + BN + 16 * jj), h1 = *(const f32x4*)(tb + BN + 16 * jj + 4);
             float v[8];
 #pragma unroll
-            for (int e = 0; e < 8; ++e)
-                v[e] = acc[jj >> 1][tm][8 * (jj & 1) + e] * (e < 4 ? s0[e & 3] : s1[e & 3]) + (e < 4 ? h0[e & 3] : h1[e & 3]);
-            if constexpr (RES) {
+            for (int e = 0; e < 8; ++e) {
+                if constexpr (RES == 2) v[e] = acc[jj >> 1][tm][8 * (jj & 1) + e];
+                else v[e] = acc[jj >> 1][tm][8 * (jj & 1) + e] * (e < 4 ? s0[e & 3] : s1[e & 3]) + (e < 4 ? h0[e & 3] : h1[e & 3]);
+            }
+            if constexpr (RES == 1) {
                 float r[8];
                 unpack8_h(rres[jj], r);
 #pragma unroll
@@ -319,7 +433,7 @@
 #pragma unroll
         for (int i = 0; i < NEI; ++i) lines[i] = *(const u32x4*)(strip + l_off + i * 1024);
         if constexpr (TM == 2) {
-            if (tm == 0 && RES) wait_vm_lgkm<0>();
+            if (tm == 0 && RES == 1) wait_vm_lgkm<0>();
         }
 #pragma unroll
         for (int i = 0; i < NEI; ++i) {
@@ -400,8 +514,8 @@
 #endif
 }
 
-template <bool POOL, bool MIX, bool RG>
-__global__ void __launch_bounds__(256, 2) igemm_kxrw_kernel(KxrwGroup g) {
+template <bool POOL, bool MIX, bool RG, class... DS>
+__global__ void __launch_bounds__(256, 2) igemm_kxrw_kernel(KxrwGroup g, DS... ds) {
 #if defined(__HIP_DEVICE_COMPILE__)
     constexpr int TM_ = 2, TN_ = 4;
     constexpr int BM = KwShape<TM_, TN_>::BM, BN = KwShape<TM_, TN_>::BN;
@@ -430,13 +544,21 @@
         if (half) {
             const int m0 = mt * BM + sub * (BM / 2);
             if (m0 >= g.p[pid].M) return;
-            if (g.p[pid].r_hi) kxrw_tile<POOL, 1, TN_, RG, true>(g, pid, m0, n0);
-            else kxrw_tile<POOL, 1, TN_, RG, false>(g, pid, m0, n0);
+            if constexpr (sizeof...(DS) != 0) {
+                const KxrwStream* sp = &kxrw_streams(ds...).s[pid];
+                if (sp->x) { kxrw_tile<POOL, 1, TN_, RG, 2>(g, pid, m0, n0, sp); return; }
+            }
+            if (g.p[pid].r_hi) kxrw_tile<POOL, 1, TN_, RG, 1>(g, pid, m0, n0);
+            else kxrw_tile<POOL, 1, TN_, RG, 0>(g, pid, m0, n0);
             return;
         }
     }
-    if (g.p[pid].r_hi) kxrw_tile<POOL, TM_, TN_, RG, true>(g, pid, mt * BM, n0);
-    else kxrw_tile<POOL, TM_, TN_, RG, false>(g, pid, mt * BM, n0);
+    if constexpr (sizeof...(DS) != 0) {
+        const KxrwStream* sp = &kxrw_streams(ds...).s[pid];
+        if (sp->x) { kxrw_tile<POOL, TM_, TN_, RG, 2>(g, pid, mt * BM, n0, sp); return; }
+    }
+    if (g.p[pid].r_hi) kxrw_tile<POOL, TM_, TN_, RG, 1>(g, pid, mt * BM, n0);
+    else kxrw_tile<POOL, TM_, TN_, RG, 0>(g, pid, mt * BM, n0);
 #endif
 }
 
@@ -473,9 +595,19 @@
     return AGP_OK;
 }
 
+template <bool MIX, bool RG>
+int launch_kxrw_ds(KxrwGroup& g, const KxrwStreams& ds, const KxrwPlan& k, hipStream_t s) {
+    constexpr int lds = KwShape<2, 4>::EPI_LDS;
+    static std::atomic<uint64_t> attr_done{0};
+    if (!agp_lds_attr((const void*)igemm_kxrw_kernel<false, MIX, RG, KxrwStreams>, lds, attr_done)) return AGP_E_LAUNCH;
+    AGP_LAUNCH((igemm_kxrw_kernel<false, MIX, RG, KxrwStreams>), dim3(MIX ? k.blocks : k.half_bid0), dim3(256), lds, s, g, ds);
+    AGP_CHECK_LAUNCH();
+    return AGP_OK;
 }
 
-int agp_internal_conv_kxrw(agp_igemm::IgemmParams* ps, int n, hipStream_t s, agp_igemm::TilePlan* plan) {
+}
+
+int agp_internal_conv_kxrw(agp_igemm::IgemmParams* ps, int n, hipStream_t s, agp_igemm::TilePlan* plan, const agp_igemm::KxrwStreams* ds) {
     using namespace agp_igemm;
     if (n < 1 || n > KXRW_MAXP || ps[0].N % 128) return AGP_E_BADARG;
     constexpr int bm = KwShape<2, 4>::BM, bn = KwShape<2, 4>::BN;
@@ -505,6 +637,13 @@
     g.mt_chunk = k.mt_chunk;
     g.half_bid0 = k.half_bid0;
     g.rflag = agp_range_flag_get();
+    if (ds) {
+        if (pool) return AGP_E_UNSUPPORTED;
+        return agp_rg_dispatch(g.rflag, [&](auto rg) {
+            constexpr bool RG = decltype(rg)::value;
+            return mix ? launch_kxrw_ds<true, RG>(g, *ds, k, s) : launch_kxrw_ds<false, RG>(g, *ds, k, s);
+        });
+    }
     return agp_rg_dispatch(g.rflag, [&](auto rg) {
         constexpr bool RG = decltype(rg)::value;
         if (mix) return pool ? launch_kxrw<true, true, RG>(g, k, s) : launch_kxrw<false, true, RG>(g, k, s);
diff --git a/agplace_amd/csrc/igemm_params.hpp b/agplace_amd/csrc/igemm_params.hpp
--- a/agplace_amd/csrc/igemm_params.hpp
+++ b/agplace_amd/csrc/igemm_params.hpp
@@ -109,6 +109,15 @@
     return pid;
 }
 
+constexpr int KXRW_MAXP = 4;
+struct KxrwStream {
+    const void* x; const void* w;
+    uint32_t x_bytes, w_bytes;
+    int sn, sh, sw, base;
+    int nc;
+};
+struct KxrwStreams { KxrwStream s[KXRW_MAXP]; };
+
 constexpr int EPI_ROWB = 64 * 4 + 16;
 
 struct TilePlan {
diff --git a/agplace_amd/csrc/igemm_s2.hip b/agplace_amd/csrc/igemm_s2.hip
--- a/agplace_amd/csrc/igemm_s2.hip
+++ b/agplace_amd/csrc/igemm_s2.hip
@@ -16,11 +16,11 @@
 constexpr int S2_BMX = S2_BM + 16;
 constexpr int S2_XBLK = S2_BMX * S2_ROWB;
 constexpr int S2_XBUF = 2 * S2_XBLK;
-template <int TN> constexpr int s2_lds() {
-    return 2 * S2_XBUF + 4 * (32 * TN * S2_ROWB) + 4 * (32 * TN) * 4;
+template <int TN, bool NODS = false> constexpr int s2_lds() {
+    return 2 * S2_XBUF + (NODS ? 3 : 4) * (32 * TN * S2_ROWB) + 4 * (32 * TN) * 4;
 }
 
-template <int TN, class... RF>
+template <int TN, bool NODS, class... RF>
 __global__ void __launch_bounds__(256, TN == 2 ? 3 : 2) igemm_s2_kernel(S2Group g, RF... rf) {
 #if defined(__HIP_DEVICE_COMPILE__)
     constexpr bool RG = sizeof...(RF) != 0;
@@ -32,7 +32,7 @@
     static_assert(NX == 5, "the vmcnt counts below are written for NX = 5");
     extern __shared__ __attribute__((aligned(16))) char smem[];
     char* const ws = smem + 2 * S2_XBUF;
-    float* const tab = (float*)(ws + 4 * S2_WTAP);
+    float* const tab = (float*)(ws + (NODS ? 3 : 4) * S2_WTAP);
 
     const int tid = threadIdx.x;
     const int lane = tid & 63;
@@ -54,7 +54,7 @@
     const int pM = p.M, pN = p.N, pKtot = p.Ktot;
     const int x_sn = p.x_sn, x_sh_ = p.x_sh, x_sw = p.x_sw, x_base = p.x_base;
     const int o_sn = p.o_sn, o_sw = p.o_sw, o_base = p.o_base;
-    const bool has_ds = p.w2_hi != nullptr;
+    const bool has_ds = !NODS && p.w2_hi != nullptr;
 
     const int lrow = lane >> 2, lpos = lane & 3;
     const int cpix = p.CK * 2;
@@ -137,11 +137,14 @@
         for (int ks = 0; ks < 2; ++ks) wrd[ks] = wrow * ROWB + (((2 * ks + lh) ^ swz32(wrow)) << 4);
     }
 
-    f32x16 acc[TN], acc2[TN];
+    f32x16 acc[TN], acc2[NODS ? 1 : TN];
 #pragma unroll
     for (int a = 0; a < TN; ++a)
 #pragma unroll
-        for (int r = 0; r < 16; ++r) { acc[a][r] = 0.f; acc2[a][r] = 0.f; }
+        for (int r = 0; r < 16; ++r) {
+            acc[a][r] = 0.f;
+            if constexpr (!NODS) acc2[a][r] = 0.f;
+        }
 
     constexpr int LPP = BN / 8, PPI = 64 / LPP, NEI = 32 / PPI;
     int eoff[NEI];
@@ -164,7 +167,10 @@
     int ky = 0, cc = 0;
     wait_vm_lgkm<NWP>();
     __builtin_amdgcn_s_barrier();
-    if (tid < BN) { tab[tid] = tab_v[0]; tab[BN + tid] = tab_v[1]; tab[2 * BN + tid] = tab_v[2]; tab[3 * BN + tid] = tab_v[3]; }
+    if (tid < BN) {
+        tab[tid] = tab_v[0]; tab[BN + tid] = tab_v[1];
+        if constexpr (!NODS) { tab[2 * BN + tid] = tab_v[2]; tab[3 * BN + tid] = tab_v[3]; }
+    }
     auto phase = [&](auto KX, auto LAST, const char* xb, int st_, int ky_, int nky_, int ncc_, int wcur_, int wnext_) {
         constexpr int kx = decltype(KX)::value;
         constexpr bool last = decltype(LAST)::value;
@@ -176,7 +182,7 @@
 #pragma unroll
             for (int t = 0; t < TN; ++t) wf[ks][t] = *(const bf16x8*)(wb + wrd[ks] + t * (32 * ROWB));
         }
-        constexpr int ndma = kx == 0 ? (last ? NWP : NWP + NX) : (last ? 0 : (kx == 2 ? 2 * NWP : NWP));
+        constexpr int ndma = kx == 0 ? (last ? NWP : NWP + NX) : (last ? 0 : (kx == 2 && !NODS ? 2 * NWP : NWP));
         auto piece = [&](int i) {
             if (kx == 0) {
                 if (i < NWP) {
@@ -192,7 +198,7 @@
             } else if (i < NWP) {
                 const int so = __builtin_amdgcn_readfirstlane((wnext_ + (kx - 1) * tapb) * wmul);
                 __builtin_amdgcn_raw_ptr_buffer_load_lds(rw, LDS_PTR(ws + (kx - 1) * S2_WTAP + (wave + NW * i) * 1024), 16, woff_c[i], so, 0, 0);
-            } else {
+            } else if constexpr (!NODS) {
                 const int so = __builtin_amdgcn_readfirstlane((nky_ == 1 ? ncc_ : 0) * 64 * dmul);
                 const int k = i - NWP;
                 __builtin_amdgcn_raw_ptr_buffer_load_lds(rd, LDS_PTR(ws + 3 * S2_WTAP + (wave + NW * k) * 1024), 16,
@@ -217,7 +223,7 @@
             if (i < ndma) __builtin_amdgcn_sched_group_barrier(0x010, 1, 0);
         }
         __builtin_amdgcn_sched_barrier(0);
-        if (kx == 1 && ky_ == 1 && has_ds) {
+        if constexpr (!NODS) if (kx == 1 && ky_ == 1 && has_ds) {
             const char* db = ws + 3 * S2_WTAP;
             bf16x8 df[2][TN];
 #pragma unroll
@@ -245,7 +251,7 @@
         wait_vm_lgkm<NX + NWP>();
         __builtin_amdgcn_s_barrier();
         phase(I2{}, std::false_type{}, xb, st, ky, nky, ncc, wcur, wnext);
-        wait_vm_lgkm<2 * NWP>();
+        wait_vm_lgkm<(NODS ? 1 : 2) * NWP>();
         __builtin_amdgcn_s_barrier();
         ky = nky; cc = ncc;
     }
@@ -295,14 +301,14 @@
         __builtin_amdgcn_fence(__ATOMIC_RELEASE, "wavefront");
     };
     epilogue(acc, tab, (bf16_t*)p.o_hi, p.relu ? 0.f : -65504.f, false);
-    if (has_ds) epilogue(acc2, tab + 2 * BN, (bf16_t*)p.o2_hi, -65504.f, true);
+    if constexpr (!NODS) if (has_ds) epilogue(acc2, tab + 2 * BN, (bf16_t*)p.o2_hi, -65504.f, true);
     rg.flush(rg_word(rf...), p.relu ? 0.f : -65504.f);
 #endif
 }
 
 }
 
-int agp_internal_conv_s2(agp_igemm::IgemmParams* ps, const agp_conv_desc* descs, int n, hipStream_t s, agp_igemm::TilePlan* plan) {
+int agp_internal_conv_s2(agp_igemm::IgemmParams* ps, const agp_conv_desc* descs, int n, hipStream_t s, agp_igemm::TilePlan* plan, bool nods) {
     using namespace agp_igemm;
     if (n < 1 || n > S2_MAXP) return AGP_E_BADARG;
     S2Group g = {};
@@ -342,9 +348,14 @@
         return AGP_OK;
     }
     int rc;
-    if (rflag) rc = w4 ? launch(igemm_s2_kernel<4, uint32_t*>, s2_lds<4>(), a4g, rflag)
-                       : launch(igemm_s2_kernel<2, uint32_t*>, s2_lds<2>(), a2g, rflag);
-    else rc = w4 ? launch(igemm_s2_kernel<4>, s2_lds<4>(), a4s) : launch(igemm_s2_kernel<2>, s2_lds<2>(), a2s);
+    if (nods) {
+        static std::atomic<uint64_t> n4s{0}, n2s{0}, n4g{0}, n2g{0};
+        if (rflag) rc = w4 ? launch(igemm_s2_kernel<4, true, uint32_t*>, s2_lds<4, true>(), n4g, rflag)
+                           : launch(igemm_s2_kernel<2, true, uint32_t*>, s2_lds<2, true>(), n2g, rflag);
+        else rc = w4 ? launch(igemm_s2_kernel<4, true>, s2_lds<4, true>(), n4s) : launch(igemm_s2_kernel<2, true>, s2_lds<2, true>(), n2s);
+    } else if (rflag) rc = w4 ? launch(igemm_s2_kernel<4, false, uint32_t*>, s2_lds<4>(), a4g, rflag)
+                              : launch(igemm_s2_kernel<2, false, uint32_t*>, s2_lds<2>(), a2g, rflag);
+    else rc = w4 ? launch(igemm_s2_kernel<4, false>, s2_lds<4>(), a4s) : launch(igemm_s2_kernel<2, false>, s2_lds<2>(), a2s);
     if (rc != AGP_OK) return rc;
     AGP_CHECK_LAUNCH();
     return AGP_OK;
diff --git a/agplace_amd/ops.py b/agplace_amd/ops.py
--- a/agplace_amd/ops.py
+++ b/agplace_amd/ops.py
@@ -637,6 +637,47 @@
     return [j[2] for j in jobs]
 
 
+class Stream2Weights:
+    __slots__ = ("cin", "cout", "plane", "shift", "fusable")
+
+    def __init__(self, weight, scale, shift):
+        cout, cin = int(weight.shape[0]), int(weight.shape[1])
+        if tuple(weight.shape[2:]) != (1, 1) or cin % 32:
+            raise ValueError("Stream2Weights: a 1x1 conv with cin % 32 == 0")
+        wf = weight.detach().float().reshape(cout, cin) * scale.detach().float().reshape(cout, 1)
+        self.cin, self.cout = cin, cout
+        self.fusable = bool(torch.isfinite(wf).all()) and bool((wf.abs() < 65504.0).all())
+        self.plane = wf.half().view(cout, cin // 32, 32).permute(1, 0, 2).contiguous() if self.fusable else None
+        self.shift = shift.detach().float().contiguous()
+
+
+def conv2d_s2_nods(jobs):
+    arr = (_lib.ConvDesc * len(jobs))()
+    keep = []
+    for d, (x, cw, out, relu) in zip(arr, jobs):
+        keep.append(cw.planes(_lib.PREC_F16))
+        _fill_conv_desc(d, x, cw, out, None, relu, _lib.PREC_F16)
+    check(_L().agp_conv2d_s2_fwd(arr, len(jobs), _lib.stream()), "agp_conv2d_s2_fwd")
+    return [j[2] for j in jobs]
+
+
+def conv2d_grouped2(jobs):
+    arr = (_lib.ConvDesc * len(jobs))()
+    st = (_lib.ConvStream2 * len(jobs))()
+    keep = []
+    for d, t, (x, cw, out, residual, relu, stream2) in zip(arr, st, jobs):
+        keep.append(cw.planes(_lib.PREC_F16))
+        _fill_conv_desc(d, x, cw, out, residual, relu, _lib.PREC_F16)
+        if stream2 is not None:
+            x2, sw = stream2
+            if x2.lo is not None or x2.pad != 1 or x2.c != sw.cin or sw.plane is None:
+                raise ValueError("conv2d_grouped2: the second stream is a one-plane fp16 map with a 1-pixel halo and fusable weights")
+            t.in_hi, t.w_cm = ptr(x2.hi), ptr(sw.plane)
+            t.n, t.hin, t.win, t.cin = x2.n, x2.h, x2.w, sw.cin
+    check(_L().agp_conv2d_fwd_grouped2(arr, st, len(jobs), _lib.stream()), "agp_conv2d_fwd_grouped2")
+    return [j[2] for j in jobs]
+
+
 def conv2d(x: SplitMap, cw: ConvWeights, out: SplitMap, residual: SplitMap = None, relu=False, prec=3, stat_partial=None, pool=None,
            bstat=None, hi_only=False):
     d = _fill_conv_desc(_lib.ConvDesc(), x, cw, out, residual, relu, prec, stat_partial, bstat)
diff --git a/agplace_amd/resnet.py b/agplace_amd/resnet.py
--- a/agplace_amd/resnet.py
+++ b/agplace_amd/resnet.py
@@ -54,6 +54,7 @@
 
 
 FUSE_STEM_POOL = True
+FUSE_DOWNSAMPLE = True
 
 
 class ResNet(nn.Module):
@@ -108,11 +109,13 @@
         key = self._version_key()
         if key != self._prep_key:
             self._prep, self._prep_key = {}, key
+            self.__dict__["_prep_fuse"] = {}
         scaled = bool(scaled) and any(self._map_exp.values())
         if scaled in self._prep:
             return self._prep[scaled]
         prep = {}
         mexp = prep["exp"] = {}
+        fuse = {}
 
         def E(name):
             return int(self._map_exp.get(name, 0)) if scaled else 0
@@ -135,8 +138,35 @@
                     mexp[(li, bi, ci)] = e_prev = e_o
                 mexp[("ds", li, bi)] = g_out
                 prep[(li, bi)] = (cws, fold(*ds, g_in, g_out) if ds else None)
+                fuse[(li, bi)] = self._fused_downsample(blk, ds, cws, g_in, g_out)
         self._prep[scaled] = prep
+        self.__dict__.setdefault("_prep_fuse", {})[scaled] = fuse
         return prep
+
+    def _prepared_fuse(self, scaled=False):
+        self._prepared(scaled)
+        return self._prep_fuse[bool(scaled) and any(self._map_exp.values())]
+
+    @staticmethod
+    def _fused_downsample(blk, ds, cws, g_in, g_out):
+        if ds is None or blk.kind != "basic" or len(cws) != 2:
+            return None
+        dc, c1, c2 = ds[0], cws[0], cws[1]
+        if tuple(dc.kernel_size) != (1, 1) or dc.stride[0] != 2 or dc.padding[0] != 0 or dc.in_channels % 32 or \
+                (c1.kh, c1.kw, c1.stride, c1.pad) != (3, 3, 2, 1) or (c2.kh, c2.kw, c2.stride, c2.pad) != (3, 3, 1, 1) or c2.cout % 128 or \
+                c2.cin % 32:
+            return None
+        if dc.weight.is_cuda and torch.cuda.is_current_stream_capturing():
+            return None
+        bn = ds[1]
+        s_d, t_d = ops.fold_exp(*ops.fold_bn(bn.weight, bn.bias, bn.running_mean, bn.running_var, bn.eps), g_in, g_out)
+        sw = ops.Stream2Weights(dc.weight, s_d, t_d)
+        if not sw.fusable:
+            return None
+        import copy
+        c2f = copy.copy(c2)
+        c2f.shift = (c2.shift + sw.shift).contiguous()
+        return sw, c2f
 
     @staticmethod
     def _input_geometry(x):
@@ -291,6 +321,7 @@
         if (b.fe_type, b.nstages) != (a.fe_type, a.nstages):
             raise ValueError("forward_maps_multi: the trunks must share one architecture")
     preps = [net._prepared(scaled=prec != 3) for net in nets]
+    fuses = [net._prepared_fuse(scaled=prec != 3) for net in nets]
     geo = [net._input_geometry(x) for net, x in zip(nets, xs)]
     devs = [g[3] for g in geo]
     nchunks = max(1, -(-geo[0][0] // STAGE1_CHUNK))
@@ -317,8 +348,12 @@
             mexp = {r: preps[r]["exp"] for r in act}
             lname = f"layer{li + 1}.{bi}"
             ds_jobs = []
+            fz = {r: fuses[r].get((li, bi)) for r in act} if (prec == 4 and FUSE_DOWNSAMPLE and ops.MAP_PROBE is None) else {}
+            fused = [r for r in act if fz.get(r) is not None]
             if cws[act[0]][1] is not None:
                 for r in act:
+                    if r in fused:
+                        continue
                     dsw = cws[r][1]
                     ho = ops.conv_out_size(cur[r].h, 3, blks[r].stride, 1)
                     wo = ops.conv_out_size(cur[r].w, 3, blks[r].stride, 1)
@@ -343,6 +378,34 @@
                 if ops.MAP_PROBE is not None:
                     for r in act:
                         ops.probe_map(nets[r], f"{lname}.out", cur[r])
+                continue
+            if fused:
+                plain = [r for r in act if r not in fused]
+                o1, o2 = {}, {}
+                for r in act:
+                    c1 = cws[r][0][0]
+                    o1[r] = view(r, f"c{li}.{bi}.0", ops.conv_out_size(cur[r].h, 3, 2, 1), ops.conv_out_size(cur[r].w, 3, 2, 1), c1.cout,
+                                 mexp[r][(li, bi, 0)])
+                    o2[r] = view(r, f"c{li}.{bi}.1", o1[r].h, o1[r].w, cws[r][0][1].cout, mexp[r][(li, bi, 1)])
+                for k in range(0, len(fused), 2):
+                    ops.conv2d_s2_nods([(cur[r], cws[r][0][0], o1[r], True) for r in fused[k:k + 2]])
+                if plain:
+                    cj = [(cur[r], cws[r][0][0], o1[r], None, True) for r in plain]
+                    if len(cj) + len(ds_jobs) <= 4:
+                        ops.conv2d_grouped(cj + ds_jobs, prec)
+                    else:
+                        ops.conv2d_grouped(ds_jobs, prec)
+                        ops.conv2d_grouped(cj, prec)
+                for k in range(0, len(act), 4):
+                    ops.conv2d_grouped2([(o1[r], fz[r][1], o2[r], None, True, (cur[r], fz[r][0])) if r in fused else
+                                         (o1[r], cws[r][0][1], o2[r], idt[r], True, None) for r in act[k:k + 4]])
+                if bi == nblocks - 1 and (li > 0 or nchunks == 1):
+                    for r in act:
+                        pool = stage_pool[r].get(li)
+                        if pool is not None:
+                            pool.fused = False
+                            pool.finish(o2[r])
+                cur = o2
                 continue
             for ci in range(nconv):
                 last = ci == nconv - 1
diff --git a/include/agplace_hip.h b/include/agplace_hip.h
--- a/include/agplace_hip.h
+++ b/include/agplace_hip.h
@@ -106,6 +106,14 @@
 int agp_conv2d_fwd(const agp_conv_desc* d, void* stream);
 
 int agp_conv2d_fwd_grouped(const agp_conv_desc* descs, int n, void* stream);
+
+typedef struct agp_conv_stream2 {
+    const void* in_hi;
+    const void* w_cm;
+    int32_t n, hin, win, cin;
+} agp_conv_stream2;
+int agp_conv2d_s2_fwd(const agp_conv_desc* descs, int n, void* stream);
+int agp_conv2d_fwd_grouped2(const agp_conv_desc* descs, const agp_conv_stream2* s2, int n, void* stream);
 
 #define AGP_CONV_KERNEL_GENERIC 1
 #define AGP_CONV_KERNEL_DIRECT_X 2
```

Result: faster. 42650 pairs/s (median of 6 runs) (+2.0%).
